# OpenVVC/OpenVVC

Hardware: AMD Instinct MI355X
Metric: decoded frames/sec, full rcn back-end decode step (H2D of the recorded picture + MC incl. BDOF/DMVR/affine-PROF/GPM/CIIP + LMCS + inverse transform + ordered intra pass + deblocking + SAO + ALF/CC-ALF + D2H of refined MVs + wait + per-picture digest + publication to the device DPB), 4K 10-bit RA rec (higher is better)
Workload: dtype u16 samples / int16 coefficients / int32 accumulate

## Files before the change

### include/ovvc_hip.h

```cpp
#ifndef OVVC_HIP_H
#define OVVC_HIP_H

#include <stddef.h>
#include <stdint.h>

#ifdef __cplusplus
extern "C" {
#endif

#define OVHIP_ABI_VERSION 9

#define OVHIP_OK        0
#define OVHIP_ENODEV   (-1)
#define OVHIP_ENOMEM   (-2)
#define OVHIP_EINVAL   (-3)
#define OVHIP_ELAUNCH  (-4)
#define OVHIP_EUNSUP   (-5)
#define OVHIP_EREF     (-6)

enum { OVHIP_DST_VII = 0, OVHIP_DCT_VIII = 1, OVHIP_DCT_II = 2 };

typedef struct ovhip_pic {
    uint16_t *y, *cb, *cr;
    int32_t   w, h;
// ... 251 lines not shown
    uint8_t cc_cb_idx, cc_cr_idx;
    uint8_t border;
    uint8_t pad;
} ovhip_alf_ctu;

typedef struct ovhip_alf_pic {
    const ovhip_alf_ctu *ctus;
    const int16_t *luma_coeff;
    const int16_t *luma_clip;
    const int16_t *chroma_coeff;
    const int16_t *chroma_clip;
    const int16_t *cc_coeff;
    uint8_t *class_scratch;
    int32_t log2_ctu_s;
} ovhip_alf_pic;

enum { OVHIP_IT_LUMA = 0,
       OVHIP_IT_CHROMA = 1,
       OVHIP_IT_REGION = 2,
       OVHIP_IT_RES_C = 3,
       OVHIP_IT_IBC_L = 4,
       OVHIP_IT_IBC_C = 5 };
enum {
    OVHIP_IF_CORNER = 1,
    OVHIP_IF_MIP = 2,
    OVHIP_IF_MIP_TR = 4,
    OVHIP_IF_BDPCM = 8,
    OVHIP_IF_BDPCM_VER = 16,
    OVHIP_IF_RES_Y = 32, OVHIP_IF_RES_CB = 64, OVHIP_IF_RES_CR = 128,
    OVHIP_IF_RES_SCALE = 256,
    OVHIP_IF_SCALE_IDX = 512,
    OVHIP_IF_IBC_FREE = 4096,
    OVHIP_IF_CORNER_L = 2048,
    OVHIP_IF_ISP = 1024
};
typedef struct ovhip_itask {
    uint16_t x, y;
    uint8_t  log2_w, log2_h;
    uint8_t  kind;
    uint8_t  mode;
    uint16_t flags;
    uint8_t  avl_lft, avl_abv;
    uint8_t  mrl_idx;
    uint8_t  ciip_wt;
    int16_t  c_scale;
    uint16_t level;
    uint16_t ctu_deps;
    uint8_t  isp_log2_cb_w, isp_log2_cb_h;
    uint8_t  isp_off_x, isp_off_y;
    uint8_t  isp_log2_pb;
    uint8_t  isp_res_mask;
    uint16_t pad[3];
} ovhip_itask;
#define OVHIP_ITASK_IBC_DX(t) ((int)(int16_t)(t).pad[0])
#define OVHIP_ITASK_IBC_DY(t) ((int)(int16_t)(t).pad[1])

typedef struct ovhip_recorder ovhip_recorder;

typedef struct ovhip_tu_state {
    uint8_t qp_y, qp_cb, qp_cr, qp_jcbcr;
    uint8_t qp_y_skip, qp_cb_skip, qp_cr_skip, qp_jcbcr_skip;
    uint8_t dep_quant;
    uint8_t mts_implicit;
    uint8_t sh_ts_disabled;
    uint8_t ict_type;
    uint8_t lmcs_scale_c;
// ... 86 lines not shown
int   ovhip_rec_tu_intra(ovhip_recorder *rec, const ovhip_tu_state *st, const ovhip_tu_desc *tu, const ovhip_itask *intra_l,
                         const ovhip_itask *intra_c);
typedef struct ovhip_ibc_desc {
    uint16_t x0, y0;
    uint8_t  log2_w, log2_h;
    uint8_t  log2_ctu;
    uint8_t  has_chroma;
    int16_t  mv_x, mv_y;
    uint16_t win_x0;
    uint16_t pad;
} ovhip_ibc_desc;
int   ovhip_rec_ibc_check(ovhip_recorder *rec, const ovhip_ibc_desc *cu);
int   ovhip_rec_tu_ibc(ovhip_recorder *rec, const ovhip_tu_state *st, const ovhip_tu_desc *tu, const ovhip_ibc_desc *cu);
size_t ovhip_rec_ibc_tasks(const ovhip_recorder *rec);
typedef struct ovhip_isp_desc {
    uint16_t x0, y0;
    uint8_t  log2_cb_w, log2_cb_h;
    uint8_t  vertical;
    uint8_t  intra_mode;
    uint8_t  cbf_mask;
    uint8_t  lfnst_flag, lfnst_idx;
    uint8_t  mts_enabled;
    uint8_t  corner[4];
    uint8_t  avl_abv[4], avl_lft[4];
    uint16_t last_pos[4];
    uint64_t sig_sb_map[4];
    const int16_t *coef;
} ovhip_isp_desc;
int   ovhip_rec_isp_cu(ovhip_recorder *rec, const ovhip_tu_state *st, const ovhip_isp_desc *cu);
void  ovhip_isp_geometry(int32_t log2_cb_w, int32_t log2_cb_h, int32_t vertical, int32_t *log2_pb, int32_t *n_pb, int32_t *log2_pred,
                         int32_t *n_pred);
const ovhip_itask *ovhip_rec_itasks(const ovhip_recorder *rec, size_t *n);
const ovhip_itask *ovhip_rec_itasks_sorted(ovhip_recorder *rec, size_t *n, const uint32_t **level_start, uint32_t *n_levels);
typedef struct ovhip_ictu {
    uint16_t cx, cy;
    uint32_t first, n;
    uint32_t deps;
} ovhip_ictu;
int   ovhip_rec_set_ctu_size(ovhip_recorder *rec, int32_t log2_ctu_s);
uint32_t ovhip_rec_itask_levels(const ovhip_recorder *rec);
const ovhip_itask *ovhip_rec_itasks_by_ctu(ovhip_recorder *rec, int32_t log2_ctu_s, size_t *n, const ovhip_ictu **ctus, size_t *n_ctus);
int   ovhip_rec_transform_tree(ovhip_recorder *rec, const ovhip_tu_state *st, const ovhip_tt_desc *tt);
int   ovhip_rec_pu(ovhip_recorder *rec, const ovhip_pu_desc *pu);
int   ovhip_rec_affine_cu(ovhip_recorder *rec, const ovhip_affine_desc *cu);
int   ovhip_rec_cu_inter(ovhip_recorder *rec, const ovhip_pu_desc *pu, const ovhip_affine_desc *aff);
int   ovhip_rec_set_ref_scale(ovhip_recorder *rec, int32_t slot, const ovhip_ref_scale *scale);
#define OVHIP_RPR_TOOL_AFFINE 1u
#define OVHIP_RPR_TOOL_PU4x4  2u
int   ovhip_rec_set_rpr_tools(ovhip_recorder *rec, uint32_t mask);
const char *ovhip_rec_refusal(const ovhip_recorder *rec);
int   ovhip_rec_ciip(ovhip_recorder *rec, int32_t x0, int32_t y0, int32_t log2_w, int32_t log2_h,
                     int32_t mode_abv, int32_t mode_lft);
int   ovhip_ciip_weight(int32_t mode_abv, int32_t mode_lft);
int   ovhip_rec_lmcs_region(ovhip_recorder *rec, int32_t x0, int32_t y0, uint32_t abv_mask, uint32_t lft_mask);
typedef struct ovhip_dbf_edge {
    uint16_t ux, uy;
    uint16_t word;
    uint8_t  comp;
    uint8_t  pad;
} ovhip_dbf_edge;
#define OVHIP_DBF_MAX_OFFSETS 8
typedef struct ovhip_dbf_offsets { int8_t beta[OVHIP_DBF_MAX_OFFSETS], tc[OVHIP_DBF_MAX_OFFSETS]; } ovhip_dbf_offsets;
const ovhip_dbf_edge *ovhip_rec_dbf_edges(const ovhip_recorder *rec, int dir, size_t *n, ovhip_dbf_offsets *offsets);
int64_t ovhip_dbf_compact(const ovhip_dbf_planes *planes, int dir, ovhip_dbf_edge *out, size_t cap);

int   ovhip_rec_dbf_ctu(ovhip_recorder *rec, const ovhip_dbf_ctu *ctu);
// ... 363 lines not shown
    int32_t threads_per_device;
    int32_t output;
    ovhip_window window;
    uint32_t extra_stages;
    int32_t rank;
    const ovhip_stream_xfer *xfer;
    int32_t intra_lookahead;
    int32_t ahead_own_queue;
} ovhip_stream_cfg;

typedef struct ovhip_stream_result {
    double   seconds;
    uint64_t n_decoded, n_second_passes, n_received, n_sent;
    uint64_t out_frames, out_bytes;
    uint8_t  out_md5[16];
    double   record_seconds;
    double   host_seconds[5];
    int32_t  status;
    char     error[192];
    double  *trace;
} ovhip_stream_result;

typedef struct ovhip_stream ovhip_stream;
int  ovhip_stream_create(ovhip_stream **out, ovhip_dpb *dpb, const ovhip_stream_cfg *cfg, const ovhip_stream_content *contents,
                         uint32_t n_contents, ovhip_job *const *jobs, uint32_t n_jobs);
void ovhip_stream_destroy(ovhip_stream *s);
int  ovhip_stream_run(ovhip_stream *s, const ovhip_stream_pic *pics, uint32_t n_total, uint32_t first, uint32_t n, uint32_t flags,
                      uint8_t *digests, ovhip_stream_result *res);
ovhip_frame *ovhip_stream_frame(ovhip_stream *s, int dev, int thread);
int  ovhip_stream_queue_info(const ovhip_stream *s, int *moved, int *sharing);
int  ovhip_stream_set_output_scale(ovhip_stream *s, int32_t out_w, int32_t out_h, const ovhip_scale_info *info);
const void *ovhip_stream_key(const ovhip_stream *s, uint32_t idx);
int  ovhip_job_test_abort_next_flow(ovhip_job *job);

#ifdef __cplusplus
}
#endif
#endif
```

### openvvc_amd/capi.py

```python
from __future__ import annotations

import ctypes as C
import os
from pathlib import Path

import numpy as np

_PKG = Path(__file__).resolve().parent
LIB_PATH = _PKG / os.environ.get("OVVC_HIP_LIB_NAME", "libovvc_hip.so")

OVHIP_ABI_VERSION = 9
OVHIP_OK, OVHIP_ENODEV, OVHIP_ENOMEM, OVHIP_EINVAL, OVHIP_ELAUNCH, OVHIP_EUNSUP, OVHIP_EREF = 0, -1, -2, -3, -4, -5, -6
DST_VII, DCT_VIII, DCT_II = 0, 1, 2
TB_TR, TB_DC, TB_TS, TB_TS_RAW = 0, 1, 2, 3
TB_FLAG_RASTER = 0x80
RES_ADD, RES_SUB, RES_ADD_HALF, RES_SUB_HALF, RES_SCALE = 0, 1, 2, 3, 4
MC_HPEL_FILT, MC_FILT_4x4, MC_NO_LUMA, MC_NO_CHROMA, MC_LMCS, MC_BDOF, MC_DMVR = 1, 2, 4, 8, 16, 32, 64
PU_BDOF, PU_DMVR, PU_GPM = 1, 2, 4
MC_GPM = 128


class Pic(C.Structure):
    _fields_ = [("y", C.c_void_p), ("cb", C.c_void_p), ("cr", C.c_void_p),
                ("w", C.c_int32), ("h", C.c_int32), ("stride_y", C.c_int32), ("stride_c", C.c_int32)]
# ... 516 lines not shown
        "ovhip_job_band_busy": (C.c_int, [vp]),
        "ovhip_job_band_progress": (C.c_int, [vp, P(i32), P(vp), P(vp)]),
        "ovhip_rec_counts": (None, [vp, P(BandCounts)]),
        "ovhip_sao_launch_rows": (C.c_int, [vp, P(Pic), P(Pic), vp, i32, i32, i32]),
        "ovhip_alf_launch_rows": (C.c_int, [vp, P(Pic), P(Pic), P(AlfPic), i32, i32]),
        "ovhip_job_wait": (C.c_int, [vp]),
        "ovhip_job_refined_mvs": (vp, [vp, P(C.c_size_t)]),
        "ovhip_job_dmvr_rows": (C.c_int64, [vp, P(Pic), u32]),
        "ovhip_job_dmvr_rows_begin": (C.c_int64, [vp, P(Pic), u32, i32]),
        "ovhip_job_dmvr_rows_collect": (C.c_int64, [vp]),
        "ovhip_job_last_stats": (C.c_int, [vp, P(JobStats)]),
        "ovhip_job_time_stage": (C.c_int, [vp, C.c_int]),
        "ovhip_job_stage_time": (C.c_int, [vp, P(C.c_double), P(C.c_uint64)]),
        "ovhip_lmcs_scale_prepare_launch": (C.c_int, [vp, P(Pic), vp, u32, vp, vp, vp, u32, vp, u32]),
        "ovhip_lmcs_inverse_untag_launch": (C.c_int, [vp, P(Pic), vp, vp, u32]),
        "ovhip_intra_flow_untag_launch": (C.c_int, [vp, P(Pic), vp, u32, i32]),
        "ovhip_tmvp_cells_launch": (C.c_int, [vp, vp, u32, vp, i32, i32, vp]),
        "ovhip_job_tmvp_cells": (vp, [vp, P(C.c_size_t)]),
        "ovhip_output_bytes": (C.c_size_t, [i32, i32, P(Window)]),
        "ovhip_output_rows": (C.c_size_t, [i32, i32, P(Window)]),
        "ovhip_output_pack_launch": (C.c_int, [vp, P(Pic), P(Window), vp]),
        "ovhip_output_row_md5_launch": (C.c_int, [vp, P(Pic), P(Window), vp]),
        "ovhip_output_bands": (C.c_size_t, [i32, i32, P(Window)]),
        "ovhip_output_tree_md5_launch": (C.c_int, [vp, P(Pic), P(Window), vp]),
        "ovhip_pic_output": (C.c_int, [vp, P(Pic), P(Window), vp]),
        "ovhip_pic_digest": (C.c_int, [vp, P(Pic), P(Window), vp]),
        "ovhip_md5_init": (None, [P(Md5State)]),
        "ovhip_md5_update": (None, [P(Md5State), vp, C.c_size_t]),
        "ovhip_md5_final": (None, [P(Md5State), vp]),
        "ovhip_d2d": (C.c_int, [vp, vp, vp, C.c_size_t]),
        "ovhip_host_alloc": (vp, [C.c_size_t]),
        "ovhip_host_free": (None, [vp]),
        "ovhip_job_test_abort_next_flow": (C.c_int, [vp]),
        "ovhip_dpb_create": (C.c_int, [P(vp), P(C.c_int), C.c_int]),
        "ovhip_dpb_create_ex": (C.c_int, [P(vp), C.c_int, P(DpbOps)]),
        "ovhip_dpb_destroy": (None, [vp]),
        "ovhip_dpb_n_devices": (C.c_int, [vp]),
        "ovhip_dpb_device": (C.c_int, [vp, C.c_int]),
        "ovhip_dpb_begin": (C.c_int, [vp, vp, C.c_int, i32, i32, P(Pic)]),
        "ovhip_dpb_want": (C.c_int, [vp, vp, C.c_int]),
        "ovhip_dpb_begin_tag": (C.c_int, [vp, vp, C.c_uint64, C.c_int, i32, i32, P(Pic)]),
        "ovhip_dpb_want_tag": (C.c_int, [vp, vp, C.c_uint64, C.c_int]),
        "ovhip_dpb_acquire_tag": (C.c_int, [vp, vp, C.c_uint64, C.c_int, P(Pic), P(vp)]),
        "ovhip_dpb_publish": (C.c_int, [vp, vp, C.c_int]),
        "ovhip_dpb_acquire": (C.c_int, [vp, vp, C.c_int, P(Pic), P(vp)]),
        "ovhip_dpb_wait_copy": (C.c_int, [vp, C.c_int, vp]),
        "ovhip_dpb_poll_tag": (C.c_int, [vp, vp, C.c_uint64]),
        "ovhip_frame_refs_ready": (C.c_int, [vp]),
        "ovhip_dpb_set_unknown_key_timeout": (None, [vp, C.c_int]),
        "ovhip_dpb_unpin": (C.c_int, [vp, vp]),
        "ovhip_dpb_release": (C.c_int, [vp, vp]),
        "ovhip_dpb_lookup": (C.c_int, [vp, vp, P(C.c_int), P(Pic)]),
        "ovhip_dpb_shutdown": (None, [vp]),
        "ovhip_dpb_get_stats": (C.c_int, [vp, P(DpbStats)]),
        "ovhip_frame_create": (C.c_int, [vp, C.c_int, i32, i32, P(vp)]),
        "ovhip_frame_destroy": (None, [vp]),
        "ovhip_frame_ctx": (vp, [vp]),
        "ovhip_frame_job": (vp, [vp]),
        "ovhip_frame_recorder": (vp, [vp]),
        "ovhip_frame_begin": (C.c_int, [vp, vp]),
        "ovhip_frame_ref": (C.c_int, [vp, vp]),
        "ovhip_frame_set_trace": (None, [vp, vp]),
        "ovhip_rccl_unique_id": (C.c_int, [vp]),
        "ovhip_rccl_create": (C.c_int, [P(vp), vp, C.c_int, C.c_int, C.c_int]),
        "ovhip_rccl_destroy": (None, [vp]),
        "ovhip_rccl_xfer": (vp, [vp]),
# ... 40 lines not shown
    if path is None:
        _lib = lib
    return lib


EXPORTED_SYMBOLS = [
    "ovhip_abi_version", "ovhip_rec_create", "ovhip_rec_destroy", "ovhip_rec_reset", "ovhip_rec_tu",
    "ovhip_rec_pu", "ovhip_rec_cu_inter", "ovhip_rec_dbf_row", "ovhip_rec_dbf_mv_prepass_view", "ovhip_rec_dbf_ctu", "ovhip_rec_dbf_planes", "ovhip_dbf_launch", "ovhip_sao_launch", "ovhip_alf_launch", "ovhip_rec_tb_cmds", "ovhip_rec_coefs", "ovhip_rec_mc_units", "ovhip_rec_mcx_units", "ovhip_mcx_launch", "ovhip_rec_affine_cu", "ovhip_rec_transform_tree", "ovhip_rec_lmcs_region", "ovhip_dbf_compact", "ovhip_rec_dbf_mv_prepass", "ovhip_dbf_launch_edges", "ovhip_rec_ciip", "ovhip_ciip_weight", "ovhip_rec_ciip_units", "ovhip_ciip_launch", "ovhip_rec_lmcs_regions", "ovhip_rec_tb_cmds_split", "ovhip_itx_launch_classes", "ovhip_itx_launch_chroma_lmcs", "ovhip_lmcs_build", "ovhip_lmcs_scale_launch", "ovhip_lmcs_inverse_launch", "ovhip_rec_aff_units", "ovhip_rec_aff_side", "ovhip_mca_launch", "ovhip_mcxa_launch", "ovhip_ctx_create",
    "ovhip_ctx_destroy", "ovhip_ctx_sync", "ovhip_ctx_shares_queue", "ovhip_ctx_new_stream", "ovhip_ctx_fork", "ovhip_ctx_join", "ovhip_last_error", "ovhip_ctx_stream", "ovhip_malloc",
    "ovhip_free", "ovhip_h2d", "ovhip_d2h", "ovhip_pic_alloc", "ovhip_pic_free", "ovhip_pic_upload",
    "ovhip_pic_download", "ovhip_itx_launch", "ovhip_mc_launch",
    "ovhip_rec_set_ref_scale", "ovhip_rec_refusal", "ovhip_rec_rpr_units", "ovhip_mc_rpr_launch",
    "ovhip_rec_set_rpr_tools", "ovhip_rec_aff_rpr_units", "ovhip_mca_rpr_launch",
    "ovhip_rec_create_ex", "ovhip_rec_set_dense_dbf_planes", "ovhip_rec_dbf_edges", "ovhip_dbf_launch_edges_ex",
    "ovhip_dmvr_search_launch", "ovhip_rec_append_raw", "ovhip_rec_set_dbf_offsets", "ovhip_rec_tu_intra", "ovhip_rec_itasks", "ovhip_rec_itasks_sorted", "ovhip_itx_launch_classes_res", "ovhip_intra_level_launch", "ovhip_intra_level_geom", "ovhip_intra_sync_words", "ovhip_intra_ctu_launch", "ovhip_intra_flow_words", "ovhip_intra_flow_items", "ovhip_intra_flow_launch",
    "ovhip_rec_itask_levels", "ovhip_rec_isp_cu", "ovhip_isp_geometry", "ovhip_rec_itasks_by_ctu", "ovhip_rec_set_ctu_size", "ovhip_job_bind", "ovhip_job_create", "ovhip_job_destroy", "ovhip_job_recorder", "ovhip_job_begin",
    "ovhip_frame_band", "ovhip_frame_band_upto", "ovhip_frame_dmvr_rows_begin_upto", "ovhip_job_dmvr_rows_begin_upto", "ovhip_frame_set_band_mode", "ovhip_frame_band_stats", "ovhip_dpb_post_rows", "ovhip_dpb_rows_tag",
    "ovhip_job_band", "ovhip_job_band_active", "ovhip_job_band_busy", "ovhip_job_band_reserve", "ovhip_job_reserve_for_picture", "ovhip_rec_reserve_for_picture", "ovhip_job_band_progress", "ovhip_rec_counts", "ovhip_sao_launch_rows", "ovhip_alf_launch_rows",
    "ovhip_job_flush", "ovhip_job_wait", "ovhip_job_refined_mvs", "ovhip_job_dmvr_rows", "ovhip_job_dmvr_rows_begin", "ovhip_job_dmvr_rows_collect", "ovhip_job_last_stats", "ovhip_job_time_stage", "ovhip_job_stage_time",
    "ovhip_output_bytes", "ovhip_output_rows", "ovhip_output_pack_launch", "ovhip_output_row_md5_launch", "ovhip_output_bands", "ovhip_output_tree_md5_launch", "ovhip_pic_output", "ovhip_pic_digest",
    "ovhip_md5_init", "ovhip_md5_update", "ovhip_md5_final", "ovhip_tmvp_cells_launch", "ovhip_job_tmvp_cells", "ovhip_intra_flow_untag_launch", "ovhip_lmcs_inverse_untag_launch", "ovhip_lmcs_scale_prepare_launch",
    "ovhip_host_alloc", "ovhip_host_free", "ovhip_d2d", "ovhip_job_test_abort_next_flow",
    "ovhip_dpb_create", "ovhip_dpb_create_ex", "ovhip_dpb_destroy", "ovhip_dpb_n_devices", "ovhip_dpb_device", "ovhip_dpb_begin", "ovhip_dpb_want",
    "ovhip_dpb_publish", "ovhip_dpb_acquire", "ovhip_dpb_wait_copy", "ovhip_dpb_poll_tag", "ovhip_frame_refs_ready", "ovhip_dpb_set_unknown_key_timeout", "ovhip_dpb_unpin", "ovhip_dpb_release", "ovhip_dpb_lookup", "ovhip_dpb_shutdown",
    "ovhip_dpb_get_stats", "ovhip_dpb_begin_tag", "ovhip_dpb_want_tag", "ovhip_dpb_acquire_tag", "ovhip_frame_begin_tag", "ovhip_frame_ref_tag", "ovhip_frame_set_trace",
    "ovhip_rccl_unique_id", "ovhip_rccl_create", "ovhip_rccl_destroy", "ovhip_rccl_xfer", "ovhip_rccl_last_error", "ovhip_rccl_stats", "ovhip_rccl_self_exchange",
    "ovhip_frame_create", "ovhip_frame_destroy", "ovhip_frame_ctx", "ovhip_frame_job", "ovhip_frame_recorder", "ovhip_frame_begin", "ovhip_frame_ref",
    "ovhip_frame_ref_at", "ovhip_frame_dmvr_rows", "ovhip_frame_dmvr_rows_begin", "ovhip_frame_dmvr_rows_collect", "ovhip_frame_submit", "ovhip_frame_fail", "ovhip_frame_last_error",
    "ovhip_calllog_create", "ovhip_calllog_destroy", "ovhip_calllog_reset", "ovhip_calllog_data", "ovhip_rec_set_calllog", "ovhip_calllog_replay",
    "ovhip_stream_create", "ovhip_stream_destroy", "ovhip_stream_run", "ovhip_stream_frame", "ovhip_stream_key", "ovhip_stream_queue_info",
    "ovhip_output_scale_check", "ovhip_output_scale_launch", "ovhip_pic_output_scaled", "ovhip_pic_digest_scaled",
    "ovhip_frame_set_output_scale", "ovhip_stream_set_output_scale", "ovhip_ctx_scratch_bytes",
    "ovhip_rec_ibc_check", "ovhip_rec_tu_ibc", "ovhip_rec_ibc_tasks",
]


def rpr_units(lib, rec) -> list:
    n = C.c_size_t(0)
    ptr = lib.ovhip_rec_rpr_units(rec, C.byref(n))
    if not ptr or not n.value:
        return []
    raw = C.string_at(ptr, n.value * C.sizeof(RprUnit))
    return [RprUnit.from_buffer_copy(raw, i * C.sizeof(RprUnit)) for i in range(n.value)]


def aff_rpr_units(lib, rec) -> list:
    n = C.c_size_t(0)
    ptr = lib.ovhip_rec_aff_rpr_units(rec, C.byref(n))
    if not ptr or not n.value:
        return []
    raw = C.string_at(ptr, n.value * C.sizeof(AffRprUnit))
    return [AffRprUnit.from_buffer_copy(raw, i * C.sizeof(AffRprUnit)) for i in range(n.value)]


def set_ref_scale(lib, rec, slot: int, scale_hor: int | None = None, scale_ver: int | None = None, ref_w: int = 0, ref_h: int = 0,
                  col_hor: int = 0, col_ver: int = 0) -> int:
    if scale_hor is None:
        return lib.ovhip_rec_set_ref_scale(rec, slot, None)
    sc = RefScale(scale_hor, scale_ver if scale_ver is not None else scale_hor, ref_w, ref_h, col_hor, col_ver)
    return lib.ovhip_rec_set_ref_scale(rec, slot, C.byref(sc))


class Recorder:

    def __init__(self, pic_w: int, pic_h: int):
        self.lib = load()
# ... 34 lines not shown
    def replay(self, log: np.ndarray) -> int:
        n = self.lib.ovhip_calllog_replay(log.ctypes.data, log.nbytes, self.h)
        if n < 0:
            raise ValueError(f"ovhip_calllog_replay -> {n}")
        return int(n)

    def tu(self, st: TuState, d: TuDesc) -> int:
        r = self.lib.ovhip_rec_tu(self.h, C.byref(st), C.byref(d))
        if r < 0:
            raise ValueError(f"ovhip_rec_tu -> {r}")
        return r

    def tu_intra(self, st: TuState, d: TuDesc, task_l: "ITask | None", task_c: "ITask | None") -> int:
        r = self.lib.ovhip_rec_tu_intra(self.h, C.byref(st), C.byref(d), C.byref(task_l) if task_l is not None else None,
                                        C.byref(task_c) if task_c is not None else None)
        if r < 0:
            raise ValueError(f"ovhip_rec_tu_intra -> {r}")
        return r

    def ibc_check(self, cu: IbcDesc) -> int:
        return self.lib.ovhip_rec_ibc_check(self.h, C.byref(cu))

    def tu_ibc(self, st: TuState, d: TuDesc, cu: IbcDesc) -> int:
        return self.lib.ovhip_rec_tu_ibc(self.h, C.byref(st), C.byref(d), C.byref(cu))

    def ibc_tasks(self) -> int:
        return int(self.lib.ovhip_rec_ibc_tasks(self.h))

    def refusal(self) -> str:
        return (self.lib.ovhip_rec_refusal(self.h) or b"").decode()

    def itasks(self) -> np.ndarray:
        return self._arr(self.lib.ovhip_rec_itasks, ITASK_DTYPE)

    def itasks_sorted(self):
        n, nl, ls = C.c_size_t(), C.c_uint32(), C.POINTER(C.c_uint32)()
        p = self.lib.ovhip_rec_itasks_sorted(self.h, C.byref(n), C.byref(ls), C.byref(nl))
        if not n.value:
            return np.zeros(0, ITASK_DTYPE), np.zeros(1, np.uint32)
        t = np.frombuffer((C.c_char * (n.value * 32)).from_address(p), dtype=ITASK_DTYPE).copy()
        return t, np.array([ls[i] for i in range(nl.value + 1)], np.uint32)

    def itasks_by_ctu(self, log2_ctu: int = 7):
        n, nc, cp = C.c_size_t(), C.c_size_t(), C.c_void_p()
        p = self.lib.ovhip_rec_itasks_by_ctu(self.h, log2_ctu, C.byref(n), C.byref(cp), C.byref(nc))
        if not n.value:
            return np.zeros(0, ITASK_DTYPE), np.zeros(0, ICTU_DTYPE)
        t = np.frombuffer((C.c_char * (n.value * 32)).from_address(p), dtype=ITASK_DTYPE).copy()
        c = np.frombuffer((C.c_char * (nc.value * 16)).from_address(cp.value), dtype=ICTU_DTYPE).copy()
        return t, c

    def transform_tree(self, st: "TuState", d: TtDesc, infos: bytes, res_cb: np.ndarray, res_cr: np.ndarray, res_y: np.ndarray) -> int:
        ib = (C.c_char * len(infos)).from_buffer_copy(infos)
        keep = [np.ascontiguousarray(a, dtype=np.int16) for a in (res_cb, res_cr, res_y)]
        d.tu_info = C.addressof(ib)
        for k in range(3):
            d.residual[k] = keep[k].ctypes.data
        r = self.lib.ovhip_rec_transform_tree(self.h, C.byref(st), C.byref(d))
        d.tu_info = None
        if r < 0:
            raise ValueError(f"ovhip_rec_transform_tree -> {r}")
        return r

    def isp_cu(self, st: TuState, d: IspDesc) -> int:
        r = self.lib.ovhip_rec_isp_cu(self.h, C.byref(st), C.byref(d))
        if r < 0:
# ... 129 lines not shown
```

### openvvc_amd/csrc/flow_state.hip.h

```cpp
#pragma once
#include <hip/hip_runtime.h>
#include <stdint.h>
#include "ovvc_hip.h"

#define OVHIP_FLOW_SYNC_WORDS 16
struct FlowState { unsigned *y, *c[2], *reg; int w4; };

static inline FlowState flow_state_of(uint32_t *d_state, int w, int h)
{
    FlowState fs;
    const size_t nu = (size_t)((w + 3) / 4) * ((h + 3) / 4);
    fs.w4 = (w + 3) / 4;
    fs.y = d_state + OVHIP_FLOW_SYNC_WORDS; fs.c[0] = fs.y + nu; fs.c[1] = fs.c[0] + nu; fs.reg = fs.c[1] + nu;
    return fs;
}

#define FLOW_ITEM_TASK_BITS  24
#define FLOW_ITEM_STRIP_BITS 5
#define FLOW_ITEM_MAX_TASKS  ((size_t)1 << FLOW_ITEM_TASK_BITS)
#define FLOW_ITEM_MAX_STRIPS (1 << FLOW_ITEM_STRIP_BITS)
struct FlowItem { uint32_t task; int strip, plane; };

__host__ __device__ static inline uint32_t flow_item_pack(uint32_t task, int strip, int plane)
{
    return task | ((uint32_t)strip << FLOW_ITEM_TASK_BITS) | ((uint32_t)plane << (FLOW_ITEM_TASK_BITS + FLOW_ITEM_STRIP_BITS));
}
__host__ __device__ static inline FlowItem flow_item_unpack(uint32_t word)
{
    FlowItem it;
    it.task = word & ((1u << FLOW_ITEM_TASK_BITS) - 1);
    it.strip = (int)((word >> FLOW_ITEM_TASK_BITS) & (FLOW_ITEM_MAX_STRIPS - 1));
    it.plane = (int)((word >> (FLOW_ITEM_TASK_BITS + FLOW_ITEM_STRIP_BITS)) & 1);
    return it;
}

extern "C" size_t ovhip_intra_flow_items_(const ovhip_itask *sorted, size_t n, uint32_t *items, size_t cap);

__device__ __forceinline__ void flow_prepare_task(const ovhip_itask &t, const FlowState &fs, unsigned epoch, int lane16)
{
    const unsigned mark = 2 * epoch;
    if (t.kind == OVHIP_IT_REGION) { if (lane16 == 0) fs.reg[t.c_scale] = mark; return; }
    const bool luma = t.kind == OVHIP_IT_LUMA || t.kind == OVHIP_IT_IBC_L;
    const bool both = t.kind == OVHIP_IT_CHROMA || t.kind == OVHIP_IT_IBC_C;
    const int sh = luma ? 2 : 1, w = 1 << t.log2_w, h = 1 << t.log2_h;
    const int ux0 = t.x >> sh, uy0 = t.y >> sh, nx = max(1, w >> sh), ny = max(1, h >> sh);
    const int l2nx = 31 - __clz(nx);
    for (int i = lane16; i < nx * ny; i += 16) {
        const int u = (uy0 + (i >> l2nx)) * fs.w4 + ux0 + (i & (nx - 1));
        if (luma) fs.y[u] = mark;
        else {
            if (both || (t.flags & OVHIP_IF_RES_CB)) fs.c[0][u] = mark;
            if (both || (t.flags & OVHIP_IF_RES_CR)) fs.c[1][u] = mark;
        }
    }
}
```

### openvvc_amd/csrc/kernels_intra.hip

```cpp
#include <stdlib.h>
#include "ovvc_common.hip.h"
#include "flow_state.hip.h"
#include "lmcs_wnd.hip.h"
#define OVT_ATTR __device__
#include "vvc_mip_tables.h"

namespace {

__device__ const short g_ang[32] = { 0, 1, 2, 3, 4, 6, 8, 10, 12, 14, 16, 18, 20, 23, 26, 29, 32, 35, 39, 45, 51, 57, 64, 73, 86, 102, 128, 171, 256, 341, 512, 1024 };
__device__ const short g_inv_ang[32] = { 0, 16384, 8192, 5461, 4096, 2731, 2048, 1638, 1365, 1170, 1024, 910, 819, 712, 630, 565, 512, 468, 420, 364,
                                         321, 287, 256, 224, 191, 161, 128, 96, 64, 48, 32, 16 };
__device__ __attribute__((aligned(4))) const signed char g_fc[32][4] = {
    { 0, 64, 0, 0 }, { -1, 63, 2, 0 }, { -2, 62, 4, 0 }, { -2, 60, 7, -1 }, { -2, 58, 10, -2 }, { -3, 57, 12, -2 }, { -4, 56, 14, -2 },
    { -4, 55, 15, -2 }, { -4, 54, 16, -2 }, { -5, 53, 18, -2 }, { -6, 52, 20, -2 }, { -6, 49, 24, -3 }, { -6, 46, 28, -4 }, { -5, 44, 29, -4 },
    { -4, 42, 30, -4 }, { -4, 39, 33, -4 }, { -4, 36, 36, -4 }, { -4, 33, 39, -4 }, { -4, 30, 42, -4 }, { -4, 29, 44, -5 }, { -4, 28, 46, -6 },
    { -3, 24, 49, -6 }, { -2, 20, 52, -6 }, { -2, 18, 53, -5 }, { -2, 16, 54, -4 }, { -2, 15, 55, -4 }, { -2, 14, 56, -4 }, { -2, 12, 57, -3 },
    { -2, 10, 58, -2 }, { -1, 7, 60, -2 }, { 0, 4, 62, -2 }, { 0, 2, 63, -1 } };

#define IR_NEG  64
#define IR_LEN  (IR_NEG + 2 * 64 + 4 + 24)
struct IntraLds {
    uint16_t abv[IR_LEN], lft[IR_LEN];
    uint16_t fabv[IR_LEN], flft[IR_LEN];
    uint16_t red[64], hup[8 * 64];
// ... 90 lines not shown
        const int n_cu = 2 * cb + 1, nb_ref = (2 * cb) / 4 + 1, len = cb + pb, last = min(4 * a, n_cu + 3);
        uint16_t *out = (arm ? s.lft : s.abv) + IR_NEG;
        for (int k = lane; k < len + 1 + 24; k += 64) {
            const int kk = min(k, len) + off;
            int v;
            if (c && a >= nb_ref) {
                const int q = min(kk, n_cu - 1);
                v = arm ? acc.ld(x0 - 1, y0 - oy - 1 + q) : acc.ld(x0 - ox - 1 + q, y0 - 1);
            } else if (c || a) {
                const int q = kk == 0 ? (c ? 0 : 1) : (a ? min(kk, last) : 0);
                v = arm ? acc.ld(x0 - 1, y0 - oy - 1 + q) : acc.ld(x0 - ox - 1 + q, y0 - 1);
            } else {
                v = other ? (arm ? acc.ld(x0, y0 - 1) : acc.ld(x0 - 1, y0)) : 1 << (OV_BD - 1);
            }
            out[k] = (uint16_t)v;
        }
    }
}

__device__ void smooth_refs(IntraLds &s, int len_a, int len_l, int lane)
{
    const uint16_t *a = s.abv + IR_NEG, *l = s.lft + IR_NEG;
    for (int i = lane; i < 2 * 64 + 4 + 24; i += 64) {
        int va, vl;
        if (i == 0) { va = (l[1] + 2 * a[0] + a[1] + 2) >> 2; vl = (a[1] + 2 * l[0] + l[1] + 2) >> 2; }
        else {
            va = i < len_a ? (a[i + 1] + 2 * a[i] + a[i - 1] + 2) >> 2 : a[i];
            vl = i < len_l ? (l[i + 1] + 2 * l[i] + l[i - 1] + 2) >> 2 : l[i];
        }
        s.fabv[IR_NEG + i] = (uint16_t)va; s.flft[IR_NEG + i] = (uint16_t)vl;
    }
}

__device__ __forceinline__ int res_scale(int v, int scale)
{
    const int sign = v & (1 << 15);
    int a = (ov_clip_bd(abs(v)) * scale + (1 << 10)) >> 11;
    return ov_clip3(sign ? -a : a, -(1 << 15), 1 << 15);
}

__device__ void pred_regular(IntraLds &s, const ovhip_itask &t, bool is_luma, const Strip st, int lane)
{
    const int l2w = t.log2_w, l2h = t.log2_h, w = 1 << l2w, h = 1 << l2h, n = w * h;
    const bool isp = t.flags & OVHIP_IF_ISP;
    const int mrl = (is_luma && !isp) ? t.mrl_idx : 0;
    const bool bdpcm = t.flags & OVHIP_IF_BDPCM;
    const bool pdpc_ok = isp ? l2h > 1 : (!mrl && !bdpcm && (is_luma || (l2w > 1 && l2h > 1)));
    const uint16_t *abv = s.abv + IR_NEG, *lft = s.lft + IR_NEG;
    if (bdpcm) {
        const bool ver = t.flags & OVHIP_IF_BDPCM_VER;
        for (int p = st.p0 + lane; p < st.p1; p += 64) { const int x = p & (w - 1), y = p >> l2w; s.pred[p - st.p0] = ver ? abv[1 + x] : lft[1 + y]; }
        return;
    }
    int mode = t.mode;
    if (mode == 0) {
        const uint16_t *a = abv + mrl, *l = lft + mrl;
        if (is_luma && !isp && !mrl && l2w + l2h > 5) { smooth_refs(s, w + 4, h + 4, lane); wave_sync(); a = s.fabv + IR_NEG; l = s.flft + IR_NEG; }
        const int scale = (l2w + l2h - 2) >> 2;
        for (int p = st.p0 + lane; p < st.p1; p += 64) {
            const int x = p & (w - 1), y = p >> l2w;
            const int pv = ((h - 1 - y) * a[1 + x] + (y + 1) * l[1 + h]) << l2w;
            const int ph = ((w - 1 - x) * l[1 + y] + (x + 1) * a[1 + w]) << l2h;
            int v = (pv + ph + n) >> (l2w + l2h + 1);
            if (pdpc_ok) { const int wt = pdpc_wgt(y, scale), wl = pdpc_wgt(x, scale); v = ov_clip_bd((l[1 + y] * wl + a[1 + x] * wt + (64 - wl - wt) * v + 32) >> 6); }
            s.pred[p - st.p0] = (uint16_t)v;
        }
        return;
    }
    if (mode == 1) {
        const uint16_t *a = abv + mrl, *l = lft + mrl;
        int sum = 0;
        if (w >= h) for (int x = lane; x < w; x += 64) sum += a[1 + x];
// ... 299 lines not shown
    int v[NP];
#pragma unroll
    for (int i = 0; i < NP; ++i) {
        const int p = min(it.p0 + lane + 64 * i, it.p1 - 1);
        v[i] = acc.ld(sx + (p & ((1 << l2w) - 1)), sy + (p >> l2w)) & 0x7fff;
    }
#pragma unroll
    for (int i = 0; i < NP; ++i) { const int p = it.p0 + lane + 64 * i; if (p < it.p1) s.pred[p - it.p0] = (uint16_t)v[i]; }
    wave_sync();
}

template <int NP>
__device__ __forceinline__ void epilogue_load(int (&rv)[NP], int (&dv)[NP], const Item &it, const uint16_t *dst, int dstride, const int16_t *rp, int rstride,
                                              int l2w, int lane)
{
#pragma unroll
    for (int i = 0; i < NP; ++i) {
        const int p = it.p0 + lane + 64 * i, x = p & ((1 << l2w) - 1), y = p >> l2w;
        rv[i] = (it.has_res && p < it.p1 && it.res_at(x)) ? rp[y * rstride + x] : 0;
        dv[i] = (it.need_d() && p < it.p1) ? dst[y * dstride + x] : 0;
    }
}

template <int NP>
__device__ __forceinline__ void epilogue_store(const IntraLds &s, const int (&rv)[NP], const int (&dv)[NP], const Item &it, int scale, uint16_t *dst, int dstride,
                                               int l2w, int lane)
{
#pragma unroll
    for (int i = 0; i < NP; ++i) {
        const int p = it.p0 + lane + 64 * i, x = p & ((1 << l2w) - 1), y = p >> l2w;
        if (p >= it.p1) break;
        int v = it.res_only ? dv[i] : s.pred[p - it.p0];
        if (it.ciip_wt) v = (v * it.ciip_wt + dv[i] * (4 - it.ciip_wt) + 2) >> 2;
        if (it.has_res) v = ov_clip_bd(v + (it.scaled ? res_scale(rv[i], scale) : rv[i]));
        dst[y * dstride + x] = (uint16_t)v;
    }
}

template <bool IBC>
__global__ __launch_bounds__(64) void k_intra_level(ovhip_pic pic, ovhip_pic res, const ovhip_itask *__restrict__ tasks, uint32_t n,
                                                    const ovhip_lmcs_region *__restrict__ regs, LmcsWnd wnd, int16_t *__restrict__ scales,
                                                    int log2_ctu)
{
    __shared__ IntraLds s;
    const uint32_t bid = blockIdx.x;
    const int strip = blockIdx.y, comp = blockIdx.z;
    if (bid >= n) return;
    const int lane = threadIdx.x;
    load_tables(s, lane);
    const ovhip_itask t = tasks[bid];
    const Item it = item_of<STRIP, IBC>(t, strip, comp);
    const PlaneAcc ya = { pic.y, pic.stride_y };
    if (it.region) {
        if (!strip && !comp) { const int v = region_scale(ya, regs[t.c_scale], wnd, lane); if (lane == 0) scales[t.c_scale] = (int16_t)v; }
        return;
    }
    if (it.p0 >= it.p1 || (it.luma && comp) || it.skip()) return;
    uint16_t *pl = it.luma ? pic.y : (comp ? pic.cr : pic.cb);
    const int dstride = it.luma ? pic.stride_y : pic.stride_c, rstride = it.luma ? res.stride_y : res.stride_c;
    uint16_t *dst = pl + t.y * dstride + t.x;
    const int16_t *rp = reinterpret_cast<const int16_t *>(it.luma ? res.y : (comp ? res.cr : res.cb)) + t.y * rstride + t.x;
    int rv[NPL], dv[NPL];
    epilogue_load(rv, dv, it, dst, dstride, rp, rstride, t.log2_w, lane);
    const int scale = it.scaled ? (it.scale_idx ? scales[t.c_scale] : t.c_scale) : 0;
    const PlaneAcc ca = { pl, pic.stride_c };
    if (IBC && t.kind >= OVHIP_IT_IBC_L) ibc_copy<NPL>(s, t, it, PlaneAcc{ pl, dstride }, lane);
    else if (!it.res_only) predict_item<NPL>(s, t, it, ya, ca, log2_ctu, DirectRefs(), lane);
// ... 288 lines not shown
        }
        if (lowered) __builtin_amdgcn_s_setprio(OVHIP_FLOW_PRIO);
    }
#pragma unroll
    for (int i = 0; i < 3; ++i) {
        const int k = lane + 64 * i;
        if (k < na + 24) s.abv[IR_NEG + k] = (uint16_t)(v[2 * i] & 0x7fff);
        if (k < nl + 24) s.lft[IR_NEG + k] = (uint16_t)(v[2 * i + 1] & 0x7fff);
    }
    return ok;
}
#define FLOW_MAX_FP 448
#ifndef FSTRIP
#define FSTRIP 256
#endif
#define FNPL   (FSTRIP / 64)
#define FJ8    ((FSTRIP + 511) / 512)
#define FJ4    ((FSTRIP + 255) / 256)

__global__ __launch_bounds__(256) void k_intra_flow_prepare(const ovhip_itask *__restrict__ tasks, uint32_t n, FlowState fs, unsigned epoch)
{
    const uint32_t ti = blockIdx.x * 16 + (threadIdx.x >> 4);
    if (ti < n) flow_prepare_task(tasks[ti], fs, epoch, threadIdx.x & 15);
}

typedef uint32_t flow_u4 __attribute__((ext_vector_type(4), aligned(4)));
typedef uint32_t flow_u2 __attribute__((ext_vector_type(2), aligned(4)));
__global__ __launch_bounds__(256) void k_flow_untag(ovhip_pic pic, const ovhip_itask *__restrict__ tasks, uint32_t n, int with_luma)
{
    const uint32_t ti = blockIdx.x * 16 + (threadIdx.x >> 4);
    if (ti >= n) return;
    const ovhip_itask t = tasks[ti];
    const bool luma = t.kind == OVHIP_IT_LUMA || t.kind == OVHIP_IT_IBC_L;
    if (t.kind == OVHIP_IT_REGION || (luma && !with_luma)) return;
    const int lane = threadIdx.x & 15;
    const int l2w = t.log2_w, w = 1 << l2w, npx = w << t.log2_h;
    const int stride = luma ? pic.stride_y : pic.stride_c;
    for (int c = 0; c < (luma ? 1 : 2); ++c) {
        if (!luma && t.kind == OVHIP_IT_RES_C && !(t.flags & (c ? OVHIP_IF_RES_CR : OVHIP_IF_RES_CB))) continue;
        uint16_t *dst = (luma ? pic.y : (c ? pic.cr : pic.cb)) + t.y * stride + t.x;
        if (w >= 4) {
            for (int p = 4 * lane; p < npx; p += 64) {
                flow_u2 *q = reinterpret_cast<flow_u2 *>(dst + (p >> l2w) * stride + (p & (w - 1)));
                flow_u2 v = *q; v[0] &= 0x03ff03ffu; v[1] &= 0x03ff03ffu; *q = v;
            }
        } else if (w == 2) {
            for (int p = 2 * lane; p < npx; p += 32) {
                uint32_t *q = reinterpret_cast<uint32_t *>(dst + (p >> l2w) * stride + (p & (w - 1)));
                *q &= 0x03ff03ffu;
            }
        } else {
            for (int p = lane; p < npx; p += 16) { uint16_t *q = dst + (p >> l2w) * stride + (p & (w - 1)); *q = *q & 0x3ff; }
        }
    }
}

struct TaggedRefs {
    const unsigned *state_y, *state_c;
    int w4; unsigned epoch; unsigned *sync;
#ifdef OVHIP_CTU_PROBE
    u64 *stamp;
    __device__ __forceinline__ void arms_ready() const { *stamp = wall_clock64(); }
#else
    __device__ __forceinline__ void arms_ready() const { }
#endif
    __device__ __forceinline__ bool operator()(IntraLds &s, const AgentAcc acc, int unit, const ovhip_itask &t, int mrl, int lane) const
    {
// ... 34 lines not shown
{
    uint32_t r;
    asm("v_pk_add_i16 %0, %1, %2 clamp\n\tv_pk_max_i16 %0, %0, 0\n\tv_pk_min_i16 %0, %0, %3" : "=&v"(r) : "v"(pred2), "v"(res2), "v"(0x03ff03ffu));
    return r;
}

template <int G>
__device__ __forceinline__ void flow_store(const IntraLds &s, const FlowRaw &q, const Item &it, int scale, uint16_t *dst, int dstride, int l2w, int lane)
{
    typedef FlowRun<G> R;
    const uint32_t tag2 = FLOW_TAG | (FLOW_TAG << 16);
    const bool plain = G > 1 && !it.ciip_wt && !it.res_only && !it.scaled && it.res_mask == 0xff;
#pragma unroll
    for (int j = 0; j < R::N; ++j) {
        const int p = R::p_of(it, j, lane), x = p & ((1 << l2w) - 1), y = p >> l2w;
        if (p >= it.p1) break;
        typename R::vec pq = 0, out;
        if constexpr (G == 1) pq = s.pred[p - it.p0];
        else if (!it.res_only) pq = *reinterpret_cast<const typename R::vec *>(&s.pred[p - it.p0]);
        if (plain) {
#pragma unroll
            for (int e = 0; e < R::DW; ++e) out[e] = (it.has_res ? pk_clip_add(pq[e], q.r[R::DW * j + e]) : pq[e]) | tag2;
        } else {
            int v[G], rv[G], dv[G];
#pragma unroll
            for (int e = 0; e < G; ++e) {
                const int sh = 16 * (e & 1), k = R::DW * j + (e >> 1);
                rv[e] = it.res_at(x + e) ? (int)(int16_t)(q.r[k] >> sh) : 0;
                dv[e] = (int)((q.d[k] >> sh) & 0xffff);
                v[e] = it.res_only ? dv[e] : (int)((pq[e >> 1] >> sh) & 0xffff);
            }
            if (it.ciip_wt) for (int e = 0; e < G; ++e) v[e] = (v[e] * it.ciip_wt + dv[e] * (4 - it.ciip_wt) + 2) >> 2;
            if (it.has_res) {
                if (it.scaled) for (int e = 0; e < G; ++e) v[e] = ov_clip_bd(v[e] + res_scale(rv[e], scale));
                else           for (int e = 0; e < G; ++e) v[e] = ov_clip_bd(v[e] + rv[e]);
            }
#pragma unroll
            for (int e = 0; e < R::DW; ++e) out[e] = ((uint32_t)v[2 * e] | (G > 1 ? (uint32_t)v[G > 1 ? 2 * e + 1 : 0] << 16 : 0u)) | tag2;
        }
        uint16_t *o = dst + y * dstride + x;
        if constexpr (G == 8) asm volatile("global_store_dwordx4 %0, %1, off sc1" :: "v"(o), "v"(out) : "memory");
        else if constexpr (G == 4) asm volatile("global_store_dwordx2 %0, %1, off sc1" :: "v"(o), "v"(out) : "memory");
        else __hip_atomic_store(o, (uint16_t)out[0], RLX_AGENT);
    }
}

struct FlowLds { IntraLds s; uint32_t fp[FLOW_MAX_FP]; int abort; };

template <bool IBC>
__global__ __launch_bounds__(64) void k_intra_flow(ovhip_pic pic, ovhip_pic res, const ovhip_itask *__restrict__ tasks, const uint32_t *__restrict__ items,
                                                   uint32_t n_items, const ovhip_lmcs_region *__restrict__ regs, LmcsWnd wnd, int16_t *scales,
                                                   int log2_ctu, FlowState fs, unsigned epoch, unsigned *sync, unsigned *abort_mirror)
{
    __shared__ FlowLds L;
    IntraLds &s = L.s;
    if (blockIdx.x >= n_items) return;
    __builtin_amdgcn_s_setprio(OVHIP_FLOW_PRIO);
    const int lane = threadIdx.x;
    load_tables(s, lane);
    int prev_level = 0;
    for (uint32_t bid = blockIdx.x; bid < n_items; bid += gridDim.x) {
    if (bid != blockIdx.x) wave_sync();
    FPROBE_DECL;
    const FlowItem fi = flow_item_unpack(items[bid]);
    const ovhip_itask t = tasks[fi.task];
    const int comp = fi.plane;
    const Item it = item_of<FSTRIP, IBC>(t, fi.strip, comp);
    const int l2w = t.log2_w, w = 1 << l2w, h = 1 << t.log2_h;
    const bool luma = it.luma;
    const bool ibc = IBC && t.kind >= OVHIP_IT_IBC_L;
    const unsigned pending = 2 * epoch;
    const int w4 = fs.w4;
    if (it.skip()) continue;

    uint16_t *pl = luma ? pic.y : (comp ? pic.cr : pic.cb);
    const int dstride = luma ? pic.stride_y : pic.stride_c, rstride = luma ? res.stride_y : res.stride_c;
    uint16_t *dst = pl + t.y * dstride + t.x;
    const int16_t *rp = reinterpret_cast<const int16_t *>(luma ? res.y : (comp ? res.cr : res.cb)) + t.y * rstride + t.x;
    const int run = w >= 8 ? 8 : (w == 4 ? 4 : 1);
    FlowRaw raw = { };
    if (!it.region) {
        if (run == 8) flow_load<8>(raw, it, dst, dstride, rp, rstride, l2w, lane);
        else if (run == 4) flow_load<4>(raw, it, dst, dstride, rp, rstride, l2w, lane);
        else flow_load<1>(raw, it, dst, dstride, rp, rstride, l2w, lane);
    }
    {
        const int gap = min((int)t.level - prev_level - 1, FLOW_NAP_MAX_LEVELS);
        prev_level = (int)t.level;
        if (gap > 0) {
            __builtin_amdgcn_s_setprio(0);
            for (int k = 0; k < 2 * gap; ++k) __builtin_amdgcn_s_sleep(FLOW_NAP_HALF_LEVEL);
            __builtin_amdgcn_s_setprio(OVHIP_FLOW_PRIO);
        }
    }
    FPROBE(0);
    int nfp = 0;
    auto add_run = [&](unsigned *base, int ux, int uy, int count, int dx, int dy) {
        count = min(count, FLOW_MAX_FP - nfp);
        for (int i = lane; i < count; i += 64) L.fp[nfp + i] = (uint32_t)(base - sync) + (uint32_t)((uy + i * dy) * w4 + ux + i * dx);
        nfp += max(count, 0);
    };
    if (it.region) {
        const ovhip_lmcs_region g = regs[t.c_scale];
        if (g.n_abv) add_run(fs.y, g.x >> 2, (g.y >> 2) - 1, g.n_abv, 1, 0);
        if (g.n_lft) add_run(fs.y, (g.x >> 2) - 1, g.y >> 2, g.n_lft, 0, 1);
    } else if (luma) {
// ... 144 lines not shown
extern "C" int ovhip_debug_set_ctu_probe(void *d_buf)
{
    u64 *p = (u64 *)d_buf;
    return hipMemcpyToSymbol(HIP_SYMBOL(g_probe), &p, sizeof(p)) == hipSuccess ? 0 : -1;
}
#endif

extern "C" size_t ovhip_intra_sync_words(int32_t width, int32_t height, int32_t log2_ctu_s)
{
    if (width <= 0 || height <= 0 || log2_ctu_s < 5 || log2_ctu_s > 7) return 0;
    const size_t s = (size_t)1 << log2_ctu_s;
    return SYNC_FLAGS + ((width + s - 1) / s) * ((height + s - 1) / s);
}

extern "C" int ovhip_intra_ctu_launch(ovhip_ctx *ctx, const ovhip_pic *pic, const ovhip_pic *res, const ovhip_itask *d_tasks, const ovhip_ictu *d_ctus,
                                      uint32_t n_ctus, const ovhip_lmcs_region *d_regions, const ovhip_lmcs_luts *luts, int16_t *d_scales,
                                      int32_t log2_ctu_s, uint32_t *d_sync, uint32_t epoch, uint32_t *abort_mirror)
{
    if (!ctx || !pic || !res) return OVHIP_EINVAL;
    OV_DEVICE(ctx);
    if (!n_ctus) return OVHIP_OK;
    if (!d_tasks || !d_ctus || !d_sync || !epoch || log2_ctu_s < 5 || log2_ctu_s > 7)
        return ov_fail(ctx, OVHIP_EINVAL, "ovhip_intra_ctu_launch: bad arguments", hipSuccess);
    if ((pic->w & 7) || (pic->h & 1) || (pic->stride_y & 3) || (pic->stride_c & 3) || ((uintptr_t)pic->y & 7) || ((uintptr_t)pic->cb & 7) || ((uintptr_t)pic->cr & 7))
        return ov_fail(ctx, OVHIP_EUNSUP, "ovhip_intra_ctu_launch: picture width must be a multiple of 8 and the planes 8-byte aligned", hipSuccess);
    const LmcsWnd wnd = lmcs_wnd_of(luts);
    const int ncx = (pic->w + (1 << log2_ctu_s) - 1) >> log2_ctu_s;
    hipLaunchKernelGGL(k_intra_ctu, dim3(n_ctus), dim3(256), 0, ctx->stream, *pic, *res, d_tasks, d_ctus, d_regions, wnd, d_scales, log2_ctu_s, d_sync, epoch, ncx,
                       abort_mirror);
    OV_LAUNCH_CHECK(ctx, "k_intra_ctu");
    return OVHIP_OK;
}

extern "C" size_t ovhip_intra_flow_items_(const ovhip_itask *sorted, size_t n, uint32_t *items, size_t cap)
{
    size_t k = 0;
    for (size_t i = 0; sorted && i < n; ++i) {
        const ovhip_itask &t = sorted[i];
        if (i >= FLOW_ITEM_MAX_TASKS) return 0;
        if (t.kind == OVHIP_IT_REGION) { if (k < cap) items[k] = flow_item_pack((uint32_t)i, 0, 0); ++k; continue; }
        const int npx = 1 << (t.log2_w + t.log2_h), strips = (npx + FSTRIP - 1) / FSTRIP, comps = (t.kind == OVHIP_IT_LUMA || t.kind == OVHIP_IT_IBC_L) ? 1 : 2;
        if (strips > FLOW_ITEM_MAX_STRIPS) return 0;
        for (int st = 0; st < strips; ++st)
            for (int c = 0; c < comps; ++c) { if (k < cap) items[k] = flow_item_pack((uint32_t)i, st, c); ++k; }
    }
    return k;
}

extern "C" size_t ovhip_intra_flow_items(const ovhip_itask *sorted, size_t n, uint32_t *items, size_t cap)
{
    const size_t k = ovhip_intra_flow_items_(sorted, n, items, cap);
    return k <= cap ? k : 0;
}

extern "C" size_t ovhip_intra_flow_words(int32_t width, int32_t height)
{
    if (width <= 0 || height <= 0) return 0;
    return SYNC_FLAGS + 4 * (size_t)((width + 3) / 4) * ((height + 3) / 4);
}

extern "C" int ovhip_intra_flow_launch(ovhip_ctx *ctx, const ovhip_pic *pic, const ovhip_pic *res, const ovhip_itask *d_tasks, uint32_t n_tasks,
                                       const uint32_t *d_items, uint32_t n_items, const ovhip_lmcs_region *d_regions, const ovhip_lmcs_luts *luts,
                                       int16_t *d_scales, int32_t log2_ctu_s, uint32_t *d_state, uint32_t epoch, uint32_t *abort_mirror, int32_t prepare,
                                       int32_t n_workers)
{
    if (!ctx || !pic || !res) return OVHIP_EINVAL;
    OV_DEVICE(ctx);
    if (!n_items) return OVHIP_OK;
    if (!d_tasks || !d_items || !d_state || !epoch || epoch >= 0x7fffffffu || log2_ctu_s < 5 || log2_ctu_s > 7)
        return ov_fail(ctx, OVHIP_EINVAL, "ovhip_intra_flow_launch: bad arguments", hipSuccess);
    const LmcsWnd wnd = lmcs_wnd_of(luts);
    const FlowState fs = flow_state_of(d_state, pic->w, pic->h);
    if (prepare & 1) {
        hipLaunchKernelGGL(k_intra_flow_prepare, dim3((n_tasks + 15) / 16), dim3(256), 0, ctx->stream, d_tasks, n_tasks, fs, epoch);
        OV_LAUNCH_CHECK(ctx, "k_intra_flow_prepare");
    }
#ifdef OVHIP_CTU_PROBE
    if (hipMemcpyToSymbolAsync(HIP_SYMBOL(g_probe_items), &d_items, sizeof(d_items), 0, hipMemcpyHostToDevice, ctx->stream) != hipSuccess) return OVHIP_ELAUNCH;
#endif
    const uint32_t grid = (n_workers > 0 && (uint32_t)n_workers < n_items) ? (uint32_t)n_workers : n_items;
    if (prepare & OVHIP_FLOW_IBC)
        hipLaunchKernelGGL(k_intra_flow<true>, dim3(grid), dim3(64), 0, ctx->stream, *pic, *res, d_tasks, d_items, n_items, d_regions, wnd, d_scales, log2_ctu_s, fs,
                           epoch, d_state, abort_mirror);
    else
// ... 17 lines not shown
```

### openvvc_amd/csrc/kernels_lmcs.hip

```cpp
#include "ovvc_common.hip.h"
#include "flow_state.hip.h"
#include "lmcs_wnd.hip.h"

namespace {

#ifndef LMCS_ROWS
#define LMCS_ROWS 4
#endif

__global__ __launch_bounds__(64) void k_lmcs_scale(ovhip_pic pic, const ovhip_lmcs_region *__restrict__ regs, uint32_t n,
                                                   LmcsWnd wnd, int16_t *__restrict__ scales, const ovhip_itask *__restrict__ tasks,
                                                   uint32_t n_tasks, FlowState fs, unsigned epoch)
{
    const uint32_t bid = blockIdx.x;
    if (bid >= n) {
        const uint32_t ti = (bid - n) * 4 + (threadIdx.x >> 4);
        if (ti < n_tasks) flow_prepare_task(tasks[ti], fs, epoch, threadIdx.x & 15);
        return;
    }
    const ovhip_lmcs_region g = regs[bid];
    if (g.ordered) return;
    const int lane = threadIdx.x;
    const uint16_t *src = pic.y + (size_t)g.y * pic.stride_y + g.x;
    const int na = 4 * g.n_abv, nl = 4 * g.n_lft;
    const long oa = g.n_abv ? (long)min(lane, na - 1) - pic.stride_y : 0;
    const long ol = g.n_lft ? (long)min(lane, nl - 1) * pic.stride_y - 1 : 0;
    const int va = src[oa], vl = src[ol];
    int sum = (g.n_abv ? va : 0) + (g.n_lft ? vl : 0);
#pragma unroll
    for (int m = 32; m; m >>= 1) sum += __shfl_xor(sum, m);
    if (lane == 0) scales[bid] = (int16_t)lmcs_scale_of_sum(wnd, sum, g.n_abv, g.n_lft);
}

typedef uint32_t lm_u2 __attribute__((ext_vector_type(2), aligned(4)));

#define UNTAG_TASKS_PER_WG 4
__device__ __forceinline__ void untag_chroma_tasks(const ovhip_pic &pic, const ovhip_itask *__restrict__ tasks, uint32_t n, uint32_t wg)
{
    const uint32_t ti = wg * UNTAG_TASKS_PER_WG + (threadIdx.x >> 6);
    if (ti >= n) return;
    const ovhip_itask t = tasks[ti];
    if (t.kind == OVHIP_IT_REGION || t.kind == OVHIP_IT_LUMA || t.kind == OVHIP_IT_IBC_L) return;
    const int lane = threadIdx.x & 63;
    const int l2w = t.log2_w, w = 1 << l2w, npx = w << t.log2_h, stride = pic.stride_c;
    const bool res_only = t.kind == OVHIP_IT_RES_C;
    const bool on0 = !res_only || (t.flags & OVHIP_IF_RES_CB), on1 = !res_only || (t.flags & OVHIP_IF_RES_CR);
    uint16_t *const d0 = pic.cb + t.y * stride + t.x, *const d1 = pic.cr + t.y * stride + t.x;
    if (w >= 4) {
        for (int base = 0; base < npx; base += 1024) {
            lm_u2 v0[4], v1[4];
#pragma unroll
            for (int k = 0; k < 4; ++k) {
                const int p = base + 4 * lane + 256 * k;
                const int o = (p >> l2w) * stride + (p & (w - 1));
                if (p < npx && on0) v0[k] = *reinterpret_cast<const lm_u2 *>(d0 + o);
                if (p < npx && on1) v1[k] = *reinterpret_cast<const lm_u2 *>(d1 + o);
            }
#pragma unroll
            for (int k = 0; k < 4; ++k) {
                const int p = base + 4 * lane + 256 * k;
                const int o = (p >> l2w) * stride + (p & (w - 1));
                if (p < npx && on0) { lm_u2 v = v0[k]; v[0] &= 0x03ff03ffu; v[1] &= 0x03ff03ffu; *reinterpret_cast<lm_u2 *>(d0 + o) = v; }
                if (p < npx && on1) { lm_u2 v = v1[k]; v[0] &= 0x03ff03ffu; v[1] &= 0x03ff03ffu; *reinterpret_cast<lm_u2 *>(d1 + o) = v; }
            }
        }
    } else if (w == 2) {
        for (int p = 2 * lane; p < npx; p += 128) {
            const int o = (p >> l2w) * stride + (p & (w - 1));
            uint32_t a = 0, b = 0;
            if (on0) a = *reinterpret_cast<const uint32_t *>(d0 + o);
            if (on1) b = *reinterpret_cast<const uint32_t *>(d1 + o);
            if (on0) *reinterpret_cast<uint32_t *>(d0 + o) = a & 0x03ff03ffu;
            if (on1) *reinterpret_cast<uint32_t *>(d1 + o) = b & 0x03ff03ffu;
        }
    } else {
        for (int p = lane; p < npx; p += 64) {
            const int o = (p >> l2w) * stride + (p & (w - 1));
            if (on0) d0[o] = d0[o] & 0x3ff;
            if (on1) d1[o] = d1[o] & 0x3ff;
        }
    }
}

__global__ __launch_bounds__(256) void k_lmcs_inverse(ovhip_pic pic, const uint16_t *__restrict__ lut, uint32_t rows_y,
                                                      const ovhip_itask *__restrict__ tasks, uint32_t n_tasks)
{
    const uint32_t untag_y = gridDim.y - rows_y;
    if (blockIdx.y < untag_y) { untag_chroma_tasks(pic, tasks, n_tasks, blockIdx.y * gridDim.x + blockIdx.x); return; }
    const uint32_t by = blockIdx.y - untag_y;

    __shared__ uint16_t s_lut[1024];
    const int nvx = pic.w >> 3;
    const int tail = pic.w & 7;
    const int y00 = (int)by * LMCS_ROWS, v00 = blockIdx.x * 256 + threadIdx.x;
    uint4 q0[LMCS_ROWS];
    const bool first = y00 < pic.h && v00 < nvx;
    if (first) {
#pragma unroll
        for (int r = 0; r < LMCS_ROWS; ++r) q0[r] = *reinterpret_cast<const uint4 *>(pic.y + (size_t)min(y00 + r, pic.h - 1) * pic.stride_y + 8 * v00);
    }
    for (int i = threadIdx.x; i < 512; i += 256) reinterpret_cast<uint32_t *>(s_lut)[i] = reinterpret_cast<const uint32_t *>(lut)[i];
    __syncthreads();
    for (int y0 = y00; y0 < pic.h; y0 += rows_y * LMCS_ROWS) {
        for (int v = v00; v < nvx; v += gridDim.x * 256) {
            uint4 q[LMCS_ROWS];
            if (y0 == y00 && v == v00) {
#pragma unroll
                for (int r = 0; r < LMCS_ROWS; ++r) q[r] = q0[r];
            } else {
#pragma unroll
                for (int r = 0; r < LMCS_ROWS; ++r) q[r] = *reinterpret_cast<const uint4 *>(pic.y + (size_t)min(y0 + r, pic.h - 1) * pic.stride_y + 8 * v);
            }
#pragma unroll
            for (int r = 0; r < LMCS_ROWS; ++r) {
                if (y0 + r >= pic.h) break;
                uint32_t *d = reinterpret_cast<uint32_t *>(&q[r]);
#pragma unroll
                for (int k = 0; k < 4; ++k) d[k] = s_lut[d[k] & 1023] | ((uint32_t)s_lut[(d[k] >> 16) & 1023] << 16);
                *reinterpret_cast<uint4 *>(pic.y + (size_t)(y0 + r) * pic.stride_y + 8 * v) = q[r];
            }
        }
// ... 7 lines not shown

}

static int lmcs_scale_launch(ovhip_ctx *ctx, const ovhip_pic *pic, const ovhip_lmcs_region *d_regions, uint32_t n_regions, const ovhip_lmcs_luts *luts,
                             int16_t *d_scales, const ovhip_itask *d_tasks, uint32_t n_tasks, uint32_t *d_state, uint32_t epoch)
{
    if (!ctx || !pic || !luts) return OVHIP_EINVAL;
    OV_DEVICE(ctx);
    if (!n_regions && !n_tasks) return OVHIP_OK;
    if (n_regions && (!d_regions || !d_scales)) return ov_fail(ctx, OVHIP_EINVAL, "ovhip_lmcs_scale_launch: null buffer", hipSuccess);
    if (n_tasks && (!d_tasks || !d_state || !epoch)) return ov_fail(ctx, OVHIP_EINVAL, "ovhip_lmcs_scale_prepare_launch: bad arguments", hipSuccess);
    const LmcsWnd w = lmcs_wnd_of(luts);
    FlowState fs;
    memset(&fs, 0, sizeof(fs));
    if (n_tasks) fs = flow_state_of(d_state, pic->w, pic->h);
    hipLaunchKernelGGL(k_lmcs_scale, dim3(n_regions + (n_tasks + 3) / 4), dim3(64), 0, ctx->stream, *pic, d_regions, n_regions, w, d_scales, d_tasks, n_tasks, fs, epoch);
    OV_LAUNCH_CHECK(ctx, n_tasks ? "k_lmcs_scale (+ flow state words)" : "k_lmcs_scale");
    return OVHIP_OK;
}

extern "C" int ovhip_lmcs_scale_launch(ovhip_ctx *ctx, const ovhip_pic *pic, const ovhip_lmcs_region *d_regions,
                                       uint32_t n_regions, const ovhip_lmcs_luts *luts, int16_t *d_scales)
{
    return lmcs_scale_launch(ctx, pic, d_regions, n_regions, luts, d_scales, nullptr, 0, nullptr, 0);
}

extern "C" int ovhip_lmcs_scale_prepare_launch(ovhip_ctx *ctx, const ovhip_pic *pic, const ovhip_lmcs_region *d_regions, uint32_t n_regions,
                                               const ovhip_lmcs_luts *luts, int16_t *d_scales, const ovhip_itask *d_tasks, uint32_t n_tasks,
                                               uint32_t *d_state, uint32_t epoch)
{
    return lmcs_scale_launch(ctx, pic, d_regions, n_regions, luts, d_scales, d_tasks, n_tasks, d_state, epoch);
}

static int lmcs_inverse_launch(ovhip_ctx *ctx, const ovhip_pic *pic, const uint16_t *d_bwd_lut, const ovhip_itask *d_tasks, uint32_t n_tasks, const char *who)
{
    if (!ctx || !pic || !d_bwd_lut) return OVHIP_EINVAL;
    OV_DEVICE(ctx);
    if ((pic->stride_y & 7) || ((uintptr_t)pic->y & 15))
        return ov_fail(ctx, OVHIP_EINVAL, "ovhip_lmcs_inverse_launch: luma plane must be 16-byte aligned with stride % 8 == 0", hipSuccess);
    const int nvx = pic->w >> 3;
    const int row_groups = (pic->h + LMCS_ROWS - 1) / LMCS_ROWS;
    const uint32_t gx = (nvx + 255) / 256 > 0 ? (nvx + 255) / 256 : 1, rows_y = row_groups < 4096 ? row_groups : 4096;
    const uint32_t untag_wgs = d_tasks ? (n_tasks + UNTAG_TASKS_PER_WG - 1) / UNTAG_TASKS_PER_WG : 0;
    hipLaunchKernelGGL(k_lmcs_inverse, dim3(gx, rows_y + (untag_wgs + gx - 1) / gx), dim3(256), 0, ctx->stream, *pic, d_bwd_lut, rows_y, d_tasks, d_tasks ? n_tasks : 0u);
    OV_LAUNCH_CHECK(ctx, who);
    return OVHIP_OK;
}

extern "C" int ovhip_lmcs_inverse_launch(ovhip_ctx *ctx, const ovhip_pic *pic, const uint16_t *d_bwd_lut)
{
    return lmcs_inverse_launch(ctx, pic, d_bwd_lut, nullptr, 0, "k_lmcs_inverse");
}

extern "C" int ovhip_lmcs_inverse_untag_launch(ovhip_ctx *ctx, const ovhip_pic *pic, const uint16_t *d_bwd_lut, const ovhip_itask *d_tasks, uint32_t n_tasks)
{
    if (n_tasks && !d_tasks) return OVHIP_EINVAL;
    return lmcs_inverse_launch(ctx, pic, d_bwd_lut, n_tasks ? d_tasks : nullptr, n_tasks, "k_lmcs_inverse (+ chroma un-tag)");
}
```

### openvvc_amd/csrc/ovvc_band.hip

```cpp
#include "ovvc_job.hip.h"

extern "C" void ovhip_rec_tb_split_range_(const ovhip_recorder *r, size_t first, size_t n, ovhip_tb_cmd *out, size_t counts[4], size_t tiny[4][4]);
extern "C" int  ovhip_rec_itasks_sorted_range_(const ovhip_recorder *r, size_t first, size_t n, ovhip_itask *out, uint32_t *level_start, size_t cap, uint32_t *n_levels);

enum { MAX_BANDS = 96, ARENA_CHUNKS = 16, BAND_LEVELS = 4096 };
struct ArenaChunk { char *host, *dev; size_t cap, used; };
struct BandRec {
    int32_t row0, row1;
    ovhip_band_counts c0, c1;
    const ovhip_itask *d_it; uint32_t n_it; int tagged;
    const ovhip_dbf_edge *d_ev, *d_eh; uint32_t n_ev, n_eh;
    int flow_charge;
    int32_t rows_final;
};
struct BandState {
    int active, n, tails, closed, failed;
    ovhip_pic dst;
    ovhip_band_counts cur;
    int32_t row_prev, dbf_rows, sao_rows, alf_rows, rows_final;
    int log2_ctu, sao_on, alf_on, filters_latched;
    uint32_t stages;
    const uint16_t *d_fwd, *d_bwd; int lmcs_up;
    ovhip_alf_pic d_alf; int alf_up;
    ovhip_lmcs_luts luts; int have_luts;
// ... 185 lines not shown
    const int32_t row_end = k.row_end;
    if (!(dst->y == bs->dst.y) || log2_ctu != bs->log2_ctu) return ov_fail(ctx, OVHIP_EINVAL, "ovhip_job_band: another picture than the first band's", hipSuccess);
    if (row_end < bs->row_prev || (!k.last && (row_end & ((1 << log2_ctu) - 1)) && row_end != j->h))
        return ov_fail(ctx, OVHIP_EINVAL, "ovhip_job_band: row_end must be a CTU-row boundary not above the previous band's", hipSuccess);
    if (bs->n >= MAX_BANDS) return ov_fail(ctx, OVHIP_EUNSUP, "ovhip_job_band: too many bands", hipSuccess);
    const uint32_t stages = bs->stages;
    band_reclaim(j, 0);

    ovhip_band_counts c1;
    ovhip_rec_counts(rec, &c1);
    if (upto) {
        const uint32_t *u = &upto->n_tb, *m = &c1.n_tb, *lo = &bs->cur.n_tb;
        for (int i = 0; i < 10; ++i) if (u[i] > m[i] || u[i] < lo[i]) return ov_fail(ctx, OVHIP_EINVAL, "ovhip_job_band: counts outside the recorded arrays", hipSuccess);
        c1 = *upto;
    }
    const ovhip_band_counts c0 = bs->cur;
    const int b = k.b = bs->n;
    BandRec &B = bs->band[b];
    const int charged = B.flow_charge;
    memset(&B, 0, sizeof(B));
    B.flow_charge = charged;
    B.row0 = bs->row_prev; B.row1 = row_end; B.c0 = k.c0 = c0; B.c1 = k.c1 = c1;
    size_t dummy = 0;
    if (ovhip_rec_ciip_units(rec, &dummy) && dummy) return ov_fail(ctx, OVHIP_EUNSUP, "ovhip_job_band: stand-alone CIIP blend units (a second picture with the caller's intra prediction)", hipSuccess);
    if (ovhip_rec_rpr_units(rec, &dummy) && dummy) return ov_fail(ctx, OVHIP_EUNSUP, "ovhip_job_band: reference picture resampling units", hipSuccess);
    if (ovhip_rec_aff_rpr_units(rec, &dummy) && dummy) return ov_fail(ctx, OVHIP_EUNSUP, "ovhip_job_band: reference picture resampling units (affine)", hipSuccess);
    if (ovhip_rec_ibc_tasks(rec)) return ov_fail(ctx, OVHIP_EUNSUP, "ovhip_job_band: intra block copy tasks (the whole-picture flush runs them)", hipSuccess);
    {
        const uint32_t *hi = &c1.n_tb, *lo = &c0.n_tb; uint32_t *n = &k.n.n_tb;
        for (int i = 0; i < 10; ++i) n[i] = hi[i] - lo[i];
    }
    if (!(stages & OVHIP_STAGE_DBF)) k.n.n_edge_v = k.n.n_edge_h = 0;
    if (!(stages & OVHIP_STAGE_INTRA)) k.n.n_itask = 0;
    k.n_items = k.n.n_itask && !(pr->stages && (stages & OVHIP_STAGE_INTRA_LEVELS)) ? ovhip_intra_flow_items_(ovhip_rec_itasks(rec, &dummy) + c0.n_itask, k.n.n_itask, nullptr, 0) : 0;

    const Switches sw = switches_of(pr);
    k.t_first = bs->tails; k.t_end = b + 1;
    if (k.t_end > k.t_first && !bs->filters_latched) {
        bs->sao_on = sw.sao_on; bs->alf_on = sw.alf_on;
        bs->filters_latched = 1;
    }
    if (bs->filters_latched && (bs->sao_on != sw.sao_on || bs->alf_on != sw.alf_on))
        return ov_fail(ctx, OVHIP_EINVAL, "ovhip_job_band: SAO / ALF switched on or off inside a picture", hipSuccess);
    k.sao_on = bs->filters_latched && bs->sao_on; k.alf_on = bs->filters_latched && bs->alf_on;
    if (k.alf_on && alf_tables_missing(pr)) return ov_fail(ctx, OVHIP_EINVAL, "ovhip_job_band: ALF tables missing", hipSuccess);
    k.dbf_new = bs->dbf_rows; k.sao_new = bs->sao_rows; k.alf_new = bs->alf_rows;
    if (k.t_end > k.t_first) {
        const int32_t E = k.t_end - 1 == b ? row_end : bs->band[k.t_end - 1].row1;
        const bool fin = k.last != 0;
        k.dbf_new = fin ? j->h : ((stages & OVHIP_STAGE_DBF) ? (E - 8 > k.dbf_new ? E - 8 : k.dbf_new) : E);
        k.sao_new = fin ? j->h : (floor8(k.dbf_new - 1) > k.sao_new ? floor8(k.dbf_new - 1) : k.sao_new);
        k.alf_new = fin ? j->h : (floor8(k.sao_new - 3) > k.alf_new ? floor8(k.sao_new - 3) : k.alf_new);
    }
    k.nb_ctu_w = (j->w + (1 << log2_ctu) - 1) >> log2_ctu;
    k.sao_r0 = bs->sao_rows >> log2_ctu; k.alf_r0 = bs->alf_rows >> log2_ctu;
    const int sao_r1 = k.sao_new > bs->sao_rows ? ((k.sao_new - 1) >> log2_ctu) + 1 : k.sao_r0;
    const int alf_r1 = k.alf_new > bs->alf_rows ? ((k.alf_new - 1) >> log2_ctu) + 1 : k.alf_r0;
    k.n_sao = k.sao_on ? (size_t)(sao_r1 - k.sao_r0) * k.nb_ctu_w : 0; k.n_alf = k.alf_on ? (size_t)(alf_r1 - k.alf_r0) * k.nb_ctu_w : 0;
    return OVHIP_OK;
}

static int band_stage(ovhip_job *j, const ovhip_pic *dst, const ovhip_job_params *pr, BandCall &k, Placement &p, Chain &c)
{
    ovhip_ctx *ctx = j->ctx;
    BandState *bs = j->bs;
    ovhip_recorder *rec = j->rec;
    const ovhip_band_counts &c0 = k.c0, &n = k.n;
    Layout L;
    const bool lmcs_now = pr->lmcs && !bs->lmcs_up, alf_now = k.alf_on && !bs->alf_up;
    p = Placement{};
    p.tabs = tables_put(L, alf_now, lmcs_now);
    const size_t o_tb = L.put(n.n_tb * sizeof(ovhip_tb_cmd)), o_coef = L.put((size_t)n.n_coef * 2), o_mc = L.put(n.n_mc * sizeof(ovhip_mc_unit)),
                 o_mcx = L.put(n.n_mcx * sizeof(ovhip_mc_unit)), o_aff = L.put(n.n_aff * sizeof(ovhip_aff_unit)), o_side = L.put((size_t)n.n_side * 4),
                 o_reg = L.put(n.n_reg * sizeof(ovhip_lmcs_region)), o_it = L.put(n.n_itask * sizeof(ovhip_itask)), o_items = L.put(k.n_items * 4),
                 o_ev = L.put(n.n_edge_v * sizeof(ovhip_dbf_edge)), o_eh = L.put(n.n_edge_h * sizeof(ovhip_dbf_edge));
    p.o_sao = L.put(k.n_sao * sizeof(ovhip_sao_ctu)); p.o_alf = L.put(k.n_alf * sizeof(ovhip_alf_ctu));
    const size_t upload_bytes = L.o;
    const size_t o_mv = L.put((size_t)n.n_mcx * 16);
    char *hb = nullptr, *db = nullptr;
    if (L.o) CHK(arena_take(j, L.o, &hb, &db));

    uint32_t n_lv = 0;
    if (n.n_tb) ovhip_rec_tb_split_range_(rec, c0.n_tb, n.n_tb, (ovhip_tb_cmd *)(hb + o_tb), c.cls, c.tiny);
    k.have_levels = n.n_itask && ovhip_rec_itasks_sorted_range_(rec, c0.n_itask, n.n_itask, (ovhip_itask *)(hb + o_it), bs->level_start, BAND_LEVELS + 2, &n_lv) == 0;
    if (n.n_itask && !k.have_levels && !k.n_items) return ov_fail(ctx, OVHIP_EUNSUP, "ovhip_job_band: a band with more levels than the table holds and blocks the flow launch cannot take", hipSuccess);
    k.h_items = (const uint32_t *)(hb + o_items);
    if (k.n_items) (void)ovhip_intra_flow_items_((const ovhip_itask *)(hb + o_it), n.n_itask, (uint32_t *)(hb + o_items), k.n_items);
    size_t all;
    if (n.n_coef) memcpy(hb + o_coef, ovhip_rec_coefs(rec, &all) + c0.n_coef, (size_t)n.n_coef * 2);
    if (n.n_mc) memcpy(hb + o_mc, ovhip_rec_mc_units(rec, &all) + c0.n_mc, n.n_mc * sizeof(ovhip_mc_unit));
    if (n.n_mcx) memcpy(hb + o_mcx, ovhip_rec_mcx_units(rec, &all) + c0.n_mcx, n.n_mcx * sizeof(ovhip_mc_unit));
    if (n.n_aff) memcpy(hb + o_aff, ovhip_rec_aff_units(rec, &all) + c0.n_aff, n.n_aff * sizeof(ovhip_aff_unit));
    if (n.n_side) memcpy(hb + o_side, ovhip_rec_aff_side(rec, &all) + c0.n_side, (size_t)n.n_side * 4);
    if (n.n_reg) memcpy(hb + o_reg, ovhip_rec_lmcs_regions(rec, &all) + c0.n_reg, n.n_reg * sizeof(ovhip_lmcs_region));
    const ovhip_dbf_edge *ev = ovhip_rec_dbf_edges(rec, 0, &all, &bs->offs), *eh = ovhip_rec_dbf_edges(rec, 1, &all, nullptr);
    if (n.n_edge_v) memcpy(hb + o_ev, ev + c0.n_edge_v, n.n_edge_v * sizeof(ovhip_dbf_edge));
    if (n.n_edge_h) memcpy(hb + o_eh, eh + c0.n_edge_h, n.n_edge_h * sizeof(ovhip_dbf_edge));
    if (k.n_sao) memcpy(hb + p.o_sao, pr->sao + (size_t)k.sao_r0 * k.nb_ctu_w, k.n_sao * sizeof(ovhip_sao_ctu));
    if (k.n_alf) memcpy(hb + p.o_alf, pr->alf_ctus + (size_t)k.alf_r0 * k.nb_ctu_w, k.n_alf * sizeof(ovhip_alf_ctu));
    tables_fill(hb, p.tabs, pr, alf_now, lmcs_now);
    if (upload_bytes) {
        OV_HIP(ctx, hipMemcpyAsync(db, hb, upload_bytes, hipMemcpyHostToDevice, ctx->stream));
        j->st.h2d_bytes += upload_bytes; j->st.n_h2d++;
    }
    OV_HIP(ctx, hipEventRecord(j->ev_h2d, ctx->stream));
    if (lmcs_now) { bs->d_fwd = (const uint16_t *)(db + p.tabs.at[T_FWD]); bs->d_bwd = (const uint16_t *)(db + p.tabs.at[T_BWD]); bs->lmcs_up = 1; bs->luts = *pr->lmcs; bs->have_luts = 1; }
    if (alf_now) { bs->d_alf = alf_pic_at(db, p.tabs, nullptr, (uint8_t *)j->dev[B_CLASS].p, bs->log2_ctu); bs->alf_up = 1; }
    if (pr->lmcs && !bs->lmcs_up) return ov_fail(ctx, OVHIP_EINVAL, "ovhip_job_band: LMCS tables", hipSuccess);
    p.block = db;
    p.at[B_TB] = db + o_tb; p.at[B_COEF] = db + o_coef; p.at[B_MC] = db + o_mc; p.at[B_MCX] = db + o_mcx; p.at[B_MV] = db + o_mv;
    p.at[B_AFF] = db + o_aff; p.at[B_SIDE] = db + o_side; p.at[B_REG] = db + o_reg; p.at[B_ITASK] = db + o_it; p.at[B_IITEM] = db + o_items;
    p.at[B_EV] = db + o_ev; p.at[B_EH] = db + o_eh;
    c.j = j; c.dst = dst; c.res = &j->res; c.log2_ctu = bs->log2_ctu;
    c.luts = pr->lmcs ? &bs->luts : nullptr; c.d_fwd = pr->lmcs ? bs->d_fwd : nullptr; c.d_scales = (int16_t *)j->dev[B_SCALE].p;
    chain_bind(c, p, c0, n, 0, 0);
    c.h_it = (const ovhip_itask *)(hb + o_it); c.lv_start = bs->level_start; c.n_lv = n_lv;
    BandRec &B = bs->band[k.b];
    B.d_it = c.d_it; B.n_it = c.n_it;
    B.d_ev = (const ovhip_dbf_edge *)p.at[B_EV]; B.n_ev = n.n_edge_v; B.d_eh = (const ovhip_dbf_edge *)p.at[B_EH]; B.n_eh = n.n_edge_h;
    j->st.n_tb += n.n_tb; j->st.n_mc += n.n_mc; j->st.n_mcx += n.n_mcx; j->st.n_aff += n.n_aff;
// ... 26 lines not shown
}

static int band_recon(ovhip_job *j, const ovhip_pic *dst, const ovhip_pic *refs, uint32_t n_refs, const ovhip_job_params *pr,
                      const BandCall &k, const Placement &p, Chain &c)
{
    ovhip_ctx *ctx = j->ctx;
    BandState *bs = j->bs;
    BandRec &B = bs->band[k.b];
    if (bs->stages & OVHIP_STAGE_MC) CHK(chain_predict(c, refs, refs, n_refs, nullptr, (int32_t *)p.at[B_MV]));
    if (!bs->ev_recon[k.b]) OV_HIP(ctx, hipEventCreateWithFlags(&bs->ev_recon[k.b], hipEventDisableTiming));
    int flow_workers = 0;
    if (k.n_items) {
        flow_workers = band_flow_take(ctx, flow_worker_count(ctx, pr->flow_workers, c.h_it, k.h_items, k.n_items, true));
        if (!flow_workers && !k.have_levels) return ov_fail(ctx, OVHIP_EUNSUP, "ovhip_job_band: flow budget exhausted and no level table", hipSuccess);
        B.flow_charge += flow_workers;
        c.n_items = flow_workers ? (uint32_t)k.n_items : 0;
    }
    const int r = band_recon_enqueue(j, dst, k, c, flow_workers);
    if (r != OVHIP_OK) {
        if (B.flow_charge) (void)hipEventRecord(bs->ev_recon[k.b], ctx->stream);
        return r;
    }
    bs->n = k.b + 1; bs->cur = k.c1; bs->row_prev = k.row_end;
    return OVHIP_OK;
}

static int band_tails(ovhip_job *j, const ovhip_pic *dst, const ovhip_job_params *pr, const BandCall &k, const Placement &p, const Chain &c)
{
    ovhip_ctx *ctx = j->ctx;
    BandState *bs = j->bs;
    const uint16_t *d_bwd = pr->lmcs && (bs->stages & OVHIP_STAGE_ITX) ? bs->d_bwd : nullptr;
    for (int t = k.t_first; t < k.t_end; ++t) {
        const BandRec &T = bs->band[t];
        if (T.row1 > T.row0) CHK(chain_unmap(j, dst, T.row0, T.row1, d_bwd, T.d_it, T.tagged == 1 ? T.n_it : 0u));
        if (bs->stages & OVHIP_STAGE_DBF) CHK(chain_deblock(c, T.d_ev, T.n_ev, T.d_eh, T.n_eh, &bs->offs));
    }
    if (k.t_end <= k.t_first) return OVHIP_OK;
    ovhip_alf_pic ap = bs->d_alf;
    ap.ctus = k.alf_on ? (const ovhip_alf_ctu *)(p.block + p.o_alf) - (size_t)k.alf_r0 * k.nb_ctu_w : nullptr;
    CHK(chain_filters(c, k.sao_on ? (const ovhip_sao_ctu *)(p.block + p.o_sao) - (size_t)k.sao_r0 * k.nb_ctu_w : nullptr, k.alf_on ? &ap : nullptr,
                      bs->sao_rows, k.sao_new, bs->alf_rows, k.alf_new));
    bs->dbf_rows = k.dbf_new; bs->sao_rows = k.sao_new; bs->alf_rows = k.alf_new;
    bs->rows_final = (k.sao_on || k.alf_on) ? k.alf_new : k.dbf_new;
    bs->tails = k.t_end;
    const int te = k.t_end - 1;
    bs->band[te].rows_final = bs->rows_final;
    if (!bs->ev_tail[te]) OV_HIP(ctx, hipEventCreateWithFlags(&bs->ev_tail[te], hipEventDisableTiming));
    OV_HIP(ctx, hipEventRecord(bs->ev_tail[te], ctx->stream));
    bs->last_event = (void *)bs->ev_tail[te]; bs->last_rows = bs->rows_final;
    return OVHIP_OK;
}

extern "C" int ovhip_job_band(ovhip_job *j, const ovhip_pic *dst, const ovhip_pic *refs, uint32_t n_refs, const ovhip_job_params *pr,
                   const ovhip_band_counts *upto, int32_t row_end, int32_t last)
{
    if (!j || !dst || !pr) return OVHIP_EINVAL;
    ovhip_ctx *ctx = j->ctx;
    OV_DEVICE(ctx);
    if (dst->w != j->w || dst->h != j->h) return ov_fail(ctx, OVHIP_EINVAL, "ovhip_job_band: picture size differs from the job's", hipSuccess);
    if (dst->stride_y != j->tmp.stride_y || dst->stride_c != j->tmp.stride_c)
        return ov_fail(ctx, OVHIP_EUNSUP, "ovhip_job_band: tight planes only (stride = width)", hipSuccess);
    if (!j->bs || !j->bs->active) CHK(ovhip_job_band_reserve(j));
    const int log2_ctu = switches_of(pr).log2_ctu;
    if (log2_ctu < 5 || log2_ctu > 7) return ov_fail(ctx, OVHIP_EINVAL, "ovhip_job_band: log2_ctu_s", hipSuccess);
    if (j->bs->closed) return ov_fail(ctx, OVHIP_EINVAL, "ovhip_job_band: the picture's last band was already submitted", hipSuccess);
    BandCall k = {};
    k.last = last; k.row_end = last || row_end > j->h ? j->h : row_end;
// ... 13 lines not shown
```

### openvvc_amd/csrc/ovvc_job.hip.h

```cpp
#pragma once
#include "ovvc_common.hip.h"
#include "flow_state.hip.h"
#include <stdlib.h>

struct BandState;

struct DevBuf { void *p; size_t cap; };

enum { B_TB, B_COEF, B_MC, B_MCX, B_MV, B_AFF, B_SIDE, B_REG, B_SCALE, B_EV, B_EH, B_PARAM, B_CLASS, B_CIIP, B_ITASK, B_ICTU, B_IITEM, B_TMVP, B_RPR, B_AFFR, B_COUNT };

struct ovhip_job {
    ovhip_ctx *ctx;
    ovhip_ctx *home;
    int32_t w, h;
    ovhip_recorder *rec;
    DevBuf dev[B_COUNT];
    ovhip_pic tmp;
    ovhip_pic res;
    uint32_t *d_sync; uint32_t epoch;
    uint32_t *d_flow;
    uint32_t *items_host; size_t items_cap;
    uint32_t *abort_host;
    char *param_host; size_t param_cap;
    int32_t *mv_host; size_t mv_cap;
    struct { int valid, has_intra; ovhip_pic dst, refs[16], intra; uint32_t n_refs; ovhip_job_params pr; } again;
    uint32_t n_retries;
    int flow_launched;
    int test_abort, test_abort_seen;
    ovhip_tmvp_cell *tmvp_host; size_t tmvp_cap, n_tmvp;
    size_t n_mv;
    size_t dmvr_first;
    size_t rows_end; int rows_pending;
    hipEvent_t ev_rows;
    hipEvent_t ev_h2d, ev_done;
    int flow_on_device;
    int flushed;
    const void *packed_prev[24];
    int resident;
    ovhip_job_stats st;
    struct BandState *bs;
    int t_stage;
    hipEvent_t t_ev[32][2]; uint8_t t_pending[32]; int t_next;
    double t_sum_ms; uint64_t t_count;
};

#define CHK(x) do { int r__ = (x); if (r__ != OVHIP_OK) return r__; } while (0)

struct Switches { uint32_t stages; int log2_ctu, sao_on, alf_on; };
static inline Switches switches_of(const ovhip_job_params *pr)
{
    const uint32_t stages = pr->stages ? pr->stages : UINT32_MAX;
    return Switches{ stages, pr->log2_ctu_s ? pr->log2_ctu_s : 7, pr->sao && (stages & OVHIP_STAGE_SAO), pr->alf_ctus && (stages & OVHIP_STAGE_ALF) };
}
static inline bool alf_tables_missing(const ovhip_job_params *pr)
{
    return !pr->alf_luma_coeff || !pr->alf_luma_clip || !pr->alf_chroma_coeff || !pr->alf_chroma_clip || !pr->alf_cc_coeff;
}

struct Layout {
    size_t o = 0;
    size_t put(size_t bytes) { const size_t at = o; o += (bytes + 255) & ~(size_t)255; return at; }
};

enum { T_LCOEF, T_LCLIP, T_CCOEF, T_CCLIP, T_CC, T_FWD, T_BWD, T_COUNT };
struct Tables { size_t at[T_COUNT]; };
static const size_t TABLE_BYTES[T_COUNT] = { 24 * OVHIP_ALF_LUMA_SET_SIZE * 2, 24 * OVHIP_ALF_LUMA_SET_SIZE * 2, 8 * 7 * 2, 8 * 7 * 2, 2 * 4 * 8 * 2, 2048, 2048 };

// ... 24 lines not shown
};

struct Chain {
    ovhip_job *j;
    ovhip_job *timer;
    const ovhip_pic *dst, *res;
    int log2_ctu;
    const ovhip_lmcs_luts *luts; const uint16_t *d_fwd; int16_t *d_scales;
    const ovhip_mc_unit *d_mc, *d_mcx; uint32_t n_mc, n_mcx;
    const ovhip_aff_unit *d_aff; uint32_t n_aff; const int32_t *d_side;
    const ovhip_rpr_unit *d_rpr; uint32_t n_rpr;
    const ovhip_aff_rpr_unit *d_affr; uint32_t n_affr;
    const ovhip_tb_cmd *d_tb; size_t cls[4], tiny[4][4]; const int16_t *d_coef;
    const ovhip_lmcs_region *d_reg; uint32_t reg0, n_reg;
    const ovhip_itask *d_it, *h_it; uint32_t n_it;
    const uint32_t *lv_start; uint32_t n_lv;
    const uint32_t *d_items; uint32_t n_items;
    int prepared;
    int ibc;
};

#pragma GCC visibility push(hidden)
void *pinned_alloc(void *user, size_t bytes);
void pinned_free(void *user, void *p);
int pinned_reserve(ovhip_job *j, void **p, size_t *cap, size_t bytes);
int dev_reserve(ovhip_job *j, int k, size_t bytes);
int state_words(ovhip_job *j, uint32_t **words, size_t n);
int ordered_arm(ovhip_job *j, uint32_t **words, size_t n);
int flow_widest(const ovhip_itask *sorted, const uint32_t *items, size_t n_items);
void chain_bind(Chain &c, const Placement &p, const ovhip_band_counts &first, const ovhip_band_counts &n, uint32_t n_rpr, uint32_t n_affr);
int chain_predict(const Chain &c, const ovhip_pic *refs_same, const ovhip_pic *refs, uint32_t n_refs, const ovhip_pic *intra, int32_t *d_mv);
int chain_residual(Chain &c, const uint16_t *d_bwd);
int chain_ordered(const Chain &c, int n_workers);
int chain_unmap(ovhip_job *j, const ovhip_pic *dst, int32_t row0, int32_t row1, const uint16_t *d_bwd, const ovhip_itask *d_it, uint32_t n_tagged);
int chain_deblock(const Chain &c, const ovhip_dbf_edge *d_ev, uint32_t n_ev, const ovhip_dbf_edge *d_eh, uint32_t n_eh, const ovhip_dbf_offsets *offs);
int chain_filters(const Chain &c, const ovhip_sao_ctu *d_sao, const ovhip_alf_pic *alf, int32_t s0, int32_t s1, int32_t a0, int32_t a1);
int flow_shift_of(int device);
int flow_worker_count(const ovhip_ctx *ctx, uint32_t asked, const ovhip_itask *sorted, const uint32_t *items, size_t n_items, bool in_band);
void flow_launch_abandoned(ovhip_job *j);
void flow_launch_clean(ovhip_job *j);
int band_flow_take(ovhip_ctx *ctx, int want);
void band_flow_give(ovhip_ctx *ctx, int n);
int band_flow_reclaim(ovhip_ctx *ctx, int *charge, hipEvent_t ev_recon, int wait);
void band_free(ovhip_job *j);
int band_reset(ovhip_job *j);
int band_active(const ovhip_job *j);
int band_wait_done(ovhip_job *j);
#pragma GCC visibility pop
```

### openvvc_amd/csrc/ovvc_picture.hip

```cpp
#include "ovvc_job.hip.h"

extern "C" int ovhip_dmvr_search_launch(ovhip_ctx *ctx, const ovhip_pic *geom, const ovhip_pic *refs, uint32_t n_refs,
                                        const ovhip_mc_unit *d_units, uint32_t n_units, int32_t *d_mv_out);

namespace {

static const ovhip_pic *same_size_refs(const ovhip_pic *geom, const ovhip_pic *refs, uint32_t n_refs, ovhip_pic *out)
{
    if (!refs || n_refs > 16) return refs;
    bool any = false;
    for (uint32_t i = 0; i < n_refs; ++i) {
        const bool same = refs[i].w == geom->w && refs[i].h == geom->h && refs[i].stride_y == geom->stride_y && refs[i].stride_c == geom->stride_c;
        out[i] = same ? refs[i] : *geom;
        any |= !same;
    }
    return any ? out : refs;
}

__global__ __launch_bounds__(256) void k_store_host(uint4 *__restrict__ dst, const uint4 *__restrict__ src, size_t n)
{
    const size_t i = (size_t)blockIdx.x * 256 + threadIdx.x;
    if (i < n) dst[i] = src[i];
}

int store_host(ovhip_ctx *ctx, void *dst_host, const void *src_dev, size_t bytes)
{
    const size_t n = (bytes + 15) / 16;
    if (!n) return OVHIP_OK;
    hipLaunchKernelGGL(k_store_host, dim3((unsigned)((n + 255) / 256)), dim3(256), 0, ctx->stream, (uint4 *)dst_host, (const uint4 *)src_dev, n);
    OV_LAUNCH_CHECK(ctx, "k_store_host");
    return OVHIP_OK;
}

double host_now_us()
{
    timespec t;
    clock_gettime(CLOCK_MONOTONIC, &t);
    return 1e6 * (double)t.tv_sec + 1e-3 * (double)t.tv_nsec;
}

int grow_trace() { static int on = -1; if (on < 0) on = getenv("OVVC_HIP_GROW_TRACE") != nullptr; return on; }

int h2d(ovhip_job *j, hipStream_t st, int k, const void *host, size_t bytes)
{
    if (!bytes) return OVHIP_OK;
    if (j->resident) return j->dev[k].cap >= bytes ? OVHIP_OK : ov_fail(j->ctx, OVHIP_EINVAL, "resident flush before a full one", hipSuccess);
    int r = dev_reserve(j, k, bytes);
    if (r) return r;
    OV_HIP(j->ctx, hipMemcpyAsync(j->dev[k].p, host, bytes, hipMemcpyHostToDevice, st));
    j->st.h2d_bytes += bytes; j->st.n_h2d++;
    return OVHIP_OK;
}

extern "C" const ovhip_tb_cmd *ovhip_rec_tb_cmds_split_tiny_(ovhip_recorder *r, size_t counts[4], size_t tiny[4][4], size_t *n);
extern "C" int ovhip_itx_launch_ex_(ovhip_ctx *ctx, const ovhip_pic *dst, const ovhip_pic *res, const ovhip_tb_cmd *d_cmds, uint32_t n_large,
                                    uint32_t n_small, const uint32_t tiny3[4], const int16_t *d_coefs, const int16_t *d_lmcs_scales, const uint16_t *d_bwd_lut);

extern "C" int ovhip_sao_launch_rows(ovhip_ctx *ctx, const ovhip_pic *dst, const ovhip_pic *src, const ovhip_sao_ctu *d_params, int32_t log2_ctu_s, int32_t row0, int32_t row1);
extern "C" int ovhip_alf_launch_rows(ovhip_ctx *ctx, const ovhip_pic *dst, const ovhip_pic *src, const ovhip_alf_pic *alf, int32_t row0, int32_t row1);

#ifndef OVHIP_PACK_LIMIT
#define OVHIP_PACK_LIMIT (1 << 20)
#endif

int t_collect(ovhip_job *j, int k)
{
    if (!j->t_pending[k]) return OVHIP_OK;
    float ms = 0.f;
    OV_HIP(j->ctx, hipEventSynchronize(j->t_ev[k][1]));
    OV_HIP(j->ctx, hipEventElapsedTime(&ms, j->t_ev[k][0], j->t_ev[k][1]));
    j->t_sum_ms += ms; j->t_count++;
    j->t_pending[k] = 0;
    return OVHIP_OK;
}

struct StageTimer {
    ovhip_job *j; int k;
    StageTimer(ovhip_job *job, int stage) : j(job), k(-1)
    {
        if (!j || j->t_stage != stage) return;
        k = j->t_next; j->t_next = (j->t_next + 1) % 32;
        if (t_collect(j, k) != OVHIP_OK || hipEventRecord(j->t_ev[k][0], j->ctx->stream) != hipSuccess) k = -1;
    }
    ~StageTimer()
    {
        if (k >= 0 && hipEventRecord(j->t_ev[k][1], j->ctx->stream) == hipSuccess) j->t_pending[k] = 1;
    }
};

int copy_rows(ovhip_ctx *ctx, const ovhip_pic *d, const ovhip_pic *s, int32_t r0, int32_t r1)
// ... 268 lines not shown
    if (d_bwd && c.cls[3]) {
        CHK(ovhip_itx_launch_ex_(ctx, c.dst, nullptr, d_tbc, (uint32_t)c.cls[2], (uint32_t)c.cls[3], t_chroma, c.d_coef, c.d_scales, d_bwd));
        j->st.n_launches++;
        return OVHIP_OK;
    }
    if (c.cls[2] + c.cls[3]) {
        CHK(ovhip_itx_launch_ex_(ctx, c.dst, c.res, d_tbc, (uint32_t)c.cls[2], (uint32_t)c.cls[3], t_chroma, c.d_coef, c.d_scales, nullptr));
        j->st.n_launches++;
    }
    if (d_bwd) { CHK(ovhip_lmcs_inverse_launch(ctx, c.dst, d_bwd)); j->st.n_launches++; }
    return OVHIP_OK;
}

int chain_ordered(const Chain &c, int n_workers)
{
    ovhip_job *j = c.j;
    if (c.n_items) {
        CHK(ovhip_intra_flow_launch(j->ctx, c.dst, c.res, c.d_it, c.n_it, c.d_items, c.n_items, c.d_reg, c.luts, c.d_scales, c.log2_ctu,
                                    j->d_flow, j->epoch, j->abort_host, (c.prepared ? 0 : 1) | (c.ibc ? OVHIP_FLOW_IBC : 0), n_workers));
        j->st.n_launches += 1 + !c.prepared;
        return OVHIP_OK;
    }
    for (uint32_t l = 0; l < c.n_lv; ++l) {
        const uint32_t a = c.lv_start[l], b = c.lv_start[l + 1];
        if (b > a) {
            CHK(ovhip_intra_level_launch(j->ctx, c.dst, c.res, c.d_it + a, b - a, c.d_reg, c.luts, c.d_scales, c.log2_ctu,
                                         ovhip_intra_level_geom(c.h_it + a, b - a)));
            j->st.n_launches++;
        }
    }
    return OVHIP_OK;
}

int chain_unmap(ovhip_job *j, const ovhip_pic *dst, int32_t row0, int32_t row1, const uint16_t *d_bwd, const ovhip_itask *d_it, uint32_t n_tagged)
{
    if (d_bwd) {
        ovhip_pic view = *dst;
        view.y = dst->y + (size_t)row0 * dst->stride_y; view.h = row1 - row0;
        CHK(ovhip_lmcs_inverse_untag_launch(j->ctx, &view, d_bwd, d_it, n_tagged));
    } else if (n_tagged) CHK(ovhip_intra_flow_untag_launch(j->ctx, dst, d_it, n_tagged, 1));
    else return OVHIP_OK;
    j->st.n_launches++;
    return OVHIP_OK;
}

int chain_deblock(const Chain &c, const ovhip_dbf_edge *d_ev, uint32_t n_ev, const ovhip_dbf_edge *d_eh, uint32_t n_eh, const ovhip_dbf_offsets *offs)
{
    StageTimer t_(c.timer, OVHIP_TIME_DBF);
    CHK(ovhip_dbf_launch_edges_ex(c.j->ctx, c.dst, d_ev, n_ev, d_eh, n_eh, offs));
    c.j->st.n_launches += (n_ev != 0) + (n_eh != 0);
    return OVHIP_OK;
}

int chain_filters(const Chain &c, const ovhip_sao_ctu *d_sao, const ovhip_alf_pic *alf, int32_t s0, int32_t s1, int32_t a0, int32_t a1)
{
    ovhip_job *j = c.j;
    if (s1 > s0) {
        if (d_sao) {
            StageTimer t_(c.timer, OVHIP_TIME_SAO);
            CHK(ovhip_sao_launch_rows(j->ctx, &j->tmp, c.dst, d_sao, c.log2_ctu, s0, s1));
            j->st.n_launches++;
        } else if (alf) CHK(copy_rows(j->ctx, &j->tmp, c.dst, s0, s1));
    }
    if (a1 > a0) {
        if (alf) {
            StageTimer t_(c.timer, OVHIP_TIME_ALF);
            CHK(ovhip_alf_launch_rows(j->ctx, c.dst, &j->tmp, alf, a0, a1));
            j->st.n_launches++;
        } else if (d_sao) CHK(copy_rows(j->ctx, c.dst, &j->tmp, a0, a1));
    }
    return OVHIP_OK;
}

namespace {

struct Gathered {
    Switches sw; size_t n_ctu;
    double t0;
    const ovhip_tb_cmd *tb; size_t cls[4], tiny[4][4];
    const int16_t *coef; const ovhip_mc_unit *mc, *mcx; const ovhip_aff_unit *aff; const int32_t *side; const ovhip_lmcs_region *reg;
    const ovhip_ciip_unit *ciip; const ovhip_rpr_unit *rpr; const ovhip_aff_rpr_unit *affr;
    const ovhip_itask *it; const ovhip_ictu *ictu; const uint32_t *lv_start; uint32_t n_lv;
    const ovhip_dbf_edge *ev, *eh; ovhip_dbf_offsets offs;
    ovhip_band_counts n;
    size_t n_ciip, n_rpr, n_affr, n_ictu;
    size_t n_items;
    bool ibc;
    int by_ctu; bool ordered, flow;
};

int flush_gather(ovhip_job *j, const ovhip_pic *dst, const ovhip_pic *intra, const ovhip_job_params *pr, Gathered &g)
{
    ovhip_ctx *ctx = j->ctx;
    if ((dst->w != j->w || dst->h != j->h)) return ov_fail(ctx, OVHIP_EINVAL, "ovhip_job_flush: picture size differs from the job's", hipSuccess);
    { const int64_t c_ = ovhip_job_dmvr_rows_collect(j); if (c_ < 0) return (int)c_; }
    g = Gathered{};
    g.sw = switches_of(pr);
    const uint32_t stages = g.sw.stages;
    const int log2_ctu = g.sw.log2_ctu;
    if (log2_ctu < 5 || log2_ctu > 7) return ov_fail(ctx, OVHIP_EINVAL, "ovhip_job_flush: log2_ctu_s", hipSuccess);
    g.n_ctu = (size_t)((j->w + (1 << log2_ctu) - 1) >> log2_ctu) * ((j->h + (1 << log2_ctu) - 1) >> log2_ctu);
    memset(&j->st, 0, sizeof(j->st));
    j->st.n_ordered_retries = j->n_retries;
    g.t0 = host_now_us();
    j->resident = (stages & OVHIP_STAGE_RESIDENT) && pr->stages;
    ovhip_recorder *rec = j->rec;

    size_t n_tb = 0, n_coef = 0, n_mc = 0, n_mcx = 0, n_aff = 0, n_side = 0, n_reg = 0, n_ev = 0, n_eh = 0;
    g.tb = ovhip_rec_tb_cmds_split_tiny_(rec, g.cls, g.tiny, &n_tb);
    if (!g.tb && n_tb) return ov_fail(ctx, OVHIP_ENOMEM, "ovhip_rec_tb_cmds_split", hipSuccess);
    g.coef = ovhip_rec_coefs(rec, &n_coef);
    g.mc = ovhip_rec_mc_units(rec, &n_mc);
    g.mcx = ovhip_rec_mcx_units(rec, &n_mcx);
    g.aff = ovhip_rec_aff_units(rec, &n_aff);
    g.side = ovhip_rec_aff_side(rec, &n_side);
    g.reg = ovhip_rec_lmcs_regions(rec, &n_reg);
    g.ciip = ovhip_rec_ciip_units(rec, &g.n_ciip);
    if (g.n_ciip && !intra)
        return ov_fail(ctx, OVHIP_EUNSUP, "ovhip_job_flush: CIIP blend units recorded but no picture with their intra prediction", hipSuccess);
    g.rpr = ovhip_rec_rpr_units(rec, &g.n_rpr);
    g.affr = ovhip_rec_aff_rpr_units(rec, &g.n_affr);
    size_t n_it = 0;
    const int want_ctu = pr->stages && (stages & OVHIP_STAGE_INTRA_CTU);
    g.ibc = ovhip_rec_ibc_tasks(rec) != 0;
    g.by_ctu = want_ctu && !g.ibc;
    int by_flow = !want_ctu && !(pr->stages && (stages & OVHIP_STAGE_INTRA_LEVELS));
    if (j->resident && by_flow && !j->flow_on_device) by_flow = 0;
    g.it = !g.by_ctu ? ovhip_rec_itasks_sorted(rec, &n_it, &g.lv_start, &g.n_lv)
                     : ovhip_rec_itasks_by_ctu(rec, log2_ctu, &n_it, &g.ictu, &g.n_ictu);
    if (by_flow && n_it) {
        g.n_items = ovhip_intra_flow_items_(g.it, n_it, j->items_host, j->items_cap / sizeof(uint32_t));
        if (g.n_items > j->items_cap / sizeof(uint32_t)) {
            CHK(pinned_reserve(j, (void **)&j->items_host, &j->items_cap, g.n_items * sizeof(uint32_t)));
            g.n_items = ovhip_intra_flow_items_(g.it, n_it, j->items_host, g.n_items);
        }
    }
    if (!g.it && ovhip_rec_itask_levels(rec)) return ov_fail(ctx, OVHIP_ENOMEM, "ovhip_job_flush: sorting the ordered tasks", hipSuccess);
    if (g.by_ctu) g.n_lv = ovhip_rec_itask_levels(rec);
    if (!(stages & OVHIP_STAGE_INTRA)) { n_it = 0; g.n_lv = 0; g.n_ictu = 0; }
    g.ordered = n_it != 0;
    g.flow = (stages & OVHIP_STAGE_INTRA) && g.n_items;
    if (g.ordered && !j->res.y) CHK(ovhip_pic_alloc(ctx, j->w, j->h, &j->res));
    if (g.ordered && (dst->stride_y != j->res.stride_y || dst->stride_c != j->res.stride_c))
        return ov_fail(ctx, OVHIP_EUNSUP, "ovhip_job_flush: pictures with ordered tasks need tight planes (stride = width)", hipSuccess);
    g.ev = ovhip_rec_dbf_edges(rec, 0, &n_ev, &g.offs);
    g.eh = ovhip_rec_dbf_edges(rec, 1, &n_eh, nullptr);
    g.n = ovhip_band_counts{ (uint32_t)n_tb, (uint32_t)n_coef, (uint32_t)n_mc, (uint32_t)n_mcx, (uint32_t)n_aff, (uint32_t)n_side, (uint32_t)n_reg,
                             (uint32_t)n_it, (uint32_t)n_ev, (uint32_t)n_eh };
    j->st.n_itasks = g.n.n_itask; j->st.n_ilevels = g.n_lv;
    j->st.n_tb = g.n.n_tb; j->st.n_mc = g.n.n_mc; j->st.n_mcx = g.n.n_mcx; j->st.n_aff = g.n.n_aff;
    j->st.n_edges_v = g.n.n_edge_v; j->st.n_edges_h = g.n.n_edge_h; j->st.n_regions = g.n.n_reg;
    if (g.sw.alf_on && alf_tables_missing(pr)) return ov_fail(ctx, OVHIP_EINVAL, "ovhip_job_flush: ALF tables missing", hipSuccess);
    return OVHIP_OK;
}

struct Small { const void *host; size_t bytes; int buf; size_t at; };

int stage_uploads(ovhip_job *j, hipStream_t ust, const Gathered &g, size_t block_bytes, const Small *small, size_t n_small, const void **packed)
{
    StageTimer t_(j, OVHIP_TIME_H2D);
    CHK(h2d(j, ust, B_PARAM, j->param_host, block_bytes));
    if (g.n.n_mcx) {
        CHK(dev_reserve(j, B_MV, (size_t)g.n.n_mcx * 16));
        CHK(pinned_reserve(j, (void **)&j->mv_host, &j->mv_cap, (size_t)g.n.n_mcx * 16));
    }
    if (g.n.n_reg) CHK(dev_reserve(j, B_SCALE, (size_t)g.n.n_reg * 2));
    for (size_t i = 0; i < n_small && !j->resident; ++i) {
        const Small &sm = small[i];
// ... 72 lines not shown
    const bool mv_direct = n_mcx && !pr->tmvp_cells && !j->resident;
    ovhip_pic same[16];
    CHK(chain_predict(c, same_size_refs(c.dst, refs, n_refs, same), refs, n_refs, intra, mv_direct ? j->mv_host : (int32_t *)p.at[B_MV]));
    if (mv_direct) j->st.d2h_bytes += n_mcx * 16;
    else if (n_mcx && !j->resident) {
        CHK(store_host(j->ctx, j->mv_host, p.at[B_MV], n_mcx * 16));
        j->st.d2h_bytes += n_mcx * 16;
    }
    j->n_mv = n_mcx;
    j->n_tmvp = 0;
    if (n_mcx && pr->tmvp_cells) {
        const size_t bytes = 4 * n_mcx * sizeof(ovhip_tmvp_cell);
        CHK(dev_reserve(j, B_TMVP, bytes));
        CHK(pinned_reserve(j, (void **)&j->tmvp_host, &j->tmvp_cap, bytes));
        CHK(tmvp_cells(j, c.d_mcx, (const int32_t *)p.at[B_MV], 0, n_mcx, c.log2_ctu));
        j->st.n_launches++; j->st.d2h_bytes += bytes;
    }
    if (g.n_ciip) { CHK(ovhip_ciip_launch(j->ctx, c.dst, intra, (const ovhip_ciip_unit *)p.at[B_CIIP], (uint32_t)g.n_ciip)); j->st.n_launches++; }
    return OVHIP_OK;
}

int flush_launch(ovhip_job *j, const ovhip_pic *dst, const ovhip_pic *refs, uint32_t n_refs, const ovhip_pic *intra, const ovhip_job_params *pr,
                 const Gathered &g, const Placement &p)
{
    ovhip_ctx *ctx = j->ctx;
    const uint32_t stages = g.sw.stages;
    const uint16_t *d_bwd = pr->lmcs ? (const uint16_t *)(p.block + p.tabs.at[T_BWD]) : nullptr;
    Chain c = {};
    c.j = j; c.timer = j; c.dst = dst; c.res = g.ordered ? &j->res : nullptr; c.log2_ctu = g.sw.log2_ctu;
    c.luts = pr->lmcs; c.d_fwd = pr->lmcs ? (const uint16_t *)(p.block + p.tabs.at[T_FWD]) : nullptr; c.d_scales = (int16_t *)j->dev[B_SCALE].p;
    chain_bind(c, p, ovhip_band_counts{}, g.n, (uint32_t)g.n_rpr, (uint32_t)g.n_affr);
    memcpy(c.cls, g.cls, sizeof(c.cls)); memcpy(c.tiny, g.tiny, sizeof(c.tiny));
    c.h_it = g.it; c.lv_start = g.lv_start; c.n_lv = g.n_lv; c.n_items = g.flow ? (uint32_t)g.n_items : 0; c.ibc = g.ibc;

    if (stages & OVHIP_STAGE_MC) CHK(launch_predict(j, c, refs, n_refs, intra, pr, g, p));
    if (g.flow) {
        CHK(ordered_arm(j, &j->d_flow, ovhip_intra_flow_words(j->w, j->h)));
        if (j->test_abort && j->n_retries == 0) {
            j->test_abort = 0; j->test_abort_seen = 1;
            OV_HIP(ctx, hipMemsetAsync(j->d_flow, 0xff, sizeof(uint32_t), ctx->stream));
            *(volatile uint32_t *)j->abort_host = 1;
        }
    }
    if (stages & OVHIP_STAGE_ITX) CHK(chain_residual(c, g.ordered ? nullptr : d_bwd));
    if (g.ordered) {
        StageTimer t_(j, OVHIP_TIME_INTRA);
        if (g.by_ctu) {
            CHK(ordered_arm(j, &j->d_sync, ovhip_intra_sync_words(j->w, j->h, 5)));
            CHK(ovhip_intra_ctu_launch(ctx, dst, &j->res, c.d_it, (const ovhip_ictu *)p.at[B_ICTU], (uint32_t)g.n_ictu, c.d_reg, pr->lmcs, c.d_scales,
                                       c.log2_ctu, j->d_sync, j->epoch, j->abort_host));
            j->st.n_launches++;
        } else {
            CHK(chain_ordered(c, g.flow ? flow_worker_count(ctx, pr->flow_workers, g.it, j->items_host, g.n_items, false) : 0));
            if (g.flow) { j->flow_launched = 1; j->st.flow_shift = (uint32_t)flow_shift_of(ctx->device); }
        }
        CHK(chain_unmap(j, dst, 0, j->h, (pr->lmcs && (stages & OVHIP_STAGE_ITX)) ? d_bwd : nullptr, c.d_it, c.n_items ? c.n_it : 0u));
    }
    if (stages & OVHIP_STAGE_DBF)
        CHK(chain_deblock(c, (const ovhip_dbf_edge *)p.at[B_EV], g.n.n_edge_v, (const ovhip_dbf_edge *)p.at[B_EH], g.n.n_edge_h, &g.offs));
    ovhip_alf_pic ap;
    if (g.sw.alf_on) {
        CHK(dev_reserve(j, B_CLASS, (size_t)((j->w + 3) / 4) * ((j->h + 3) / 4)));
        ap = alf_pic_at(p.block, p.tabs, (const ovhip_alf_ctu *)(p.block + p.o_alf), (uint8_t *)j->dev[B_CLASS].p, c.log2_ctu);
    }
    CHK(chain_filters(c, g.sw.sao_on ? (const ovhip_sao_ctu *)(p.block + p.o_sao) : nullptr, g.sw.alf_on ? &ap : nullptr, 0, j->h, 0, j->h));
    OV_HIP(ctx, hipEventRecord(j->ev_done, ctx->stream));
    return OVHIP_OK;
}

}

extern "C" {

int ovhip_job_create(ovhip_ctx *ctx, int32_t w, int32_t h, ovhip_job **out)
{
    if (!ctx || !out || w <= 0 || h <= 0 || (w & 1) || (h & 1)) return OVHIP_EINVAL;
    OV_DEVICE(ctx);
    *out = nullptr;
    ovhip_job *j = (ovhip_job *)calloc(1, sizeof(*j));
    if (!j) return OVHIP_ENOMEM;
    j->ctx = ctx; j->home = ctx; j->w = w; j->h = h; j->t_stage = -1;
    const ovhip_allocator al = { pinned_alloc, pinned_free, nullptr };
    j->rec = ovhip_rec_create_ex(w, h, &al);
    if (!j->rec) { free(j); return OVHIP_ENOMEM; }
    ovhip_rec_set_dense_dbf_planes(j->rec, 0);
    int r = ovhip_pic_alloc(ctx, w, h, &j->tmp);
    if (r == OVHIP_OK && hipEventCreateWithFlags(&j->ev_h2d, hipEventDisableTiming) != hipSuccess) r = OVHIP_ENODEV;
    if (r == OVHIP_OK && hipEventCreateWithFlags(&j->ev_done, hipEventDisableTiming) != hipSuccess) r = OVHIP_ENODEV;
    if (r == OVHIP_OK && hipEventCreateWithFlags(&j->ev_rows, hipEventDisableTiming) != hipSuccess) r = OVHIP_ENODEV;
// ... 209 lines not shown
    else if (log2_ctu_s) {
        CHK(pinned_reserve(j, (void **)&j->tmvp_host, &j->tmvp_cap, 4 * n * sizeof(ovhip_tmvp_cell)));
        for (size_t i = 4 * first; i < 4 * n; ++i) { j->tmvp_host[i] = ovhip_tmvp_cell{}; j->tmvp_host[i].cell = OVHIP_TMVP_NONE; }
        j->n_tmvp = 4 * n;
    }
    j->dmvr_first = n;
    j->rows_end = n;
    return (int64_t)n;
}

int64_t ovhip_job_dmvr_rows(ovhip_job *j, const ovhip_pic *refs, uint32_t n_refs)
{
    const int64_t n = ovhip_job_dmvr_rows_begin(j, refs, n_refs, 0);
    return n < 0 ? n : ovhip_job_dmvr_rows_collect(j);
}

int ovhip_job_flush(ovhip_job *j, const ovhip_pic *dst, const ovhip_pic *refs, uint32_t n_refs, const ovhip_pic *intra,
                    const ovhip_job_params *pr)
{
    if (!j || !dst || !pr) return OVHIP_EINVAL;
    j->again.valid = 0;
    j->n_retries = 0;
    const int r = job_flush_impl(j, dst, refs, n_refs, intra, pr);
    j->again.valid = r == OVHIP_OK && n_refs <= 16;
    j->again.dst = *dst;
    for (uint32_t i = 0; i < n_refs && i < 16; ++i) j->again.refs[i] = refs[i];
    j->again.n_refs = n_refs;
    j->again.has_intra = intra != nullptr;
    if (intra) j->again.intra = *intra;
    j->again.pr = *pr;
    return r;
}

int ovhip_job_test_abort_next_flow(ovhip_job *j)
{
    if (!j) return OVHIP_EINVAL;
    j->test_abort = 1;
    return OVHIP_OK;
}

static int job_flush_impl(ovhip_job *j, const ovhip_pic *dst, const ovhip_pic *refs, uint32_t n_refs, const ovhip_pic *intra,
                          const ovhip_job_params *pr)
{
    OV_DEVICE(j->ctx);
    Gathered g;
    Placement p;
    CHK(flush_gather(j, dst, intra, pr, g));
    CHK(flush_stage(j, pr, g, p));
    const double t3 = host_now_us();
    CHK(flush_launch(j, dst, refs, n_refs, intra, pr, g, p));
    j->st.host_us_launch = (uint32_t)(host_now_us() - t3);
    return OVHIP_OK;
}

}
```

### openvvc_amd/csrc/ovvc_record_intra.c

```c
#include <stdlib.h>
#include <string.h>
#include "ovvc_hip.h"
#include "ovvc_record_priv.h"

static int
maps_ready(ovhip_recorder *r)
{
    const int w4 = (r->pic_w + 3) >> 2, h4 = (r->pic_h + 3) >> 2;
    if (!r->lvl_y) {
        r->lvl_y = (uint16_t *)calloc((size_t)w4 * h4, 2);
        r->lvl_c = (uint16_t *)calloc((size_t)w4 * h4, 2);
        if (!r->lvl_y || !r->lvl_c) return -1;
        r->lvl_w4 = w4; r->lvl_h4 = h4; r->lvl_dirty = 0;
    }
    if (r->lvl_dirty) {
        memset(r->lvl_y, 0, (size_t)w4 * h4 * 2); memset(r->lvl_c, 0, (size_t)w4 * h4 * 2);
        r->lvl_dirty = 0;
    }
    return 0;
}

int
ovhip_rec_intra_reset_(ovhip_recorder *r)
{
    r->n_itask = 0; r->n_ibc = 0; r->n_ilevels = 0; r->max_ilevel = 0;
    if (r->lvl_y) r->lvl_dirty = 1;
    return 0;
}

void
ovhip_rec_intra_free_(ovhip_recorder *r)
{
    free(r->lvl_y); free(r->lvl_c); free(r->reg_level);
    r->lvl_y = r->lvl_c = NULL; r->reg_level = NULL;
}

static int
max_level(ovhip_recorder *r, const uint16_t *map, int ux0, int uy0, int nx, int ny)
{
    int m = 0;
    int x1 = ux0 + nx, y1 = uy0 + ny;
    const int sh = r->log2_ctu - 2;
    if (ux0 < 0) ux0 = 0;
    if (uy0 < 0) uy0 = 0;
    if (x1 > r->lvl_w4) x1 = r->lvl_w4;
    if (y1 > r->lvl_h4) y1 = r->lvl_h4;
    for (int y = uy0; y < y1; ++y)
        for (int x = ux0; x < x1; ++x) {
            const int l = map[y * r->lvl_w4 + x];
            if (!l) continue;
            if (l > m) m = l;
            const int dx = (x >> sh) - r->scan_cx, dy = (y >> sh) - r->scan_cy;
            if (dx | dy) {
                if (dy == 0 && dx == -1) r->scan_deps |= 1;
                else if (dy == -1 && dx == -1) r->scan_deps |= 2;
                else if (dy == -1 && dx == 0) r->scan_deps |= 4;
                else if (dy == -1 && dx == 1) r->scan_deps |= 8;
                else r->scan_deps |= 0x10;
            }
        }
    return m;
}

static void
scan_begin(ovhip_recorder *r, int luma_x, int luma_y)
{
    r->scan_cx = luma_x >> r->log2_ctu; r->scan_cy = luma_y >> r->log2_ctu; r->scan_deps = 0;
}

static void
set_level(ovhip_recorder *r, uint16_t *map, int ux0, int uy0, int nx, int ny, int level)
{
    int x1 = ux0 + nx, y1 = uy0 + ny;
    if (x1 > r->lvl_w4) x1 = r->lvl_w4;
    if (y1 > r->lvl_h4) y1 = r->lvl_h4;
    for (int y = uy0; y < y1; ++y)
        for (int x = ux0; x < x1; ++x) map[y * r->lvl_w4 + x] = (uint16_t)level;
}

uint16_t
ovhip_rec_region_level_(ovhip_recorder *r, int32_t x0, int32_t y0, int n_abv, int n_lft)
{
    r->region_deps = 0;
    if (!r->n_itask || maps_ready(r)) return 0;
    const int ux = x0 >> 2, uy = y0 >> 2;
    int m = 0, k;
    scan_begin(r, x0, y0);
    if (n_abv && (k = max_level(r, r->lvl_y, ux, uy - 1, n_abv, 1)) > m) m = k;
    if (n_lft && (k = max_level(r, r->lvl_y, ux - 1, uy, 1, n_lft)) > m) m = k;
    r->region_deps = r->scan_deps;
    return (uint16_t)(m ? m + 1 : 0);
}

int
ovhip_rec_itask_add_(ovhip_recorder *r, const ovhip_itask *in, uint16_t extra_level)
{
    if (maps_ready(r)) return OVHIP_ENOMEM;
    if (r->n_itask + 1 > r->cap_itask && ovhip_rec_grow_(r, (void **)&r->itask, &r->cap_itask, r->n_itask + 1, sizeof(ovhip_itask))) return OVHIP_ENOMEM;
    ovhip_itask t = *in;
    const int w = 1 << t.log2_w, h = 1 << t.log2_h;
    int m = extra_level, k;
    const int cs = t.kind == OVHIP_IT_CHROMA || t.kind == OVHIP_IT_RES_C || t.kind == OVHIP_IT_IBC_C;
    scan_begin(r, t.x << cs, t.y << cs);
    if (t.kind == OVHIP_IT_REGION) r->scan_deps = r->region_deps;
    if (t.kind == OVHIP_IT_LUMA) {
        const int ux = t.x >> 2, uy = t.y >> 2, nx = (w + 3) >> 2, ny = (h + 3) >> 2;
        const int isp = !!(t.flags & OVHIP_IF_ISP);
        const int uxa = isp ? (t.x - t.isp_off_x) >> 2 : ux, uyl = isp ? (t.y - t.isp_off_y) >> 2 : uy;
        if ((t.flags & OVHIP_IF_CORNER) && (k = max_level(r, r->lvl_y, uxa - 1, uy - 1, 1, 1)) > m) m = k;
        if (t.avl_abv && (k = max_level(r, r->lvl_y, uxa, uy - 1, t.avl_abv, 1)) > m) m = k;
        if (t.avl_lft && (k = max_level(r, r->lvl_y, ux - 1, uyl, 1, t.avl_lft)) > m) m = k;
        if (t.ciip_wt && (k = max_level(r, r->lvl_y, ux, uy, nx, ny)) > m) m = k;
        if (m >= 65534) return OVHIP_EUNSUP;
        t.level = (uint16_t)(m + 1);
        set_level(r, r->lvl_y, ux, uy, nx, ny, t.level);
    } else if (t.kind == OVHIP_IT_CHROMA || t.kind == OVHIP_IT_RES_C) {
        const int ux = t.x >> 1, uy = t.y >> 1, nx = (w + 1) >> 1, ny = (h + 1) >> 1;
        if (t.kind == OVHIP_IT_CHROMA) {
            if (t.mode >= 67) {
                const int ext = w < h ? w : h;
                const int na = (w + ext + 1) >> 1, nl = (h + ext + 1) >> 1;
                if ((k = max_level(r, r->lvl_y, ux, uy, nx, ny)) > m) m = k;
                if (t.avl_abv) { if ((k = max_level(r, r->lvl_y, ux - 1, uy - 1, na + 1, 1)) > m) m = k; if ((k = max_level(r, r->lvl_c, ux, uy - 1, na, 1)) > m) m = k; }
                if (t.avl_lft) { if ((k = max_level(r, r->lvl_y, ux - 1, uy - 1, 1, nl + 1)) > m) m = k; if ((k = max_level(r, r->lvl_c, ux - 1, uy, 1, nl)) > m) m = k; }
            } else {
                if ((t.flags & OVHIP_IF_CORNER) && (k = max_level(r, r->lvl_c, ux - 1, uy - 1, 1, 1)) > m) m = k;
                if (t.avl_abv && (k = max_level(r, r->lvl_c, ux, uy - 1, t.avl_abv, 1)) > m) m = k;
                if (t.avl_lft && (k = max_level(r, r->lvl_c, ux - 1, uy, 1, t.avl_lft)) > m) m = k;
            }
        }
        if ((t.kind == OVHIP_IT_RES_C || t.ciip_wt) && (k = max_level(r, r->lvl_c, ux, uy, nx, ny)) > m) m = k;
        if (m >= 65534) return OVHIP_EUNSUP;
        t.level = (uint16_t)(m + 1);
        set_level(r, r->lvl_c, ux, uy, nx, ny, t.level);
    } else if (t.kind == OVHIP_IT_IBC_L || t.kind == OVHIP_IT_IBC_C) {
        const int sh = cs ? 1 : 2, rnd = (1 << sh) - 1;
        uint16_t *map = cs ? r->lvl_c : r->lvl_y;
        const int sx = t.x + OVHIP_ITASK_IBC_DX(t), sy = t.y + OVHIP_ITASK_IBC_DY(t);
        if (sx < 0 || sy < 0) return OVHIP_EINVAL;
        const int ux0 = sx >> sh, uy0 = sy >> sh, ux1 = (sx + w - 1) >> sh, uy1 = (sy + h - 1) >> sh;
        k = max_level(r, map, ux0, uy0, ux1 - ux0 + 1, uy1 - uy0 + 1);
        if (!k) t.flags |= OVHIP_IF_IBC_FREE;
        if (k > m) m = k;
        if (m >= 65534) return OVHIP_EUNSUP;
        t.level = (uint16_t)(m + 1);
        set_level(r, map, t.x >> sh, t.y >> sh, (w + rnd) >> sh, (h + rnd) >> sh, t.level);
        ++r->n_ibc;
    } else if (t.kind == OVHIP_IT_REGION) {
        if (m >= 65534) return OVHIP_EUNSUP;
        t.level = (uint16_t)(m + 1);
    } else {
        return OVHIP_EINVAL;
    }
    t.ctu_deps = (uint16_t)(0x8000u | ((unsigned)r->log2_ctu << 8) | (r->scan_deps & 0x1f));
    r->itask[r->n_itask] = t;
    if (t.level > r->max_ilevel) r->max_ilevel = t.level;
    return (int)r->n_itask++;
}

size_t ovhip_rec_ibc_tasks(const ovhip_recorder *r) { return r ? r->n_ibc : 0; }

int
ovhip_rec_set_ctu_size(ovhip_recorder *r, int32_t log2_ctu_s)
{
    if (!r || log2_ctu_s < 5 || log2_ctu_s > 7) return OVHIP_EINVAL;
    if (r->log) ovhip_calllog_ctu_size_(r->log, log2_ctu_s);
    r->log2_ctu = log2_ctu_s;
    return OVHIP_OK;
}

uint32_t
ovhip_rec_itask_levels(const ovhip_recorder *r)
{
    if (!r) return 0;
    uint32_t m = r->max_ilevel;
    if (!m) for (size_t i = 0; i < r->n_itask; ++i) if (r->itask[i].level > m) m = r->itask[i].level;
    return m;
}

const ovhip_itask *
ovhip_rec_itasks(const ovhip_recorder *r, size_t *n)
{
    if (!r || !n) return NULL;
    *n = r->n_itask;
    return r->itask;
}

const ovhip_itask *
ovhip_rec_itasks_sorted(ovhip_recorder *r, size_t *n, const uint32_t **level_start, uint32_t *n_levels)
{
    if (!r || !n || !level_start || !n_levels) return NULL;
    *n = r->n_itask; *n_levels = 0; *level_start = NULL;
    if (!r->n_itask) return r->itask;
    uint32_t maxl = 0;
    for (size_t i = 0; i < r->n_itask; ++i) if (r->itask[i].level > maxl) maxl = r->itask[i].level;
    if (ovhip_rec_grow_(r, (void **)&r->itask_sorted, &r->cap_isorted, r->n_itask, sizeof(ovhip_itask))) { *n = 0; return NULL; }
    {
        if (r->cap_ilevel < (size_t)(maxl + 2) * 2) {
            uint32_t *q = (uint32_t *)realloc(r->ilevel_start, (size_t)(maxl + 2) * 2 * sizeof(uint32_t));
            if (!q) { *n = 0; return NULL; }
            r->ilevel_start = q; r->cap_ilevel = (size_t)(maxl + 2) * 2;
        }
    }
    uint32_t *start = r->ilevel_start;
    memset(start, 0, (maxl + 2) * sizeof(uint32_t));
    for (size_t i = 0; i < r->n_itask; ++i) start[r->itask[i].level]++;
    uint32_t acc = 0;
    for (uint32_t l = 1; l <= maxl; ++l) { const uint32_t c = start[l]; start[l] = acc; acc += c; }
    start[maxl + 1] = acc;
    uint32_t *fill = start + maxl + 2;
    memcpy(fill, start, (maxl + 2) * sizeof(uint32_t));
    for (size_t i = 0; i < r->n_itask; ++i) r->itask_sorted[fill[r->itask[i].level]++] = r->itask[i];
    r->n_ilevels = maxl;
    *n_levels = maxl;
    *level_start = start + 1;
    return r->itask_sorted;
}

int
ovhip_rec_itasks_sorted_range_(const ovhip_recorder *r, size_t first, size_t n, ovhip_itask *out, uint32_t *level_start, size_t cap, uint32_t *n_levels)
{
    *n_levels = 0;
    if (!n) return 0;
    const ovhip_itask *t = r->itask + first;
    uint32_t minl = 0xffffffffu, maxl = 0;
    for (size_t i = 0; i < n; ++i) { if (t[i].level < minl) minl = t[i].level; if (t[i].level > maxl) maxl = t[i].level; }
    const size_t span = (size_t)(maxl - minl) + 1;
    uint32_t *cnt = (uint32_t *)calloc(span + 1, sizeof(uint32_t));
    if (!cnt) return -1;
    for (size_t i = 0; i < n; ++i) cnt[t[i].level - minl]++;
    uint32_t acc = 0, nl = 0;
    int fits = 1;
    for (size_t l = 0; l < span; ++l) {
        const uint32_t c = cnt[l];
        cnt[l] = acc;
        if (c) { if (nl < cap) level_start[nl] = acc; else fits = 0; ++nl; }
        acc += c;
    }
    if (nl < cap) level_start[nl] = acc; else fits = 0;
    for (size_t i = 0; i < n; ++i) out[cnt[t[i].level - minl]++] = t[i];
    free(cnt);
    *n_levels = nl;
    return fits ? 0 : -1;
}

const ovhip_itask *
ovhip_rec_itasks_by_ctu(ovhip_recorder *r, int32_t log2_ctu_s, size_t *n, const ovhip_ictu **ctus, size_t *n_ctus)
{
    if (!r || !n || !ctus || !n_ctus || log2_ctu_s < 5 || log2_ctu_s > 7) return NULL;
    *n = 0; *ctus = NULL; *n_ctus = 0;
    if (!r->n_itask) return r->itask;
    const uint32_t *lv; uint32_t nlv; size_t nt;
    const ovhip_itask *sorted = ovhip_rec_itasks_sorted(r, &nt, &lv, &nlv);
    if (!sorted) return NULL;
    const int ncx = (r->pic_w + (1 << log2_ctu_s) - 1) >> log2_ctu_s, ncy = (r->pic_h + (1 << log2_ctu_s) - 1) >> log2_ctu_s;
    const size_t nctu = (size_t)ncx * ncy;
    if (r->cap_ctu_count < 2 * nctu + 1) {
        uint32_t *q = (uint32_t *)realloc(r->ctu_count, (2 * nctu + 1) * sizeof(uint32_t));
        if (!q) return NULL;
        r->ctu_count = q; r->cap_ctu_count = 2 * nctu + 1;
    }
    if (ovhip_rec_grow_(r, (void **)&r->itask_ctu, &r->cap_itask_ctu, nt, sizeof(ovhip_itask))) return NULL;
    uint32_t *start = r->ctu_count, *fill = r->ctu_count + nctu + 1;
    memset(start, 0, (nctu + 1) * sizeof(uint32_t));
#define CHROMA_OF(t) ((t).kind == OVHIP_IT_CHROMA || (t).kind == OVHIP_IT_RES_C || (t).kind == OVHIP_IT_IBC_C)
#define CTU_OF(t) ((size_t)((CHROMA_OF(t) ? (t).y * 2 : (t).y) >> log2_ctu_s) * ncx + ((CHROMA_OF(t) ? (t).x * 2 : (t).x) >> log2_ctu_s))
    size_t used = 0;
    int precise = 1;
    for (size_t i = 0; i < nt; ++i) {
        const size_t c = CTU_OF(sorted[i]);
        if (c >= nctu) return NULL;
        if (!start[c]++) ++used;
        const unsigned d = sorted[i].ctu_deps;
// ... 36 lines not shown
```

### openvvc_amd/csrc/ovvc_record_priv.h

```cpp
#ifndef OVVC_RECORD_PRIV_H
#define OVVC_RECORD_PRIV_H
#include <stddef.h>
#include "ovvc_hip.h"

struct ovhip_recorder {
    int32_t pic_w, pic_h;
    ovhip_allocator al; int has_al;
    ovhip_tb_cmd  *tb;    size_t n_tb,   cap_tb;
    int16_t       *coef;  size_t n_coef, cap_coef;
    ovhip_mc_unit *mc;    size_t n_mc,   cap_mc;
    ovhip_mc_unit *mcx;   size_t n_mcx,  cap_mcx;
    ovhip_aff_unit *aff;  size_t n_aff,  cap_aff;
    int32_t *aff_side;    size_t n_side, cap_side;
    ovhip_lmcs_region *reg; size_t n_reg, cap_reg;
    ovhip_ciip_unit *ciip; size_t n_ciip, cap_ciip;
    ovhip_tb_cmd *tb_split; size_t cap_split;
    uint16_t *dbf_luma_v, *dbf_luma_h, *dbf_cb_v, *dbf_cr_v, *dbf_cb_h, *dbf_cr_h;
    int32_t dbf_w4, dbf_h4;
    int16_t dbf_beta_offset, dbf_tc_offset;
    int dense_planes;
    ovhip_dbf_edge *edge_v, *edge_h; size_t n_edge_v, cap_edge_v, n_edge_h, cap_edge_h;
    ovhip_dbf_offsets dbf_off; int n_dbf_off;
    ovhip_itask *itask; size_t n_itask, cap_itask;
    size_t n_ibc;
    ovhip_itask *itask_sorted; size_t cap_isorted;
    uint32_t *ilevel_start; size_t cap_ilevel; uint32_t n_ilevels, max_ilevel;
    ovhip_itask *itask_ctu; size_t cap_itask_ctu;
    ovhip_ictu *ictu; size_t cap_ictu;
    uint32_t *ctu_count; size_t cap_ctu_count;
    uint16_t *lvl_y, *lvl_c;
    int32_t lvl_w4, lvl_h4; int lvl_dirty;
    int log2_ctu;
    int scan_cx, scan_cy; uint32_t scan_deps, region_deps;
    uint16_t *reg_level; size_t cap_reglvl;
    ovhip_calllog *log;
    ovhip_ref_scale ref_scale[256]; uint32_t n_scaled;
    ovhip_rpr_unit *rpr; size_t n_rpr, cap_rpr;
    ovhip_aff_rpr_unit *affr; size_t n_affr, cap_affr;
    uint32_t rpr_tools;
    const char *refusal;
};

void ovhip_calllog_tu_(ovhip_calllog *l, const ovhip_tu_state *st, const ovhip_tu_desc *tu, const ovhip_itask *il, const ovhip_itask *ic);
void ovhip_calllog_tu_ibc_(ovhip_calllog *l, const ovhip_tu_state *st, const ovhip_tu_desc *tu, const ovhip_ibc_desc *cu);
void ovhip_calllog_isp_(ovhip_calllog *l, const ovhip_tu_state *st, const ovhip_isp_desc *cu);
void ovhip_calllog_pu_(ovhip_calllog *l, const ovhip_pu_desc *pu);
void ovhip_calllog_affine_(ovhip_calllog *l, const ovhip_affine_desc *cu);
void ovhip_calllog_region_(ovhip_calllog *l, int32_t x0, int32_t y0, uint32_t abv, uint32_t lft);
void ovhip_calllog_dbf_(ovhip_calllog *l, const ovhip_dbf_ctu *c);
void ovhip_calllog_ciip_(ovhip_calllog *l, int32_t x0, int32_t y0, int32_t log2_w, int32_t log2_h, int32_t mode_abv, int32_t mode_lft);
void ovhip_calllog_ctu_size_(ovhip_calllog *l, int32_t log2_ctu_s);
void ovhip_calllog_ref_scale_(ovhip_calllog *l, int32_t slot, const ovhip_ref_scale *sc);
void ovhip_calllog_rpr_tools_(ovhip_calllog *l, uint32_t mask);

int  ovhip_rec_intra_reset_(ovhip_recorder *r);
void ovhip_rec_rpr_reset_(ovhip_recorder *r);
void ovhip_rec_intra_free_(ovhip_recorder *r);
int  ovhip_rec_itask_add_(ovhip_recorder *r, const ovhip_itask *t, uint16_t extra_level);
uint16_t ovhip_rec_region_level_(ovhip_recorder *r, int32_t x0, int32_t y0, int n_abv, int n_lft);

int  ovhip_rec_grow_(ovhip_recorder *r, void **p, size_t *cap, size_t need, size_t elem);
#define grow(p, cap, need, elem) ((need) <= *(cap) ? 0 : ovhip_rec_grow_(r, p, cap, need, elem))
void ovhip_rec_free_(ovhip_recorder *r, void *p);

// ... 7 lines not shown
```

### openvvc_amd/engine.py

```python
from __future__ import annotations

import ctypes as C

import numpy as np

from . import capi


class EngineError(RuntimeError):
    pass


class Context:
    def __init__(self, device: int = 0, stream: int | None = None):
        self.lib = capi.load()
        h = C.c_void_p()
        r = self.lib.ovhip_ctx_create(C.byref(h), device, C.c_void_p(stream) if stream else None)
        if r != 0:
            raise EngineError(f"ovhip_ctx_create(device={device}) failed: {r} (no HIP device? the engine has no CPU fallback)")
        self.h = h
        self._bufs = []

    def _chk(self, r, what):
        if r != 0:
# ... 403 lines not shown
        for p in self.refs + [self.dst, self.tmp] + ([self.intra] if self.intra else []):
            p.free()


class Job:

    def __init__(self, ctx: Context, w: int, h: int):
        self.ctx, self.lib, self.w, self.h = ctx, ctx.lib, w, h
        j = C.c_void_p()
        ctx._chk(self.lib.ovhip_job_create(ctx.h, w, h, C.byref(j)), "job_create")
        self.j = j
        self.rec = capi.Recorder.__new__(capi.Recorder)
        self.rec.lib, self.rec.h, self.rec._keep = self.lib, self.lib.ovhip_job_recorder(j), []
        self._keep = {}

    def close(self):
        if self.j:
            self.rec.h = None
            self.lib.ovhip_job_destroy(self.j)
            self.j = None

    def begin(self):
        self.ctx._chk(self.lib.ovhip_job_begin(self.j), "job_begin")

    def load_workload(self, wl):
        self.begin()
        r = self.rec
        for which, arr in ((capi.REC_COEF, wl.coefs), (capi.REC_TB, wl.tb_cmds), (capi.REC_MC, wl.mc_units),
                           (capi.REC_MCX, wl.mcx_units), (capi.REC_AFF, wl.aff_units), (capi.REC_SIDE, wl.aff_side),
                           (capi.REC_REGION, wl.lmcs_regions), (capi.REC_CIIP, wl.ciip_units), (capi.REC_ITASK, wl.itasks),
                           (capi.REC_EDGE_V, wl.dbf_edges[0]), (capi.REC_EDGE_H, wl.dbf_edges[1])):
            if arr is not None and len(arr):
                r.append_raw(which, arr)
        offs = capi.DbfOffsets()
        for i in range(8):
            offs.beta[i], offs.tc[i] = wl.dbf_planes["beta_offset"], wl.dbf_planes["tc_offset"]
        self.ctx._chk(self.lib.ovhip_rec_set_dbf_offsets(r.h, C.byref(offs), 1), "set_dbf_offsets")
        self.params = self.make_params(wl)

    def make_params(self, wl, log2_ctu: int = 7, stages: int = 0) -> "capi.JobParams":
        keep = self._keep
        keep["sao"] = np.ascontiguousarray(wl.sao_params)
        keep["alf"] = {k: np.ascontiguousarray(wl.alf[k], dtype=dt) for k, dt in capi.ALF_TABLES}
        keep["lmcs"] = wl.lmcs
        a = keep["alf"]
        p = capi.JobParams()
        p.lmcs = C.addressof(wl.lmcs) if wl.lmcs is not None else None
        p.sao = keep["sao"].ctypes.data
        p.alf_ctus = a["ctus"].ctypes.data
        p.alf_luma_coeff, p.alf_luma_clip = a["luma_coeff"].ctypes.data, a["luma_clip"].ctypes.data
        p.alf_chroma_coeff, p.alf_chroma_clip = a["chroma_coeff"].ctypes.data, a["chroma_clip"].ctypes.data
        p.alf_cc_coeff = a["cc_coeff"].ctypes.data
        p.log2_ctu_s, p.stages = log2_ctu, stages
        return p

    def flush(self, dst: "DevPic", refs: list, intra: "DevPic | None" = None, params=None):
        arr = (capi.Pic * max(len(refs), 1))(*[r.s for r in refs])
        self.ctx._chk(self.lib.ovhip_job_flush(self.j, C.byref(dst.s), arr, len(refs), C.byref(intra.s) if intra else None,
                                               C.byref(params if params is not None else self.params)), "job_flush")

    def wait(self):
        self.ctx._chk(self.lib.ovhip_job_wait(self.j), "job_wait")

    def band(self, dst: "DevPic", refs: list, row_end: int, last: bool = False, upto: "capi.BandCounts | None" = None, params=None):
        arr = (capi.Pic * max(len(refs), 1))(*[r.s for r in refs])
        self.ctx._chk(self.lib.ovhip_job_band(self.j, C.byref(dst.s), arr, len(refs), C.byref(params if params is not None else self.params),
# ... 21 lines not shown
        if n < 0:
            self.ctx._chk(int(n), "job_dmvr_rows")
        return int(n)

    def dmvr_rows_begin(self, refs: list, log2_ctu: int = 0) -> int:
        arr = (capi.Pic * max(len(refs), 1))(*[r.s for r in refs])
        n = self.lib.ovhip_job_dmvr_rows_begin(self.j, arr, len(refs), log2_ctu)
        if n < 0:
            self.ctx._chk(int(n), "job_dmvr_rows_begin")
        return int(n)

    def dmvr_rows_collect(self) -> int:
        n = self.lib.ovhip_job_dmvr_rows_collect(self.j)
        if n < 0:
            self.ctx._chk(int(n), "job_dmvr_rows_collect")
        return int(n)

    def refined_mvs(self) -> np.ndarray:
        n = C.c_size_t()
        p = self.lib.ovhip_job_refined_mvs(self.j, C.byref(n))
        if not n.value:
            return np.zeros((0, 4), np.int32)
        return np.frombuffer((C.c_int32 * (4 * n.value)).from_address(p), dtype=np.int32).reshape(-1, 4).copy()

    def tmvp_cells(self) -> np.ndarray:
        n = C.c_size_t()
        p = self.lib.ovhip_job_tmvp_cells(self.j, C.byref(n))
        if not n.value:
            return np.zeros(0, capi.TMVP_CELL_DTYPE)
        return np.ctypeslib.as_array(C.cast(p, C.POINTER(C.c_uint8)), (n.value * capi.TMVP_CELL_DTYPE.itemsize,)).view(capi.TMVP_CELL_DTYPE).copy()

    def test_abort_next_flow(self):
        self.ctx._chk(self.lib.ovhip_job_test_abort_next_flow(self.j), "job_test_abort_next_flow")

    def stats(self) -> "capi.JobStats":
        s = capi.JobStats()
        self.lib.ovhip_job_last_stats(self.j, C.byref(s))
        return s

    def time_stage(self, name: "str | None"):
        self.ctx._chk(self.lib.ovhip_job_time_stage(self.j, capi.TIME_STAGES.index(name) if name else -1), "job_time_stage")

    def stage_time(self):
        s, n = C.c_double(), C.c_uint64()
        self.ctx._chk(self.lib.ovhip_job_stage_time(self.j, C.byref(s), C.byref(n)), "job_stage_time")
        return s.value * 1e-3, n.value


def band_counts(wl, rows, log2_ctu: int = 7) -> list:
    def cut(ctu_row, what):
        ctu_row = np.asarray(ctu_row, np.int64)
        if len(ctu_row) > 1 and (np.diff(ctu_row) < 0).any():
            raise EngineError(f"band_counts: {what} are not in CTU-row order")
        return [int(np.searchsorted(ctu_row, r >> log2_ctu, side="left")) for r in rows]

    def arr(a, dt):
        return np.zeros(0, dt) if a is None or not len(a) else np.asarray(a).view(dt).reshape(-1)

    tb, mc, mcx = arr(wl.tb_cmds, capi.TB_CMD_DTYPE), arr(wl.mc_units, capi.MC_UNIT_DTYPE), arr(wl.mcx_units, capi.MC_UNIT_DTYPE)
    aff, reg, it = arr(wl.aff_units, capi.AFF_UNIT_DTYPE), arr(wl.lmcs_regions, capi.LMCS_REGION_DTYPE), arr(wl.itasks, capi.ITASK_DTYPE)
    ev, eh = arr(wl.dbf_edges[0], capi.DBF_EDGE_DTYPE), arr(wl.dbf_edges[1], capi.DBF_EDGE_DTYPE)
    n_coef = 0 if wl.coefs is None else len(wl.coefs)
    n_side = 0 if wl.aff_side is None else len(wl.aff_side)
    tb_row = (tb["y"].astype(np.int64) << (tb["plane"] != 0)) >> log2_ctu
    it_chroma = (it["kind"] == capi.IT_CHROMA) | (it["kind"] == capi.IT_RES_C)
    it_row = (it["y"].astype(np.int64) << it_chroma) >> log2_ctu
# ... 240 lines not shown
```

### openvvc_amd/synth.py

```python
from __future__ import annotations

import ctypes as C
from dataclasses import dataclass, field

import numpy as np

LM_FRAC = 0.35
ISP_FRAC = 0.08

from . import capi

DEFAULT_SEED = 0x266


def smooth_plane(rs: np.random.RandomState, h: int, w: int) -> np.ndarray:
    gh, gw = h // 16 + 2, w // 16 + 2
    g = rs.randint(64, 960, size=(gh, gw)).astype(np.float32)
    yy = np.linspace(0, gh - 1.001, h, dtype=np.float32)
    xx = np.linspace(0, gw - 1.001, w, dtype=np.float32)
    y0 = yy.astype(np.int32); x0 = xx.astype(np.int32)
    fy = (yy - y0)[:, None]; fx = (xx - x0)[None, :]
    a = g[y0][:, x0]; b = g[y0][:, x0 + 1]; c = g[y0 + 1][:, x0]; d = g[y0 + 1][:, x0 + 1]
    p = (a * (1 - fx) + b * fx) * (1 - fy) + (c * (1 - fx) + d * fx) * fy
    p += rs.randint(-12, 13, size=(h, w))
# ... 36 lines not shown

    for cy in range(0, pic_h, ctu):
        for cx in range(0, pic_w, ctu):
            rec(cx, cy, ctu, ctu)
    return np.array(out, dtype=np.int32)


@dataclass
class Workload:
    w: int
    h: int
    seed: int
    refs: list
    ref_pocs: list
    cus: np.ndarray
    mc_units: np.ndarray
    tb_cmds: np.ndarray
    coefs: np.ndarray
    n_luma_cmds: int = 0
    tb_classes: tuple = (0, 0, 0, 0)
    mcx_units: np.ndarray = None
    aff_units: np.ndarray = None
    aff_side: np.ndarray = None
    ciip_units: np.ndarray = None
    intra: tuple = None
    lmcs: "capi.LmcsLuts" = None
    lmcs_regions: np.ndarray = None
    dbf_ctus: np.ndarray = None
    dbf_planes: dict = None
    dbf_edges: list = None
    sao_params: np.ndarray = None
    alf: dict = None
    itasks: np.ndarray = None
    calllog: np.ndarray = None
    stats: dict = field(default_factory=dict)

    @property
    def frame_bytes(self) -> int:
        return self.w * self.h * 3

    @property
    def lmcs_fwd(self):
        return None if self.lmcs is None else np.frombuffer(bytes(self.lmcs), np.uint16)[:1024].copy()

    @property
    def lmcs_bwd(self):
        return None if self.lmcs is None else np.frombuffer(bytes(self.lmcs), np.uint16)[1024:2048].copy()


def _coef_values(rs, n):
    mag = np.minimum(rs.geometric(0.35, size=n), 600).astype(np.int32)
    big = rs.random_sample(n) < 0.01
    mag = np.where(big, rs.randint(100, 4000, size=n), mag)
    sign = np.where(rs.random_sample(n) < 0.5, -1, 1)
    return (mag * sign).astype(np.int16)


def _lmcs_tables(rs) -> "capi.LmcsLuts":
    d = capi.LmcsData()
    d.min_bin_idx, d.delta_max_bin_idx = 1, 1
    d.crs_offset = int(rs.randint(-3, 4))
    for i in range(16):
        d.cw_delta[i] = int(rs.randint(-14, 15))
    return capi.lmcs_build(d)


# ... 316 lines not shown
                        else:
                            lx = min(nx, 1 + int(rs.geometric(0.55))); ly = min(ny, 1 + int(rs.geometric(0.55)))
                            m = 0
                            for sy in range(ly):
                                for sx in range(lx):
                                    if (sx or sy) and rs.random_sample() < 0.35:
                                        continue
                                    m |= 1 << (sy * 8 + sx)
                                    o = sy * 4 * cw + sx * 16
                                    dens = 0.7 if (sx == 0 and sy == 0) else 0.3
                                    vals = coef_pool[pool_pos:pool_pos + 16].copy(); pool_pos += 16
                                    vals[rs.random_sample(16) > dens] = 0
                                    buf[o:o + 16] = vals
                            if buf[0] == 0:
                                buf[0] = 1
                            td.sig_sb_map[comp] = m; td.last_pos[comp] = 0x0101
                        pool_pos %= (len(coef_pool) - 4096)
                    td.coef[comp] = buf.ctypes.data
                if task_l is not None or task_c is not None:
                    rec.tu_intra(st, td, task_l, task_c)
                else:
                    rec.tu(st, td)
                n_tu += 1
        done[y >> 2:(y + (1 << l2h)) >> 2, x >> 2:(x + (1 << l2w)) >> 2] = True

    cmds, classes = rec.tb_cmds_split()
    n_luma = classes[0] + classes[1]
    wl = Workload(w, h, seed, refs, pocs, cus, rec.mc_units(), cmds, rec.coefs(), n_luma_cmds=n_luma, tb_classes=classes)
    wl.mcx_units, wl.aff_units, wl.aff_side, wl.ciip_units = rec.mcx_units(), rec.aff_units(), rec.aff_side(), rec.ciip_units()
    if (len(wl.ciip_units) or (mode == CIIP).any()) and not dev_intra:
        wl.intra = random_picture(rs, w, h)
    if dev_intra:
        wl.itasks = rec.itasks()
    if lmcs_on:
        wl.lmcs = _lmcs_tables(rs)
        wl.lmcs_regions = rec.lmcs_regions()
    wl.dbf_ctus = make_dbf_ctus(rs, w, h, cus)
    wl.dbf_planes, wl.dbf_edges = record_dbf(rec, wl.dbf_ctus)
    if calllog:
        wl.calllog = rec.take_calllog()
    wl.sao_params = make_sao_params(rs, w, h)
    wl.alf = make_alf(rs, w, h)
    u, ux, ua = wl.mc_units, wl.mcx_units, wl.aff_units
    area = lambda a: a["w"].astype(np.int64) * a["h"]
    nref = lambda a: np.where(a["dir"] == 3, 2, 1)
    tot = area(u).sum() + area(ux).sum() + area(ua).sum()
    wl.stats = {
        "n_cu": int(n), "n_tu": int(n_tu), "n_isp_cus": int(n_isp), "n_mc_units": int(len(u)), "n_mcx_units": int(len(ux)),
        "n_aff_units": int(len(ua)), "n_ciip_units": int(len(wl.ciip_units)), "n_tb_cmds": int(len(wl.tb_cmds)),
        "n_luma_cmds": int(n_luma), "n_lmcs_regions": 0 if wl.lmcs_regions is None else int(len(wl.lmcs_regions)),
        "cu_modes": {k: int((mode == v).sum()) for k, v in (("plain", PLAIN), ("bdof", BDOF), ("dmvr", DMVR), ("affine", AFFINE), ("gpm", GPM), ("ciip", CIIP))
                     + ((("intra", INTRA),) if dev_intra else ())},
        "n_itasks": 0 if wl.itasks is None else int(len(wl.itasks)),
        "n_ilevels": 0 if wl.itasks is None or not len(wl.itasks) else int(wl.itasks["level"].max()),
        "coef_bytes": int(wl.coefs.nbytes),
        "cmd_bytes": int(u.nbytes + ux.nbytes + ua.nbytes + wl.aff_side.nbytes + wl.tb_cmds.nbytes),
        "r_bar": float(((area(u) * nref(u)).sum() + 2 * area(ux).sum() + (area(ua) * nref(ua)).sum()) / max(1, tot)),
    }
    rec.close()
    return wl


def _pack_bits(win):
    sh = np.arange(win.shape[0], dtype=np.uint64)[:, None]
    return (win.astype(np.uint64) << sh).sum(axis=0, dtype=np.uint64)

# ... 115 lines not shown
```

Before: 3632.

## Defer unreferenced chroma residual-only intra tasks into the LMCS inverse untag pass

The recorder now tracks which chroma residual-only intra tasks are never read by later intra prediction. Such tasks are flagged DEFER, dropped from the ordered intra flow, and their residual add is applied inside the LMCS inverse kernel's chroma untag blocks. Flow item generation also skips disabled Cb/Cr components. This is meant to shorten the serialized intra flow and its sync overhead, in exchange for extra host-side dependency bookkeeping and residual reads in the LMCS kernel.

```diff
diff --git a/include/ovvc_hip.h b/include/ovvc_hip.h
--- a/include/ovvc_hip.h
+++ b/include/ovvc_hip.h
@@ -307,6 +307,7 @@
     OVHIP_IF_SCALE_IDX = 512,
     OVHIP_IF_IBC_FREE = 4096,
     OVHIP_IF_CORNER_L = 2048,
+    OVHIP_IF_DEFER = 8192,
     OVHIP_IF_ISP = 1024
 };
 typedef struct ovhip_itask {
@@ -459,6 +460,8 @@
                          int32_t *n_pred);
 const ovhip_itask *ovhip_rec_itasks(const ovhip_recorder *rec, size_t *n);
 const ovhip_itask *ovhip_rec_itasks_sorted(ovhip_recorder *rec, size_t *n, const uint32_t **level_start, uint32_t *n_levels);
+size_t ovhip_rec_itask_deferrable(const ovhip_recorder *rec, uint8_t *marks, size_t cap);
+int    ovhip_rec_set_itask_deferrable(ovhip_recorder *rec, const uint8_t *marks, size_t n);
 typedef struct ovhip_ictu {
     uint16_t cx, cy;
     uint32_t first, n;
@@ -888,6 +891,7 @@
 int  ovhip_stream_set_output_scale(ovhip_stream *s, int32_t out_w, int32_t out_h, const ovhip_scale_info *info);
 const void *ovhip_stream_key(const ovhip_stream *s, uint32_t idx);
 int  ovhip_job_test_abort_next_flow(ovhip_job *job);
+int  ovhip_job_flow_counts(const ovhip_job *job, uint32_t *n_items, uint32_t *n_deferred);
 
 #ifdef __cplusplus
 }
diff --git a/openvvc_amd/capi.py b/openvvc_amd/capi.py
--- a/openvvc_amd/capi.py
+++ b/openvvc_amd/capi.py
@@ -572,6 +572,9 @@
         "ovhip_host_alloc": (vp, [C.c_size_t]),
         "ovhip_host_free": (None, [vp]),
         "ovhip_job_test_abort_next_flow": (C.c_int, [vp]),
+        "ovhip_job_flow_counts": (C.c_int, [vp, P(C.c_uint32), P(C.c_uint32)]),
+        "ovhip_rec_itask_deferrable": (C.c_size_t, [vp, vp, C.c_size_t]),
+        "ovhip_rec_set_itask_deferrable": (C.c_int, [vp, vp, C.c_size_t]),
         "ovhip_dpb_create": (C.c_int, [P(vp), P(C.c_int), C.c_int]),
         "ovhip_dpb_create_ex": (C.c_int, [P(vp), C.c_int, P(DpbOps)]),
         "ovhip_dpb_destroy": (None, [vp]),
@@ -678,6 +681,7 @@
     "ovhip_output_scale_check", "ovhip_output_scale_launch", "ovhip_pic_output_scaled", "ovhip_pic_digest_scaled",
     "ovhip_frame_set_output_scale", "ovhip_stream_set_output_scale", "ovhip_ctx_scratch_bytes",
     "ovhip_rec_ibc_check", "ovhip_rec_tu_ibc", "ovhip_rec_ibc_tasks",
+    "ovhip_job_flow_counts", "ovhip_rec_itask_deferrable", "ovhip_rec_set_itask_deferrable",
 ]
 
 
@@ -778,6 +782,20 @@
 
     def itasks(self) -> np.ndarray:
         return self._arr(self.lib.ovhip_rec_itasks, ITASK_DTYPE)
+
+    def itask_deferrable(self) -> "np.ndarray | None":
+        n = self.lib.ovhip_rec_itask_deferrable(self.h, None, 0)
+        if not n:
+            return None
+        m = np.zeros(n, np.uint8)
+        self.lib.ovhip_rec_itask_deferrable(self.h, m.ctypes.data, n)
+        return m
+
+    def set_itask_deferrable(self, marks: np.ndarray):
+        m = np.ascontiguousarray(marks, np.uint8)
+        r = self.lib.ovhip_rec_set_itask_deferrable(self.h, m.ctypes.data, len(m))
+        if r != 0:
+            raise ValueError(f"ovhip_rec_set_itask_deferrable -> {r}")
 
     def itasks_sorted(self):
         n, nl, ls = C.c_size_t(), C.c_uint32(), C.POINTER(C.c_uint32)()
diff --git a/openvvc_amd/csrc/flow_state.hip.h b/openvvc_amd/csrc/flow_state.hip.h
--- a/openvvc_amd/csrc/flow_state.hip.h
+++ b/openvvc_amd/csrc/flow_state.hip.h
@@ -2,6 +2,7 @@
 #include <hip/hip_runtime.h>
 #include <stdint.h>
 #include "ovvc_hip.h"
+#include "ovvc_common.hip.h"
 
 #define OVHIP_FLOW_SYNC_WORDS 16
 struct FlowState { unsigned *y, *c[2], *reg; int w4; };
@@ -34,11 +35,20 @@
     return it;
 }
 
-extern "C" size_t ovhip_intra_flow_items_(const ovhip_itask *sorted, size_t n, uint32_t *items, size_t cap);
+extern "C" size_t ovhip_intra_flow_items_(const ovhip_itask *sorted, size_t n, uint32_t *items, size_t cap, size_t *n_deferred);
+
+__device__ __forceinline__ int res_scale(int v, int scale)
+{
+    const int sign = v & (1 << 15);
+    int a = (ov_clip_bd(abs(v)) * scale + (1 << 10)) >> 11;
+    return ov_clip3(sign ? -a : a, -(1 << 15), 1 << 15);
+}
+__device__ __forceinline__ int res_add_clip(int v, int res, bool scaled, int scale) { return ov_clip_bd(v + (scaled ? res_scale(res, scale) : res)); }
 
 __device__ __forceinline__ void flow_prepare_task(const ovhip_itask &t, const FlowState &fs, unsigned epoch, int lane16)
 {
     const unsigned mark = 2 * epoch;
+    if (t.flags & OVHIP_IF_DEFER) return;
     if (t.kind == OVHIP_IT_REGION) { if (lane16 == 0) fs.reg[t.c_scale] = mark; return; }
     const bool luma = t.kind == OVHIP_IT_LUMA || t.kind == OVHIP_IT_IBC_L;
     const bool both = t.kind == OVHIP_IT_CHROMA || t.kind == OVHIP_IT_IBC_C;
diff --git a/openvvc_amd/csrc/kernels_intra.hip b/openvvc_amd/csrc/kernels_intra.hip
--- a/openvvc_amd/csrc/kernels_intra.hip
+++ b/openvvc_amd/csrc/kernels_intra.hip
@@ -146,12 +146,6 @@
     }
 }
 
-__device__ __forceinline__ int res_scale(int v, int scale)
-{
-    const int sign = v & (1 << 15);
-    int a = (ov_clip_bd(abs(v)) * scale + (1 << 10)) >> 11;
-    return ov_clip3(sign ? -a : a, -(1 << 15), 1 << 15);
-}
 
 __device__ void pred_regular(IntraLds &s, const ovhip_itask &t, bool is_luma, const Strip st, int lane)
 {
@@ -517,7 +511,7 @@
         if (p >= it.p1) break;
         int v = it.res_only ? dv[i] : s.pred[p - it.p0];
         if (it.ciip_wt) v = (v * it.ciip_wt + dv[i] * (4 - it.ciip_wt) + 2) >> 2;
-        if (it.has_res) v = ov_clip_bd(v + (it.scaled ? res_scale(rv[i], scale) : rv[i]));
+        if (it.has_res) v = res_add_clip(v, rv[i], it.scaled, scale);
         dst[y * dstride + x] = (uint16_t)v;
     }
 }
@@ -872,7 +866,7 @@
     if (ti >= n) return;
     const ovhip_itask t = tasks[ti];
     const bool luma = t.kind == OVHIP_IT_LUMA || t.kind == OVHIP_IT_IBC_L;
-    if (t.kind == OVHIP_IT_REGION || (luma && !with_luma)) return;
+    if (t.kind == OVHIP_IT_REGION || (luma && !with_luma) || (t.flags & OVHIP_IF_DEFER)) return;
     const int lane = threadIdx.x & 15;
     const int l2w = t.log2_w, w = 1 << l2w, npx = w << t.log2_h;
     const int stride = luma ? pic.stride_y : pic.stride_c;
@@ -973,8 +967,8 @@
             }
             if (it.ciip_wt) for (int e = 0; e < G; ++e) v[e] = (v[e] * it.ciip_wt + dv[e] * (4 - it.ciip_wt) + 2) >> 2;
             if (it.has_res) {
-                if (it.scaled) for (int e = 0; e < G; ++e) v[e] = ov_clip_bd(v[e] + res_scale(rv[e], scale));
-                else           for (int e = 0; e < G; ++e) v[e] = ov_clip_bd(v[e] + rv[e]);
+                if (it.scaled) for (int e = 0; e < G; ++e) v[e] = res_add_clip(v[e], rv[e], true, scale);
+                else           for (int e = 0; e < G; ++e) v[e] = res_add_clip(v[e], rv[e], false, 0);
             }
 #pragma unroll
             for (int e = 0; e < R::DW; ++e) out[e] = ((uint32_t)v[2 * e] | (G > 1 ? (uint32_t)v[G > 1 ? 2 * e + 1 : 0] << 16 : 0u)) | tag2;
@@ -1012,7 +1006,6 @@
     const bool ibc = IBC && t.kind >= OVHIP_IT_IBC_L;
     const unsigned pending = 2 * epoch;
     const int w4 = fs.w4;
-    if (it.skip()) continue;
 
     uint16_t *pl = luma ? pic.y : (comp ? pic.cr : pic.cb);
     const int dstride = luma ? pic.stride_y : pic.stride_c, rstride = luma ? res.stride_y : res.stride_c;
@@ -1223,24 +1216,29 @@
     return OVHIP_OK;
 }
 
-extern "C" size_t ovhip_intra_flow_items_(const ovhip_itask *sorted, size_t n, uint32_t *items, size_t cap)
-{
-    size_t k = 0;
+extern "C" size_t ovhip_intra_flow_items_(const ovhip_itask *sorted, size_t n, uint32_t *items, size_t cap, size_t *n_deferred)
+{
+    size_t k = 0, nd = 0;
+    if (n_deferred) *n_deferred = 0;
     for (size_t i = 0; sorted && i < n; ++i) {
         const ovhip_itask &t = sorted[i];
         if (i >= FLOW_ITEM_MAX_TASKS) return 0;
+        if (n_deferred && (t.flags & OVHIP_IF_DEFER)) { ++nd; continue; }
         if (t.kind == OVHIP_IT_REGION) { if (k < cap) items[k] = flow_item_pack((uint32_t)i, 0, 0); ++k; continue; }
         const int npx = 1 << (t.log2_w + t.log2_h), strips = (npx + FSTRIP - 1) / FSTRIP, comps = (t.kind == OVHIP_IT_LUMA || t.kind == OVHIP_IT_IBC_L) ? 1 : 2;
         if (strips > FLOW_ITEM_MAX_STRIPS) return 0;
+        const unsigned on[2] = { t.kind != OVHIP_IT_RES_C || (t.flags & OVHIP_IF_RES_CB), t.kind != OVHIP_IT_RES_C || (t.flags & OVHIP_IF_RES_CR) };
         for (int st = 0; st < strips; ++st)
-            for (int c = 0; c < comps; ++c) { if (k < cap) items[k] = flow_item_pack((uint32_t)i, st, c); ++k; }
-    }
+            for (int c = 0; c < comps; ++c) { if (!on[c]) continue; if (k < cap) items[k] = flow_item_pack((uint32_t)i, st, c); ++k; }
+    }
+    if (n_deferred) *n_deferred = nd;
     return k;
 }
 
 extern "C" size_t ovhip_intra_flow_items(const ovhip_itask *sorted, size_t n, uint32_t *items, size_t cap)
 {
-    const size_t k = ovhip_intra_flow_items_(sorted, n, items, cap);
+    size_t nd;
+    const size_t k = ovhip_intra_flow_items_(sorted, n, items, cap, &nd);
     return k <= cap ? k : 0;
 }
 
diff --git a/openvvc_amd/csrc/kernels_lmcs.hip b/openvvc_amd/csrc/kernels_lmcs.hip
--- a/openvvc_amd/csrc/kernels_lmcs.hip
+++ b/openvvc_amd/csrc/kernels_lmcs.hip
@@ -35,7 +35,15 @@
 typedef uint32_t lm_u2 __attribute__((ext_vector_type(2), aligned(4)));
 
 #define UNTAG_TASKS_PER_WG 4
-__device__ __forceinline__ void untag_chroma_tasks(const ovhip_pic &pic, const ovhip_itask *__restrict__ tasks, uint32_t n, uint32_t wg)
+__device__ __forceinline__ uint32_t deferred_add2(uint32_t old2, uint32_t res2, bool scaled, int scale)
+{
+    const int a = res_add_clip((int)(old2 & 0xffff), (int)(int16_t)(res2 & 0xffff), scaled, scale);
+    const int b = res_add_clip((int)(old2 >> 16), (int)(int16_t)(res2 >> 16), scaled, scale);
+    return (uint32_t)a | ((uint32_t)b << 16);
+}
+
+__device__ __forceinline__ void untag_chroma_tasks(const ovhip_pic &pic, const ovhip_pic &res, const int16_t *__restrict__ scales,
+                                                   const ovhip_itask *__restrict__ tasks, uint32_t n, uint32_t wg)
 {
     const uint32_t ti = wg * UNTAG_TASKS_PER_WG + (threadIdx.x >> 6);
     if (ti >= n) return;
@@ -46,7 +54,22 @@
     const bool res_only = t.kind == OVHIP_IT_RES_C;
     const bool on0 = !res_only || (t.flags & OVHIP_IF_RES_CB), on1 = !res_only || (t.flags & OVHIP_IF_RES_CR);
     uint16_t *const d0 = pic.cb + t.y * stride + t.x, *const d1 = pic.cr + t.y * stride + t.x;
-    if (w >= 4) {
+    const bool defer = res_only && (t.flags & OVHIP_IF_DEFER);
+    if (defer && !res.cb) return;
+    const bool scaled = t.flags & OVHIP_IF_RES_SCALE;
+    const int scale = (defer && scaled) ? ((t.flags & OVHIP_IF_SCALE_IDX) ? (int)scales[t.c_scale] : (int)t.c_scale) : 0;
+    const int rstride = res.stride_c;
+    const int16_t *const r0 = reinterpret_cast<const int16_t *>(res.cb) + t.y * rstride + t.x, *const r1 = reinterpret_cast<const int16_t *>(res.cr) + t.y * rstride + t.x;
+    if (w >= 4 && defer) {
+        for (int p = 4 * lane; p < npx; p += 256) {
+            const int o = (p >> l2w) * stride + (p & (w - 1)), ro = (p >> l2w) * rstride + (p & (w - 1));
+            lm_u2 v0 = 0, v1 = 0, q0 = 0, q1 = 0;
+            if (on0) { v0 = *reinterpret_cast<const lm_u2 *>(d0 + o); q0 = *reinterpret_cast<const lm_u2 *>(r0 + ro); }
+            if (on1) { v1 = *reinterpret_cast<const lm_u2 *>(d1 + o); q1 = *reinterpret_cast<const lm_u2 *>(r1 + ro); }
+            if (on0) { v0[0] = deferred_add2(v0[0], q0[0], scaled, scale); v0[1] = deferred_add2(v0[1], q0[1], scaled, scale); *reinterpret_cast<lm_u2 *>(d0 + o) = v0; }
+            if (on1) { v1[0] = deferred_add2(v1[0], q1[0], scaled, scale); v1[1] = deferred_add2(v1[1], q1[1], scaled, scale); *reinterpret_cast<lm_u2 *>(d1 + o) = v1; }
+        }
+    } else if (w >= 4) {
         for (int base = 0; base < npx; base += 1024) {
             lm_u2 v0[4], v1[4];
 #pragma unroll
@@ -66,27 +89,30 @@
         }
     } else if (w == 2) {
         for (int p = 2 * lane; p < npx; p += 128) {
-            const int o = (p >> l2w) * stride + (p & (w - 1));
-            uint32_t a = 0, b = 0;
+            const int o = (p >> l2w) * stride + (p & (w - 1)), ro = (p >> l2w) * rstride + (p & (w - 1));
+            uint32_t a = 0, b = 0, ra = 0, rb = 0;
             if (on0) a = *reinterpret_cast<const uint32_t *>(d0 + o);
             if (on1) b = *reinterpret_cast<const uint32_t *>(d1 + o);
-            if (on0) *reinterpret_cast<uint32_t *>(d0 + o) = a & 0x03ff03ffu;
-            if (on1) *reinterpret_cast<uint32_t *>(d1 + o) = b & 0x03ff03ffu;
+            if (on0 && defer) ra = *reinterpret_cast<const uint32_t *>(r0 + ro);
+            if (on1 && defer) rb = *reinterpret_cast<const uint32_t *>(r1 + ro);
+            if (on0) *reinterpret_cast<uint32_t *>(d0 + o) = defer ? deferred_add2(a, ra, scaled, scale) : a & 0x03ff03ffu;
+            if (on1) *reinterpret_cast<uint32_t *>(d1 + o) = defer ? deferred_add2(b, rb, scaled, scale) : b & 0x03ff03ffu;
         }
     } else {
         for (int p = lane; p < npx; p += 64) {
-            const int o = (p >> l2w) * stride + (p & (w - 1));
-            if (on0) d0[o] = d0[o] & 0x3ff;
-            if (on1) d1[o] = d1[o] & 0x3ff;
+            const int o = (p >> l2w) * stride + (p & (w - 1)), ro = (p >> l2w) * rstride + (p & (w - 1));
+            if (on0) d0[o] = defer ? (uint16_t)res_add_clip(d0[o], r0[ro], scaled, scale) : (uint16_t)(d0[o] & 0x3ff);
+            if (on1) d1[o] = defer ? (uint16_t)res_add_clip(d1[o], r1[ro], scaled, scale) : (uint16_t)(d1[o] & 0x3ff);
         }
     }
 }
 
 __global__ __launch_bounds__(256) void k_lmcs_inverse(ovhip_pic pic, const uint16_t *__restrict__ lut, uint32_t rows_y,
-                                                      const ovhip_itask *__restrict__ tasks, uint32_t n_tasks)
+                                                      const ovhip_itask *__restrict__ tasks, uint32_t n_tasks, ovhip_pic res,
+                                                      const int16_t *__restrict__ scales)
 {
     const uint32_t untag_y = gridDim.y - rows_y;
-    if (blockIdx.y < untag_y) { untag_chroma_tasks(pic, tasks, n_tasks, blockIdx.y * gridDim.x + blockIdx.x); return; }
+    if (blockIdx.y < untag_y) { untag_chroma_tasks(pic, res, scales, tasks, n_tasks, blockIdx.y * gridDim.x + blockIdx.x); return; }
     const uint32_t by = blockIdx.y - untag_y;
 
     __shared__ uint16_t s_lut[1024];
@@ -160,7 +186,8 @@
     return lmcs_scale_launch(ctx, pic, d_regions, n_regions, luts, d_scales, d_tasks, n_tasks, d_state, epoch);
 }
 
-static int lmcs_inverse_launch(ovhip_ctx *ctx, const ovhip_pic *pic, const uint16_t *d_bwd_lut, const ovhip_itask *d_tasks, uint32_t n_tasks, const char *who)
+static int lmcs_inverse_launch(ovhip_ctx *ctx, const ovhip_pic *pic, const uint16_t *d_bwd_lut, const ovhip_itask *d_tasks, uint32_t n_tasks,
+                               const ovhip_pic *res, const int16_t *d_scales, const char *who)
 {
     if (!ctx || !pic || !d_bwd_lut) return OVHIP_EINVAL;
     OV_DEVICE(ctx);
@@ -170,18 +197,27 @@
     const int row_groups = (pic->h + LMCS_ROWS - 1) / LMCS_ROWS;
     const uint32_t gx = (nvx + 255) / 256 > 0 ? (nvx + 255) / 256 : 1, rows_y = row_groups < 4096 ? row_groups : 4096;
     const uint32_t untag_wgs = d_tasks ? (n_tasks + UNTAG_TASKS_PER_WG - 1) / UNTAG_TASKS_PER_WG : 0;
-    hipLaunchKernelGGL(k_lmcs_inverse, dim3(gx, rows_y + (untag_wgs + gx - 1) / gx), dim3(256), 0, ctx->stream, *pic, d_bwd_lut, rows_y, d_tasks, d_tasks ? n_tasks : 0u);
+    hipLaunchKernelGGL(k_lmcs_inverse, dim3(gx, rows_y + (untag_wgs + gx - 1) / gx), dim3(256), 0, ctx->stream, *pic, d_bwd_lut, rows_y, d_tasks, d_tasks ? n_tasks : 0u,
+                       res ? *res : ovhip_pic{}, d_scales);
     OV_LAUNCH_CHECK(ctx, who);
     return OVHIP_OK;
 }
 
 extern "C" int ovhip_lmcs_inverse_launch(ovhip_ctx *ctx, const ovhip_pic *pic, const uint16_t *d_bwd_lut)
 {
-    return lmcs_inverse_launch(ctx, pic, d_bwd_lut, nullptr, 0, "k_lmcs_inverse");
+    return lmcs_inverse_launch(ctx, pic, d_bwd_lut, nullptr, 0, nullptr, nullptr, "k_lmcs_inverse");
 }
 
 extern "C" int ovhip_lmcs_inverse_untag_launch(ovhip_ctx *ctx, const ovhip_pic *pic, const uint16_t *d_bwd_lut, const ovhip_itask *d_tasks, uint32_t n_tasks)
 {
     if (n_tasks && !d_tasks) return OVHIP_EINVAL;
-    return lmcs_inverse_launch(ctx, pic, d_bwd_lut, n_tasks ? d_tasks : nullptr, n_tasks, "k_lmcs_inverse (+ chroma un-tag)");
-}
+    return lmcs_inverse_launch(ctx, pic, d_bwd_lut, n_tasks ? d_tasks : nullptr, n_tasks, nullptr, nullptr, "k_lmcs_inverse (+ chroma un-tag)");
+}
+
+extern "C" int ovhip_lmcs_inverse_untag_launch_(ovhip_ctx *ctx, const ovhip_pic *pic, const uint16_t *d_bwd_lut, const ovhip_itask *d_tasks, uint32_t n_tasks,
+                                                const ovhip_pic *res, const int16_t *d_scales)
+{
+    if (n_tasks && !d_tasks) return OVHIP_EINVAL;
+    return lmcs_inverse_launch(ctx, pic, d_bwd_lut, n_tasks ? d_tasks : nullptr, n_tasks, n_tasks ? res : nullptr, d_scales,
+                               "k_lmcs_inverse (+ chroma un-tag, deferred adds)");
+}
diff --git a/openvvc_amd/csrc/ovvc_band.hip b/openvvc_amd/csrc/ovvc_band.hip
--- a/openvvc_amd/csrc/ovvc_band.hip
+++ b/openvvc_amd/csrc/ovvc_band.hip
@@ -241,7 +241,7 @@
     }
     if (!(stages & OVHIP_STAGE_DBF)) k.n.n_edge_v = k.n.n_edge_h = 0;
     if (!(stages & OVHIP_STAGE_INTRA)) k.n.n_itask = 0;
-    k.n_items = k.n.n_itask && !(pr->stages && (stages & OVHIP_STAGE_INTRA_LEVELS)) ? ovhip_intra_flow_items_(ovhip_rec_itasks(rec, &dummy) + c0.n_itask, k.n.n_itask, nullptr, 0) : 0;
+    k.n_items = k.n.n_itask && !(pr->stages && (stages & OVHIP_STAGE_INTRA_LEVELS)) ? ovhip_intra_flow_items_(ovhip_rec_itasks(rec, &dummy) + c0.n_itask, k.n.n_itask, nullptr, 0, nullptr) : 0;
 
     const Switches sw = switches_of(pr);
     k.t_first = bs->tails; k.t_end = b + 1;
@@ -294,7 +294,7 @@
     k.have_levels = n.n_itask && ovhip_rec_itasks_sorted_range_(rec, c0.n_itask, n.n_itask, (ovhip_itask *)(hb + o_it), bs->level_start, BAND_LEVELS + 2, &n_lv) == 0;
     if (n.n_itask && !k.have_levels && !k.n_items) return ov_fail(ctx, OVHIP_EUNSUP, "ovhip_job_band: a band with more levels than the table holds and blocks the flow launch cannot take", hipSuccess);
     k.h_items = (const uint32_t *)(hb + o_items);
-    if (k.n_items) (void)ovhip_intra_flow_items_((const ovhip_itask *)(hb + o_it), n.n_itask, (uint32_t *)(hb + o_items), k.n_items);
+    if (k.n_items) (void)ovhip_intra_flow_items_((const ovhip_itask *)(hb + o_it), n.n_itask, (uint32_t *)(hb + o_items), k.n_items, nullptr);
     size_t all;
     if (n.n_coef) memcpy(hb + o_coef, ovhip_rec_coefs(rec, &all) + c0.n_coef, (size_t)n.n_coef * 2);
     if (n.n_mc) memcpy(hb + o_mc, ovhip_rec_mc_units(rec, &all) + c0.n_mc, n.n_mc * sizeof(ovhip_mc_unit));
@@ -387,7 +387,7 @@
     const uint16_t *d_bwd = pr->lmcs && (bs->stages & OVHIP_STAGE_ITX) ? bs->d_bwd : nullptr;
     for (int t = k.t_first; t < k.t_end; ++t) {
         const BandRec &T = bs->band[t];
-        if (T.row1 > T.row0) CHK(chain_unmap(j, dst, T.row0, T.row1, d_bwd, T.d_it, T.tagged == 1 ? T.n_it : 0u));
+        if (T.row1 > T.row0) CHK(chain_unmap(j, dst, T.row0, T.row1, d_bwd, T.d_it, T.tagged == 1 ? T.n_it : 0u, nullptr, nullptr));
         if (bs->stages & OVHIP_STAGE_DBF) CHK(chain_deblock(c, T.d_ev, T.n_ev, T.d_eh, T.n_eh, &bs->offs));
     }
     if (k.t_end <= k.t_first) return OVHIP_OK;
diff --git a/openvvc_amd/csrc/ovvc_job.hip.h b/openvvc_amd/csrc/ovvc_job.hip.h
--- a/openvvc_amd/csrc/ovvc_job.hip.h
+++ b/openvvc_amd/csrc/ovvc_job.hip.h
@@ -33,6 +33,7 @@
     size_t rows_end; int rows_pending;
     hipEvent_t ev_rows;
     hipEvent_t ev_h2d, ev_done;
+    uint32_t flow_items, flow_deferred;
     int flow_on_device;
     int flushed;
     const void *packed_prev[24];
@@ -123,7 +124,8 @@
 int chain_predict(const Chain &c, const ovhip_pic *refs_same, const ovhip_pic *refs, uint32_t n_refs, const ovhip_pic *intra, int32_t *d_mv);
 int chain_residual(Chain &c, const uint16_t *d_bwd);
 int chain_ordered(const Chain &c, int n_workers);
-int chain_unmap(ovhip_job *j, const ovhip_pic *dst, int32_t row0, int32_t row1, const uint16_t *d_bwd, const ovhip_itask *d_it, uint32_t n_tagged);
+int chain_unmap(ovhip_job *j, const ovhip_pic *dst, int32_t row0, int32_t row1, const uint16_t *d_bwd, const ovhip_itask *d_it, uint32_t n_tagged,
+                const ovhip_pic *res, const int16_t *d_scales);
 int chain_deblock(const Chain &c, const ovhip_dbf_edge *d_ev, uint32_t n_ev, const ovhip_dbf_edge *d_eh, uint32_t n_eh, const ovhip_dbf_offsets *offs);
 int chain_filters(const Chain &c, const ovhip_sao_ctu *d_sao, const ovhip_alf_pic *alf, int32_t s0, int32_t s1, int32_t a0, int32_t a1);
 int flow_shift_of(int device);
diff --git a/openvvc_amd/csrc/ovvc_picture.hip b/openvvc_amd/csrc/ovvc_picture.hip
--- a/openvvc_amd/csrc/ovvc_picture.hip
+++ b/openvvc_amd/csrc/ovvc_picture.hip
@@ -56,6 +56,8 @@
 extern "C" int ovhip_itx_launch_ex_(ovhip_ctx *ctx, const ovhip_pic *dst, const ovhip_pic *res, const ovhip_tb_cmd *d_cmds, uint32_t n_large,
                                     uint32_t n_small, const uint32_t tiny3[4], const int16_t *d_coefs, const int16_t *d_lmcs_scales, const uint16_t *d_bwd_lut);
 
+extern "C" int ovhip_lmcs_inverse_untag_launch_(ovhip_ctx *ctx, const ovhip_pic *pic, const uint16_t *d_bwd_lut, const ovhip_itask *d_tasks, uint32_t n_tasks,
+                                                const ovhip_pic *res, const int16_t *d_scales);
 extern "C" int ovhip_sao_launch_rows(ovhip_ctx *ctx, const ovhip_pic *dst, const ovhip_pic *src, const ovhip_sao_ctu *d_params, int32_t log2_ctu_s, int32_t row0, int32_t row1);
 extern "C" int ovhip_alf_launch_rows(ovhip_ctx *ctx, const ovhip_pic *dst, const ovhip_pic *src, const ovhip_alf_pic *alf, int32_t row0, int32_t row1);
 
@@ -390,12 +392,13 @@
     return OVHIP_OK;
 }
 
-int chain_unmap(ovhip_job *j, const ovhip_pic *dst, int32_t row0, int32_t row1, const uint16_t *d_bwd, const ovhip_itask *d_it, uint32_t n_tagged)
+int chain_unmap(ovhip_job *j, const ovhip_pic *dst, int32_t row0, int32_t row1, const uint16_t *d_bwd, const ovhip_itask *d_it, uint32_t n_tagged,
+                const ovhip_pic *res, const int16_t *d_scales)
 {
     if (d_bwd) {
         ovhip_pic view = *dst;
         view.y = dst->y + (size_t)row0 * dst->stride_y; view.h = row1 - row0;
-        CHK(ovhip_lmcs_inverse_untag_launch(j->ctx, &view, d_bwd, d_it, n_tagged));
+        CHK(ovhip_lmcs_inverse_untag_launch_(j->ctx, &view, d_bwd, d_it, n_tagged, res, d_scales));
     } else if (n_tagged) CHK(ovhip_intra_flow_untag_launch(j->ctx, dst, d_it, n_tagged, 1));
     else return OVHIP_OK;
     j->st.n_launches++;
@@ -443,6 +446,7 @@
     ovhip_band_counts n;
     size_t n_ciip, n_rpr, n_affr, n_ictu;
     size_t n_items;
+    size_t n_deferred;
     bool ibc;
     int by_ctu; bool ordered, flow;
 };
@@ -487,11 +491,12 @@
     g.it = !g.by_ctu ? ovhip_rec_itasks_sorted(rec, &n_it, &g.lv_start, &g.n_lv)
                      : ovhip_rec_itasks_by_ctu(rec, log2_ctu, &n_it, &g.ictu, &g.n_ictu);
     if (by_flow && n_it) {
-        g.n_items = ovhip_intra_flow_items_(g.it, n_it, j->items_host, j->items_cap / sizeof(uint32_t));
+        g.n_items = ovhip_intra_flow_items_(g.it, n_it, j->items_host, j->items_cap / sizeof(uint32_t), &g.n_deferred);
         if (g.n_items > j->items_cap / sizeof(uint32_t)) {
             CHK(pinned_reserve(j, (void **)&j->items_host, &j->items_cap, g.n_items * sizeof(uint32_t)));
-            g.n_items = ovhip_intra_flow_items_(g.it, n_it, j->items_host, g.n_items);
+            g.n_items = ovhip_intra_flow_items_(g.it, n_it, j->items_host, g.n_items, &g.n_deferred);
         }
+        if (g.n_deferred && !(pr->lmcs && (stages & OVHIP_STAGE_ITX))) g.n_items = 0;
     }
     if (!g.it && ovhip_rec_itask_levels(rec)) return ov_fail(ctx, OVHIP_ENOMEM, "ovhip_job_flush: sorting the ordered tasks", hipSuccess);
     if (g.by_ctu) g.n_lv = ovhip_rec_itask_levels(rec);
@@ -630,6 +635,7 @@
     chain_bind(c, p, ovhip_band_counts{}, g.n, (uint32_t)g.n_rpr, (uint32_t)g.n_affr);
     memcpy(c.cls, g.cls, sizeof(c.cls)); memcpy(c.tiny, g.tiny, sizeof(c.tiny));
     c.h_it = g.it; c.lv_start = g.lv_start; c.n_lv = g.n_lv; c.n_items = g.flow ? (uint32_t)g.n_items : 0; c.ibc = g.ibc;
+    j->flow_items = c.n_items; j->flow_deferred = c.n_items ? (uint32_t)g.n_deferred : 0;
 
     if (stages & OVHIP_STAGE_MC) CHK(launch_predict(j, c, refs, n_refs, intra, pr, g, p));
     if (g.flow) {
@@ -652,7 +658,7 @@
             CHK(chain_ordered(c, g.flow ? flow_worker_count(ctx, pr->flow_workers, g.it, j->items_host, g.n_items, false) : 0));
             if (g.flow) { j->flow_launched = 1; j->st.flow_shift = (uint32_t)flow_shift_of(ctx->device); }
         }
-        CHK(chain_unmap(j, dst, 0, j->h, (pr->lmcs && (stages & OVHIP_STAGE_ITX)) ? d_bwd : nullptr, c.d_it, c.n_items ? c.n_it : 0u));
+        CHK(chain_unmap(j, dst, 0, j->h, (pr->lmcs && (stages & OVHIP_STAGE_ITX)) ? d_bwd : nullptr, c.d_it, c.n_items ? c.n_it : 0u, &j->res, c.d_scales));
     }
     if (stages & OVHIP_STAGE_DBF)
         CHK(chain_deblock(c, (const ovhip_dbf_edge *)p.at[B_EV], g.n.n_edge_v, (const ovhip_dbf_edge *)p.at[B_EH], g.n.n_edge_h, &g.offs));
@@ -928,6 +934,13 @@
     return r;
 }
 
+int ovhip_job_flow_counts(const ovhip_job *j, uint32_t *n_items, uint32_t *n_deferred)
+{
+    if (!j || !n_items || !n_deferred) return OVHIP_EINVAL;
+    *n_items = j->flow_items; *n_deferred = j->flow_deferred;
+    return OVHIP_OK;
+}
+
 int ovhip_job_test_abort_next_flow(ovhip_job *j)
 {
     if (!j) return OVHIP_EINVAL;
diff --git a/openvvc_amd/csrc/ovvc_record_intra.c b/openvvc_amd/csrc/ovvc_record_intra.c
--- a/openvvc_amd/csrc/ovvc_record_intra.c
+++ b/openvvc_amd/csrc/ovvc_record_intra.c
@@ -10,7 +10,8 @@
     if (!r->lvl_y) {
         r->lvl_y = (uint16_t *)calloc((size_t)w4 * h4, 2);
         r->lvl_c = (uint16_t *)calloc((size_t)w4 * h4, 2);
-        if (!r->lvl_y || !r->lvl_c) return -1;
+        r->held_c = (uint8_t *)calloc((size_t)w4 * h4, 1);
+        if (!r->lvl_y || !r->lvl_c || !r->held_c) return -1;
         r->lvl_w4 = w4; r->lvl_h4 = h4; r->lvl_dirty = 0;
     }
     if (r->lvl_dirty) {
@@ -23,7 +24,7 @@
 int
 ovhip_rec_intra_reset_(ovhip_recorder *r)
 {
-    r->n_itask = 0; r->n_ibc = 0; r->n_ilevels = 0; r->max_ilevel = 0;
+    r->n_itask = 0; r->n_ibc = 0; r->n_ilevels = 0; r->max_ilevel = 0; r->n_itask_marked = 0; r->marks_given = 0;
     if (r->lvl_y) r->lvl_dirty = 1;
     return 0;
 }
@@ -31,14 +32,15 @@
 void
 ovhip_rec_intra_free_(ovhip_recorder *r)
 {
-    free(r->lvl_y); free(r->lvl_c); free(r->reg_level);
-    r->lvl_y = r->lvl_c = NULL; r->reg_level = NULL;
+    free(r->lvl_y); free(r->lvl_c); free(r->reg_level); free(r->held_c); free(r->itask_held);
+    r->lvl_y = r->lvl_c = NULL; r->reg_level = NULL; r->held_c = NULL; r->itask_held = NULL; r->cap_iheld = 0;
 }
 
 static int
 max_level(ovhip_recorder *r, const uint16_t *map, int ux0, int uy0, int nx, int ny)
 {
     int m = 0;
+    const int chroma = map == r->lvl_c;
     int x1 = ux0 + nx, y1 = uy0 + ny;
     const int sh = r->log2_ctu - 2;
     if (ux0 < 0) ux0 = 0;
@@ -50,6 +52,7 @@
             const int l = map[y * r->lvl_w4 + x];
             if (!l) continue;
             if (l > m) m = l;
+            if (chroma) r->held_c[y * r->lvl_w4 + x] |= 1;
             const int dx = (x >> sh) - r->scan_cx, dy = (y >> sh) - r->scan_cy;
             if (dx | dy) {
                 if (dy == 0 && dx == -1) r->scan_deps |= 1;
@@ -76,6 +79,20 @@
     if (y1 > r->lvl_h4) y1 = r->lvl_h4;
     for (int y = uy0; y < y1; ++y)
         for (int x = ux0; x < x1; ++x) map[y * r->lvl_w4 + x] = (uint16_t)level;
+}
+
+static void
+set_level_c(ovhip_recorder *r, int ux0, int uy0, int nx, int ny, int level)
+{
+    int x1 = ux0 + nx, y1 = uy0 + ny;
+    if (x1 > r->lvl_w4) x1 = r->lvl_w4;
+    if (y1 > r->lvl_h4) y1 = r->lvl_h4;
+    for (int y = uy0; y < y1; ++y)
+        for (int x = ux0; x < x1; ++x) {
+            const int u = y * r->lvl_w4 + x;
+            r->held_c[u] = r->lvl_c[u] ? 2 : 0;
+            r->lvl_c[u] = (uint16_t)level;
+        }
 }
 
 uint16_t
@@ -132,7 +149,7 @@
         if ((t.kind == OVHIP_IT_RES_C || t.ciip_wt) && (k = max_level(r, r->lvl_c, ux, uy, nx, ny)) > m) m = k;
         if (m >= 65534) return OVHIP_EUNSUP;
         t.level = (uint16_t)(m + 1);
-        set_level(r, r->lvl_c, ux, uy, nx, ny, t.level);
+        set_level_c(r, ux, uy, nx, ny, t.level);
     } else if (t.kind == OVHIP_IT_IBC_L || t.kind == OVHIP_IT_IBC_C) {
         const int sh = cs ? 1 : 2, rnd = (1 << sh) - 1;
         uint16_t *map = cs ? r->lvl_c : r->lvl_y;
@@ -144,7 +161,8 @@
         if (k > m) m = k;
         if (m >= 65534) return OVHIP_EUNSUP;
         t.level = (uint16_t)(m + 1);
-        set_level(r, map, t.x >> sh, t.y >> sh, (w + rnd) >> sh, (h + rnd) >> sh, t.level);
+        if (cs) set_level_c(r, t.x >> sh, t.y >> sh, (w + rnd) >> sh, (h + rnd) >> sh, t.level);
+        else set_level(r, map, t.x >> sh, t.y >> sh, (w + rnd) >> sh, (h + rnd) >> sh, t.level);
         ++r->n_ibc;
     } else if (t.kind == OVHIP_IT_REGION) {
         if (m >= 65534) return OVHIP_EUNSUP;
@@ -155,6 +173,7 @@
     t.ctu_deps = (uint16_t)(0x8000u | ((unsigned)r->log2_ctu << 8) | (r->scan_deps & 0x1f));
     r->itask[r->n_itask] = t;
     if (t.level > r->max_ilevel) r->max_ilevel = t.level;
+    if (r->n_itask_marked == r->n_itask && !r->marks_given) ++r->n_itask_marked;
     return (int)r->n_itask++;
 }
 
@@ -184,6 +203,55 @@
     if (!r || !n) return NULL;
     *n = r->n_itask;
     return r->itask;
+}
+
+static int
+marks_resolve(ovhip_recorder *r)
+{
+    if (!r->n_itask || r->n_itask_marked != r->n_itask) return 0;
+    if (r->marks_given) return 1;
+    if (r->cap_iheld < r->n_itask) {
+        uint8_t *q = (uint8_t *)realloc(r->itask_held, r->cap_itask);
+        if (!q) return 0;
+        r->itask_held = q; r->cap_iheld = r->cap_itask;
+    }
+    for (size_t i = 0; i < r->n_itask; ++i) {
+        const ovhip_itask *t = &r->itask[i];
+        int held = t->kind != OVHIP_IT_RES_C;
+        if (!held) {
+            const int ux = t->x >> 1, uy = t->y >> 1;
+            int x1 = ux + (((1 << t->log2_w) + 1) >> 1), y1 = uy + (((1 << t->log2_h) + 1) >> 1);
+            if (x1 > r->lvl_w4) x1 = r->lvl_w4;
+            if (y1 > r->lvl_h4) y1 = r->lvl_h4;
+            for (int y = uy; y < y1 && !held; ++y)
+                for (int x = ux; x < x1; ++x) held |= r->held_c[y * r->lvl_w4 + x];
+        }
+        r->itask_held[i] = (uint8_t)(held != 0);
+    }
+    return 1;
+}
+
+size_t
+ovhip_rec_itask_deferrable(const ovhip_recorder *rc, uint8_t *marks, size_t cap)
+{
+    ovhip_recorder *r = (ovhip_recorder *)rc;
+    if (!r || !marks_resolve(r)) return 0;
+    for (size_t i = 0; marks && i < r->n_itask && i < cap; ++i) marks[i] = r->itask[i].kind == OVHIP_IT_RES_C && !r->itask_held[i];
+    return r->n_itask;
+}
+
+int
+ovhip_rec_set_itask_deferrable(ovhip_recorder *r, const uint8_t *marks, size_t n)
+{
+    if (!r || (n && !marks) || n != r->n_itask) return OVHIP_EINVAL;
+    if (r->cap_iheld < n) {
+        uint8_t *q = (uint8_t *)realloc(r->itask_held, n);
+        if (!q) return OVHIP_ENOMEM;
+        r->itask_held = q; r->cap_iheld = n;
+    }
+    for (size_t i = 0; i < n; ++i) r->itask_held[i] = !marks[i];
+    r->n_itask_marked = n; r->marks_given = 1;
+    return OVHIP_OK;
 }
 
 const ovhip_itask *
@@ -210,7 +278,13 @@
     start[maxl + 1] = acc;
     uint32_t *fill = start + maxl + 2;
     memcpy(fill, start, (maxl + 2) * sizeof(uint32_t));
-    for (size_t i = 0; i < r->n_itask; ++i) r->itask_sorted[fill[r->itask[i].level]++] = r->itask[i];
+    const int marked = marks_resolve(r);
+    for (size_t i = 0; i < r->n_itask; ++i) {
+        ovhip_itask *o = &r->itask_sorted[fill[r->itask[i].level]++];
+        *o = r->itask[i];
+        o->flags &= (uint16_t)~OVHIP_IF_DEFER;
+        if (marked && o->kind == OVHIP_IT_RES_C && !r->itask_held[i]) o->flags |= OVHIP_IF_DEFER;
+    }
     r->n_ilevels = maxl;
     *n_levels = maxl;
     *level_start = start + 1;
@@ -238,7 +312,7 @@
         acc += c;
     }
     if (nl < cap) level_start[nl] = acc; else fits = 0;
-    for (size_t i = 0; i < n; ++i) out[cnt[t[i].level - minl]++] = t[i];
+    for (size_t i = 0; i < n; ++i) { ovhip_itask *o = &out[cnt[t[i].level - minl]++]; *o = t[i]; o->flags &= (uint16_t)~OVHIP_IF_DEFER; }
     free(cnt);
     *n_levels = nl;
     return fits ? 0 : -1;
diff --git a/openvvc_amd/csrc/ovvc_record_priv.h b/openvvc_amd/csrc/ovvc_record_priv.h
--- a/openvvc_amd/csrc/ovvc_record_priv.h
+++ b/openvvc_amd/csrc/ovvc_record_priv.h
@@ -30,6 +30,7 @@
     uint32_t *ctu_count; size_t cap_ctu_count;
     uint16_t *lvl_y, *lvl_c;
     int32_t lvl_w4, lvl_h4; int lvl_dirty;
+    uint8_t *held_c, *itask_held; size_t cap_iheld, n_itask_marked; int marks_given;
     int log2_ctu;
     int scan_cx, scan_cy; uint32_t scan_deps, region_deps;
     uint16_t *reg_level; size_t cap_reglvl;
diff --git a/openvvc_amd/engine.py b/openvvc_amd/engine.py
--- a/openvvc_amd/engine.py
+++ b/openvvc_amd/engine.py
@@ -459,6 +459,8 @@
                            (capi.REC_EDGE_V, wl.dbf_edges[0]), (capi.REC_EDGE_H, wl.dbf_edges[1])):
             if arr is not None and len(arr):
                 r.append_raw(which, arr)
+        if wl.itasks is not None and len(wl.itasks) and getattr(wl, "itask_deferrable", None) is not None:
+            r.set_itask_deferrable(wl.itask_deferrable)
         offs = capi.DbfOffsets()
         for i in range(8):
             offs.beta[i], offs.tc[i] = wl.dbf_planes["beta_offset"], wl.dbf_planes["tc_offset"]
@@ -546,6 +548,11 @@
 
     def test_abort_next_flow(self):
         self.ctx._chk(self.lib.ovhip_job_test_abort_next_flow(self.j), "job_test_abort_next_flow")
+
+    def flow_counts(self) -> tuple:
+        a, b = C.c_uint32(), C.c_uint32()
+        self.ctx._chk(self.lib.ovhip_job_flow_counts(self.j, C.byref(a), C.byref(b)), "job_flow_counts")
+        return int(a.value), int(b.value)
 
     def stats(self) -> "capi.JobStats":
         s = capi.JobStats()
diff --git a/openvvc_amd/synth.py b/openvvc_amd/synth.py
--- a/openvvc_amd/synth.py
+++ b/openvvc_amd/synth.py
@@ -92,6 +92,7 @@
     sao_params: np.ndarray = None
     alf: dict = None
     itasks: np.ndarray = None
+    itask_deferrable: np.ndarray = None
     calllog: np.ndarray = None
     stats: dict = field(default_factory=dict)
 
@@ -474,6 +475,7 @@
         wl.intra = random_picture(rs, w, h)
     if dev_intra:
         wl.itasks = rec.itasks()
+        wl.itask_deferrable = rec.itask_deferrable()
     if lmcs_on:
         wl.lmcs = _lmcs_tables(rs)
         wl.lmcs_regions = rec.lmcs_regions()
```

After: 3723, median of 6. 1.03x the previous value.
